# JuliaRobotics/RigidBodyDynamics.jl

Hardware: AMD Instinct MI355X
Metric: ABA dynamics! evals/sec (Atlas 30-DoF, batch) (higher is better)
Workload: dtype f64

## Files before the change

### include/rbd_hip.h

```cpp
#ifndef RBD_HIP_H
#define RBD_HIP_H

#include <stdint.h>

#ifdef __cplusplus
extern "C" {
#endif

enum {
  RBD_OK = 0,
  RBD_ERR_INVALID_ARGUMENT = 1,
  RBD_ERR_DIMENSION_MISMATCH = 2,
  RBD_ERR_UNSUPPORTED = 3,
  RBD_ERR_NO_DEVICE = 4,
  RBD_ERR_HIP = 5,
  RBD_ERR_OUT_OF_MEMORY = 6,
  RBD_ERR_HAS_LOOPS = 7,
  RBD_ERR_NOT_POSITIVE_DEFINITE = 8
};

enum {
  RBD_JOINT_FIXED = 0,
  RBD_JOINT_REVOLUTE = 1,
  RBD_JOINT_PRISMATIC = 2,
// ... 1 lines not shown
  RBD_JOINT_PLANAR = 4,
  RBD_JOINT_QUAT_SPHERICAL = 5,
  RBD_JOINT_SINCOS_REVOLUTE = 6
};

enum { RBD_F64 = 0, RBD_F32 = 1 };
enum { RBD_LAYOUT_SOA = 0, RBD_LAYOUT_AOS = 1 };
enum { RBD_MEM_DEVICE = 0, RBD_MEM_HOST = 1 };
enum {
  RBD_ALGO_ABA = 0,
  RBD_ALGO_CRBA_CHOLESKY = 1,
  RBD_ALGO_ABA_LANES = 2,
  RBD_ALGO_ABA_CHAINS = 3,
  RBD_ALGO_ABA_BANKS = 4,
  RBD_ALGO_ABA_TRACKS = 5,
  RBD_ALGO_ABA_WALK = 6,
  RBD_ALGO_ABA_PIPE = 7,
  RBD_ALGO_ABA_COMPILED = 8
};

typedef struct rbd_loop_joint {
  int32_t predecessor;
  int32_t successor;
  int32_t joint_type;
  int32_t _pad;
  double axis[3];
  double pred_rot[9];
  double pred_trans[3];
  double succ_rot[9];
  double succ_trans[3];
  double rotation_from_z_aligned[9];
  double gains[4];
} rbd_loop_joint_t;

typedef struct rbd_contact_point {
  int32_t body;
  int32_t _pad;
  double location[3];
  double hc_k, hc_lambda, hc_n;
  double mu, k, b;
} rbd_contact_point_t;
typedef struct rbd_halfspace {
  double point[3];
  double outward_normal[3];
} rbd_halfspace_t;

typedef struct rbd_flat_model {
  int32_t n_bodies;
  int32_t nq, nv;
  int32_t n_loops;
  const int32_t* parent;
  const int32_t* joint_type;
  const int32_t* q_offset;
  const int32_t* v_offset;
  const double* joint_axis;
  const double* joint_axis2;
  const double* pred_rot;
  const double* pred_trans;
  const double* inertia_moment;
  const double* inertia_cross;
  const double* inertia_mass;
  double gravity[3];
  const rbd_loop_joint_t* loops;
  int32_t n_contact_points;
  int32_t n_halfspaces;
  const rbd_contact_point_t* contact_points;
  const rbd_halfspace_t* halfspaces;
} rbd_flat_model_t;

typedef struct rbd_model rbd_model_t;
typedef struct rbd_ws rbd_ws_t;

typedef struct rbd_opts {
  int32_t layout;
  int32_t memory;
  int32_t algorithm;
  int32_t stabilization;
} rbd_opts_t;

int rbd_model_create(const rbd_flat_model_t* desc, rbd_model_t** out);
int rbd_model_destroy(rbd_model_t* model);
int rbd_model_bank_plan(const rbd_model_t* model, int32_t* lanes, int32_t* first_level_of_bank1, int32_t* bodies_bank0, int32_t* bodies_bank1,
                        int32_t* aba_in_scope);
int rbd_model_track_plan(const rbd_model_t* model, int32_t* dims, int32_t* table, int32_t table_cap, int32_t* ri, int32_t ri_cap, double* rr, int32_t rr_cap);
int rbd_model_reroot_plan(const rbd_model_t* model, int32_t* dims, int32_t* ri, int32_t ri_cap, double* rr, int32_t rr_cap, int32_t* wk, int32_t wk_cap,
                          int32_t* chain_i, double* chain_r, double* fxp);
int rbd_model_chain_plan(const rbd_model_t* model, int32_t* tracks, int32_t* steps, int32_t* lds_fields, int32_t* table, int32_t capacity);
int rbd_model_dims(const rbd_model_t* model, int32_t* n_bodies, int32_t* nq, int32_t* nv, int32_t* nc);

int rbd_workspace_create(const rbd_model_t* model, int32_t max_batch, int32_t device,
                         int32_t dtype, void* stream, rbd_ws_t** out);
int rbd_workspace_destroy(rbd_ws_t* ws);
int rbd_workspace_set_stream(rbd_ws_t* ws, void* stream);
int rbd_workspace_set_loop_gains(rbd_ws_t* ws, const double* gains);
int rbd_sync(rbd_ws_t* ws);

int rbd_dynamics(rbd_ws_t* ws, int32_t B, const void* q, const void* v, const void* tau,
                 const void* fext, void* vdot, void* qdot, void* lambda, const rbd_opts_t* opts);

int rbd_inverse_dynamics(rbd_ws_t* ws, int32_t B, const void* q, const void* v, const void* vdot,
                         const void* fext, void* tau_out, const rbd_opts_t* opts);

int rbd_dynamics_bias(rbd_ws_t* ws, int32_t B, const void* q, const void* v, const void* fext,
                      void* c_out, const rbd_opts_t* opts);

int rbd_inverse_dynamics_bodies(rbd_ws_t* ws, int32_t B, const void* q, const void* v, const void* vdot, const void* fext, void* tau_out,
                                void* jointwrenches_out, void* accelerations_out, const rbd_opts_t* opts);
int rbd_dynamics_bias_bodies(rbd_ws_t* ws, int32_t B, const void* q, const void* v, const void* fext, void* c_out, void* jointwrenches_out,
                             void* accelerations_out, const rbd_opts_t* opts);

int rbd_mass_matrix(rbd_ws_t* ws, int32_t B, const void* q, void* M_out, const rbd_opts_t* opts);

int rbd_mass_matrix_solve(rbd_ws_t* ws, int32_t B, const void* q, const void* rhs, void* x,
                          void* M_out, const rbd_opts_t* opts);
int rbd_mass_matrix_solve_packed(rbd_ws_t* ws, int32_t B, const void* q, const void* rhs, void* x, void* M_packed_out, const rbd_opts_t* opts);

int rbd_cholesky_solve(rbd_ws_t* ws, int32_t B, const void* M, const void* rhs, void* x, void* L_out, const rbd_opts_t* opts);

int rbd_dynamics_result(rbd_ws_t* ws, int32_t B, void* M, void* c, void* K, void* k,
                        const rbd_opts_t* opts);
int rbd_workspace_bind_result(rbd_ws_t* ws, void* M, void* c);

int rbd_simulate(rbd_ws_t* ws, int32_t B, void* q, void* v, const void* tau, const void* fext, double dt, int32_t nsteps,
                 const rbd_opts_t* opts);
int rbd_mk_stage(rbd_ws_t* ws, int32_t B, int32_t stage, double dt, void* q, void* v, const void* vdot_prev, const rbd_opts_t* opts);

enum { RBD_CONTROL_CONSTANT = 0, RBD_CONTROL_TABLE = 1, RBD_CONTROL_PD = 2 };
typedef struct rbd_control {
  int32_t kind;
  int32_t per_stage;
  const void* tau;
  const void* q_des;
  const void* kp;
  const void* kd;
} rbd_control_t;
int rbd_simulate_controlled(rbd_ws_t* ws, int32_t B, void* q, void* v, const rbd_control_t* control, const void* fext, double dt, int32_t nsteps,
                            const rbd_opts_t* opts);

int rbd_model_contact_dims(const rbd_model_t* model, int32_t* n_contact_points, int32_t* n_halfspaces, int32_t* n_additional_states);
int rbd_contact_dynamics(rbd_ws_t* ws, int32_t B, const void* q, const void* v, void* s, void* contactwrenches, void* sdot, const rbd_opts_t* opts);
int rbd_dynamics_contact(rbd_ws_t* ws, int32_t B, const void* q, const void* v, void* s, const void* tau, const void* fext, void* vdot, void* qdot,
                         void* sdot, void* contactwrenches, void* totalwrenches, const rbd_opts_t* opts);
int rbd_simulate_contact(rbd_ws_t* ws, int32_t B, void* q, void* v, void* s, const void* tau, const void* fext, double dt, int32_t nsteps,
                         const rbd_opts_t* opts);

int rbd_kinematics(rbd_ws_t* ws, int32_t B, const void* q, const void* v, void* momentum_matrix, void* com, void* energy,
                   const rbd_opts_t* opts);

int rbd_momentum(rbd_ws_t* ws, int32_t B, const void* q, const void* v, void* out, const rbd_opts_t* opts);

int rbd_geometric_jacobian(rbd_ws_t* ws, int32_t B, const void* q, int32_t base_body, int32_t target_body, void* jac, const rbd_opts_t* opts);

typedef struct rbd_comm rbd_comm_t;
int rbd_comm_unique_id(void* id128);
int rbd_comm_create(const void* id128, int32_t world, int32_t rank, int32_t device, rbd_comm_t** out);
int rbd_comm_destroy(rbd_comm_t* comm);
int rbd_comm_info(const rbd_comm_t* comm, int32_t* world, int32_t* rank);
int rbd_gather(rbd_comm_t* comm, int32_t dtype, const void* shard, void* gathered, int64_t count, int32_t root , void* stream);
int rbd_gatherv(rbd_comm_t* comm, int32_t dtype, const void* shard, void* gathered, const int64_t* counts, int32_t root , void* stream);
const char* rbd_comm_last_error(void);

int rbd_inverse_dynamics_jvp(rbd_ws_t* ws, int32_t B, int32_t ntan, const void* q, const void* v, const void* vdot,
                             const void* fext, const void* dq, const void* dv, const void* dvdot, const void* dfext,
                             void* tau_out, void* dtau_out, const rbd_opts_t* opts);
int rbd_dynamics_jvp(rbd_ws_t* ws, int32_t B, int32_t ntan, const void* q, const void* v, const void* tau,
                     const void* fext, const void* dq, const void* dv, const void* dtau, const void* dfext,
// ... 50 lines not shown
```

### rigidbodydynamics.jl_amd/__init__.py

```python
from .mechanism import (DEFAULT_GRAVITATIONAL_ACCELERATION, CartesianFrame3D, Fixed, FlatModel, Joint, JointType, Mechanism,
                        Planar, Prismatic, QuaternionFloating, QuaternionSpherical, Revolute, RigidBody, SinCosRevolute,
                        SpatialInertia, Transform3D, attach_, flatten, rand_configuration, rand_velocity,
                        remove_fixed_tree_joints_, rot_z_y_x, rotation_between, ContactPoint, HalfSpace3D, HuntCrossleyModel, SoftContactModel,
                        ViscoelasticCoulombModel, add_contact_point_, add_environment_primitive_, hunt_crossley_hertz)
from .urdf import default_urdf_joint_types, parse_pose, parse_urdf, write_urdf
from .builders import (maximal_coordinates, FOUR_BAR_INITIAL_Q, FOUR_BAR_INITIAL_V, double_pendulum, four_bar_linkage, quickstart_double_pendulum,
                       rand_tree_mechanism, randmech, tree_mechanism)
from .flatio import load_flat_model, save_flat_model
from . import _capi
from .state import (PDGains, SE3PDGains, default_constraint_stabilization_gains, TorqueTable, PDControl, jit_source, jit_precompile, jit_status, bank_plan, track_plan, reroot_plan, momentum, momentum_rate_bias, geometric_jacobian_, chain_plan, center_of_mass, gravitational_potential_energy, kinetic_energy, momentum_matrix_, DimensionMismatch, DynamicsResult, MechanismState, dynamics_, dynamics_bias_, dynamics_ode_, inverse_dynamics_, mass_matrix_, unpack_lower, inverse_dynamics_jvp_, dynamics_jvp_, inverse_dynamics_derivatives_, dynamics_derivatives_, simulate_jvp_, simulate_step_derivatives_, inverse_dynamics_vjp_, dynamics_vjp_, simulate_vjp_, jacobian_view, set_points_, point_kinematics_, point_kinematics_vjp_, point_jacobian_view, contact_dynamics_vjp_, dynamics_contact_vjp_, simulate_contact_vjp_,
                    mass_matrix_solve_, rand_, set_configuration_, set_velocity_, simulate_, sync, last_kernel, zero_configuration_)
from .distributed import Comm, gather_results, shard_range, shard_sizes
from . import autograd
```

### rigidbodydynamics.jl_amd/_capi.py

```python
from __future__ import annotations

import atexit
import ctypes
import os

_HERE = os.path.dirname(os.path.abspath(__file__))
LIB_PATH = os.environ.get("RBD_LIB") or os.path.join(_HERE, "csrc", "librbd_hip.so")

RBD_OK = 0
HEADER_VERSION = 700
F64, F32 = 0, 1
LAYOUT_SOA, LAYOUT_AOS = 0, 1
MEM_DEVICE, MEM_HOST = 0, 1
ALGO_ABA, ALGO_CRBA_CHOLESKY, ALGO_ABA_LANES, ALGO_ABA_CHAINS, ALGO_ABA_BANKS, ALGO_ABA_TRACKS, ALGO_ABA_WALK, ALGO_ABA_PIPE, ALGO_ABA_COMPILED = 0, 1, 2, 3, 4, 5, 6, 7, 8

SYMBOLS = (
    "rbd_model_create", "rbd_model_destroy", "rbd_model_dims", "rbd_workspace_create", "rbd_workspace_destroy",
    "rbd_workspace_set_stream", "rbd_sync", "rbd_dynamics", "rbd_inverse_dynamics", "rbd_dynamics_bias", "rbd_mass_matrix",
    "rbd_mass_matrix_solve", "rbd_dynamics_result", "rbd_status_string", "rbd_last_hip_error",
    "rbd_workspace_enable_timing", "rbd_workspace_last_kernel_ms", "rbd_version", "rbd_simulate", "rbd_mk_stage", "rbd_cholesky_solve", "rbd_kinematics", "rbd_model_chain_plan", "rbd_workspace_last_kernel", "rbd_geometric_jacobian", "rbd_momentum", "rbd_model_bank_plan", "rbd_model_track_plan", "rbd_inverse_dynamics_bodies", "rbd_dynamics_bias_bodies",
    "rbd_model_reroot_plan", "rbd_model_contact_dims", "rbd_contact_dynamics", "rbd_dynamics_contact", "rbd_simulate_contact",
    "rbd_workspace_bind_result", "rbd_workspace_set_loop_gains", "rbd_jit_precompile", "rbd_jit_source", "rbd_jit_status", "rbd_jit_wait_idle", "rbd_simulate_controlled", "rbd_comm_unique_id", "rbd_comm_create", "rbd_comm_destroy", "rbd_comm_info", "rbd_gather", "rbd_gatherv", "rbd_mass_matrix_solve_packed", "rbd_comm_last_error", "rbd_jit_check_walk_object",
    "rbd_inverse_dynamics_jvp", "rbd_dynamics_jvp", "rbd_inverse_dynamics_derivatives", "rbd_dynamics_derivatives",
    "rbd_simulate_jvp", "rbd_simulate_step_derivatives",
    "rbd_inverse_dynamics_vjp", "rbd_dynamics_vjp",
    "rbd_simulate_vjp",
    "rbd_workspace_set_points", "rbd_point_kinematics", "rbd_point_kinematics_vjp",
    "rbd_contact_dynamics_vjp", "rbd_dynamics_contact_vjp",
    "rbd_simulate_contact_vjp",
)


class Opts(ctypes.Structure):
    _fields_ = [("layout", ctypes.c_int32), ("memory", ctypes.c_int32), ("algorithm", ctypes.c_int32), ("stabilization", ctypes.c_int32)]


class Control(ctypes.Structure):
    _fields_ = [("kind", ctypes.c_int32), ("per_stage", ctypes.c_int32), ("tau", ctypes.c_void_p), ("q_des", ctypes.c_void_p), ("kp", ctypes.c_void_p),
                ("kd", ctypes.c_void_p)]


CONTROL_CONSTANT, CONTROL_TABLE, CONTROL_PD = 0, 1, 2


class RBDError(RuntimeError):
    def __init__(self, status, where, detail=""):
        self.status = status
        super().__init__(f"{where}: status {status} ({detail})")


_lib = None


def lib():
    global _lib
    if _lib is None:
        if not os.path.exists(LIB_PATH):
            raise FileNotFoundError(f"{LIB_PATH} not built — run `python -c 'import __graft_entry__ as g; g.build()'` "
                                    "(rigidbodydynamics.jl_amd has no CPU fallback)")
        L = ctypes.CDLL(LIB_PATH)
        if L.rbd_version() != HEADER_VERSION:
            raise RuntimeError(f"{LIB_PATH} reports rbd_version {L.rbd_version()}, this binding is for {HEADER_VERSION}: rebuild (csrc/build.sh)")
        vp, i32 = ctypes.c_void_p, ctypes.c_int32
        L.rbd_status_string.restype = ctypes.c_char_p
        L.rbd_status_string.argtypes = [ctypes.c_int]
        L.rbd_last_hip_error.restype = ctypes.c_char_p
        L.rbd_model_create.argtypes = [vp, ctypes.POINTER(vp)]
        L.rbd_model_destroy.argtypes = [vp]
        L.rbd_model_dims.argtypes = [vp] + [ctypes.POINTER(i32)] * 4
        L.rbd_workspace_create.argtypes = [vp, i32, i32, i32, vp, ctypes.POINTER(vp)]
        L.rbd_workspace_destroy.argtypes = [vp]
        L.rbd_workspace_set_stream.argtypes = [vp, vp]
        L.rbd_workspace_bind_result.argtypes = [vp, vp, vp]
        L.rbd_workspace_set_loop_gains.argtypes = [vp, ctypes.POINTER(ctypes.c_double)]
        L.rbd_sync.argtypes = [vp]
        L.rbd_dynamics.argtypes = [vp, i32, vp, vp, vp, vp, vp, vp, vp, ctypes.POINTER(Opts)]
        L.rbd_inverse_dynamics.argtypes = [vp, i32, vp, vp, vp, vp, vp, ctypes.POINTER(Opts)]
        L.rbd_dynamics_bias.argtypes = [vp, i32, vp, vp, vp, vp, ctypes.POINTER(Opts)]
        L.rbd_inverse_dynamics_bodies.argtypes = [vp, i32, vp, vp, vp, vp, vp, vp, vp, ctypes.POINTER(Opts)]
        L.rbd_dynamics_bias_bodies.argtypes = [vp, i32, vp, vp, vp, vp, vp, vp, ctypes.POINTER(Opts)]
        L.rbd_mass_matrix.argtypes = [vp, i32, vp, vp, ctypes.POINTER(Opts)]
        L.rbd_mass_matrix_solve.argtypes = [vp, i32, vp, vp, vp, vp, ctypes.POINTER(Opts)]
        L.rbd_mass_matrix_solve_packed.argtypes = [vp, i32, vp, vp, vp, vp, ctypes.POINTER(Opts)]
        L.rbd_dynamics_result.argtypes = [vp, i32, vp, vp, vp, vp, ctypes.POINTER(Opts)]
        L.rbd_cholesky_solve.argtypes = [vp, i32, vp, vp, vp, vp, ctypes.POINTER(Opts)]
        L.rbd_inverse_dynamics_jvp.argtypes = [vp, i32, i32] + [vp] * 10 + [ctypes.POINTER(Opts)]
        L.rbd_dynamics_jvp.argtypes = [vp, i32, i32] + [vp] * 10 + [ctypes.POINTER(Opts)]
        L.rbd_inverse_dynamics_derivatives.argtypes = [vp, i32] + [vp] * 8 + [ctypes.POINTER(Opts)]
        L.rbd_dynamics_derivatives.argtypes = [vp, i32] + [vp] * 8 + [ctypes.POINTER(Opts)]
        L.rbd_simulate_jvp.argtypes = [vp, i32, i32, vp, vp, vp, vp, ctypes.c_double, i32, vp, vp, vp, vp, ctypes.POINTER(Opts)]
        L.rbd_simulate_step_derivatives.argtypes = [vp, i32, vp, vp, vp, vp, ctypes.c_double, vp, vp, ctypes.POINTER(Opts)]
        L.rbd_inverse_dynamics_vjp.argtypes = [vp, i32] + [vp] * 10 + [ctypes.POINTER(Opts)]
        L.rbd_dynamics_vjp.argtypes = [vp, i32] + [vp] * 10 + [ctypes.POINTER(Opts)]
        L.rbd_simulate_vjp.argtypes = [vp, i32, vp, vp, vp, vp, ctypes.c_double, i32, vp, vp, vp, vp, ctypes.POINTER(Opts)]
        L.rbd_workspace_set_points.argtypes = [vp, i32, ctypes.POINTER(i32), ctypes.POINTER(ctypes.c_double)]
        L.rbd_point_kinematics.argtypes = [vp, i32] + [vp] * 7 + [ctypes.POINTER(Opts)]
        L.rbd_point_kinematics_vjp.argtypes = [vp, i32] + [vp] * 6 + [ctypes.POINTER(Opts)]
        L.rbd_contact_dynamics_vjp.argtypes = [vp, i32] + [vp] * 9 + [ctypes.POINTER(Opts)]
        L.rbd_dynamics_contact_vjp.argtypes = [vp, i32] + [vp] * 15 + [ctypes.POINTER(Opts)]
        L.rbd_simulate_contact_vjp.argtypes = [vp, i32] + [vp] * 5 + [ctypes.c_double, i32] + [vp] * 5 + [ctypes.POINTER(Opts)]
        L.rbd_model_chain_plan.argtypes = [vp, ctypes.POINTER(i32), ctypes.POINTER(i32), ctypes.POINTER(i32), ctypes.POINTER(i32), i32]
        L.rbd_model_track_plan.argtypes = [vp, ctypes.POINTER(i32), ctypes.POINTER(i32), i32, ctypes.POINTER(i32), i32, ctypes.POINTER(ctypes.c_double), i32]
        L.rbd_comm_unique_id.argtypes = [vp]
        L.rbd_comm_create.argtypes = [vp, i32, i32, i32, ctypes.POINTER(vp)]
        L.rbd_comm_destroy.argtypes = [vp]
        L.rbd_comm_info.argtypes = [vp, ctypes.POINTER(i32), ctypes.POINTER(i32)]
        L.rbd_gather.argtypes = [vp, i32, vp, vp, ctypes.c_int64, i32, vp]
        L.rbd_gatherv.argtypes = [vp, i32, vp, vp, ctypes.POINTER(ctypes.c_int64), i32, vp]
        L.rbd_comm_last_error.restype = ctypes.c_char_p
        L.rbd_workspace_last_kernel.argtypes = [vp]
        L.rbd_workspace_last_kernel.restype = ctypes.c_char_p
        L.rbd_geometric_jacobian.argtypes = [vp, i32, vp, i32, i32, vp, ctypes.POINTER(Opts)]
        L.rbd_momentum.argtypes = [vp, i32, vp, vp, vp, ctypes.POINTER(Opts)]
        L.rbd_model_bank_plan.argtypes = [vp] + [ctypes.POINTER(i32)] * 5
        L.rbd_kinematics.argtypes = [vp, i32, vp, vp, vp, vp, vp, ctypes.POINTER(Opts)]
        L.rbd_simulate.argtypes = [vp, i32, vp, vp, vp, vp, ctypes.c_double, i32, ctypes.POINTER(Opts)]
        L.rbd_mk_stage.argtypes = [vp, i32, i32, ctypes.c_double, vp, vp, vp, ctypes.POINTER(Opts)]
        L.rbd_simulate_controlled.argtypes = [vp, i32, vp, vp, ctypes.POINTER(Control), vp, ctypes.c_double, i32, ctypes.POINTER(Opts)]
        L.rbd_model_reroot_plan.argtypes = [vp, ctypes.POINTER(i32), ctypes.POINTER(i32), i32, ctypes.POINTER(ctypes.c_double), i32, ctypes.POINTER(i32), i32,
                                            ctypes.POINTER(i32), ctypes.POINTER(ctypes.c_double), ctypes.POINTER(ctypes.c_double)]
        L.rbd_model_contact_dims.argtypes = [vp] + [ctypes.POINTER(i32)] * 3
        L.rbd_contact_dynamics.argtypes = [vp, i32, vp, vp, vp, vp, vp, ctypes.POINTER(Opts)]
        L.rbd_dynamics_contact.argtypes = [vp, i32, vp, vp, vp, vp, vp, vp, vp, vp, vp, vp, ctypes.POINTER(Opts)]
        L.rbd_simulate_contact.argtypes = [vp, i32, vp, vp, vp, vp, vp, ctypes.c_double, i32, ctypes.POINTER(Opts)]
        L.rbd_workspace_enable_timing.argtypes = [vp, i32]
        L.rbd_jit_precompile.argtypes = [vp, i32, ctypes.c_char_p, ctypes.c_int64]
        L.rbd_jit_source.argtypes = [vp, i32, i32, ctypes.c_char_p, ctypes.c_int64]
        L.rbd_jit_source.restype = ctypes.c_int64
        L.rbd_jit_status.argtypes = [vp, i32, i32]
        L.rbd_jit_check_walk_object.argtypes = [ctypes.c_char_p, ctypes.c_char_p, ctypes.c_int64, ctypes.c_char_p, ctypes.c_int64]
        L.rbd_jit_wait_idle.argtypes = []
        L.rbd_jit_wait_idle.restype = None
        atexit.register(L.rbd_jit_wait_idle)
        L.rbd_workspace_last_kernel_ms.argtypes = [vp, ctypes.POINTER(ctypes.c_float)]
        _lib = L
    return _lib


def check(status: int, where: str):
    if status != RBD_OK:
        L = lib()
        detail = L.rbd_status_string(status).decode()
        hip = L.rbd_last_hip_error().decode()
        if hip and (status in (4, 5, 6) or (status == 3 and "differs from the interpreting kernel" in hip)):
            detail += "; " + hip
        raise RBDError(status, where, detail)
```

### rigidbodydynamics.jl_amd/csrc/rbd_bank.hpp

```cpp
#pragma once

#ifndef RBD_BANK_WAVES
#define RBD_BANK_WAVES 2
#endif
#ifndef RBD_BANK_FK_LDS
#define RBD_BANK_FK_LDS 0
#endif
#ifndef RBD_BANK_HANDOFF_LDS
#define RBD_BANK_HANDOFF_LDS 0
#endif

#ifdef RBD_BANK_FIXED_NL
#define RBD_BANK_UNROLL _Pragma("unroll")
namespace rbd { constexpr int kBankNs[] = {RBD_BANK_FIXED_NS}; }
#define RBD_BK_NL RBD_BANK_FIXED_NL
#define RBD_BK_L0 RBD_BANK_FIXED_L0
#define RBD_BK_NS(l) kBankNs[l]
#ifdef RBD_BANK_FIXED_PERM
#define RBD_BK_PERM(l) (((RBD_BANK_FIXED_PERM) >> (l)) & 1ull)
#else
#define RBD_BK_PERM(l) (kBankNs[l] > 1)
#endif
#else
#define RBD_BANK_UNROLL _Pragma("unroll 1")
#define RBD_BK_NL M.nlevels
#define RBD_BK_L0 M.L0
#define RBD_BK_NS(l) ns_next(nss, M.ns_desc)
#define RBD_BK_PERM(l) ((M.perm_down >> (l)) & 1)
#endif

namespace rbd {

template <typename T> struct alignas(2 * sizeof(T)) Pair2 { T a, b; };

RBD_DEV void wave_lds_sync() {
  __builtin_amdgcn_fence(__ATOMIC_RELEASE, "wavefront");
  __builtin_amdgcn_wave_barrier();
  __builtin_amdgcn_fence(__ATOMIC_ACQUIRE, "wavefront");
}


#define RBD_MASSIGN6(MOV)                                                                                                              \
  unsigned long long sv;                                                                                                               \
  asm volatile("s_and_saveexec_b64 %[sv], %[mk]\n\t" MOV " %[d0], %[s0]\n\t" MOV " %[d1], %[s1]\n\t" MOV " %[d2], %[s2]\n\t" MOV          \
               " %[d3], %[s3]\n\t" MOV " %[d4], %[s4]\n\t" MOV " %[d5], %[s5]\n\ts_mov_b64 exec, %[sv]\n\ts_nop 0"                         \
               : [sv] "=&s"(sv), [d0] "+v"(d[0]), [d1] "+v"(d[1]), [d2] "+v"(d[2]), [d3] "+v"(d[3]), [d4] "+v"(d[4]), [d5] "+v"(d[5])    \
               : [mk] "s"(mask), [s0] "v"(s[0]), [s1] "v"(s[1]), [s2] "v"(s[2]), [s3] "v"(s[3]), [s4] "v"(s[4]), [s5] "v"(s[5])          \
               : "scc")
RBD_DEV void massign6(unsigned long long mask, double* d, const double* s) { RBD_MASSIGN6("v_mov_b64"); }
RBD_DEV void massign6(unsigned long long mask, float* d, const float* s) { RBD_MASSIGN6("v_mov_b32"); }
template <typename T, int N> RBD_DEV void massign(bool m, T* d, const T* s) {
  static_assert(N % 6 == 0, "blocks of 6");
  const unsigned long long mask = __builtin_amdgcn_ballot_w64(m);
#pragma unroll
  for (int k = 0; k < N; k += 6) massign6(mask, d + k, s + k);
}

enum { PK_KIN = 0, PK_FWD = 6, PARK_PAIRS = 16, PK_XCH = 16, XCH_PAIRS = 14, BANK_LDS_PAIRS = PARK_PAIRS + XCH_PAIRS };

template <typename T, int N> RBD_DEV void lds_put(Pair2<T>* col, int pair0, const T* x) {
#pragma unroll
  for (int i = 0; i < (N + 1) / 2; ++i) {
    Pair2<T> v;
    v.a = x[2 * i];
    v.b = (2 * i + 1 < N) ? x[2 * i + 1] : T(0);
    col[(pair0 + i) * 256] = v;
  }
}
template <typename T, int N> RBD_DEV void lds_get(const Pair2<T>* col, int pair0, T* x) {
#pragma unroll
  for (int i = 0; i < (N + 1) / 2; ++i) {
    const Pair2<T> v = col[(pair0 + i) * 256];
    x[2 * i] = v.a;
    if (2 * i + 1 < N) x[2 * i + 1] = v.b;
  }
}

__host__ __device__ constexpr int sym_row(int e) { return e < 6 ? 0 : e < 11 ? 1 : e < 15 ? 2 : e < 18 ? 3 : e < 20 ? 4 : 5; }
__host__ __device__ constexpr int sym_col(int e) { return e - SI(sym_row(e), sym_row(e)) + sym_row(e); }

template <typename T> struct BankRegs {
  Body<T> b;
  const T* rb;
  int pcol;
  T K[24];
  RBD_DEV T* R() { return K; }
  RBD_DEV T* p() { return K + 9; }
  RBD_DEV T* Tw() { return K + 12; }
  RBD_DEV T* vJ() { return K + 18; }
  T S[6], cb[6], IA[21], pA[6], U[6], Dinv, u;
  T tj[6];
  T acc[6], vd[6];
};

template <typename T> RBD_DEV void load_bank_body(const BankModel& M, int k, long B, Body<T>& b) {
  const int tid = blockIdx.x * blockDim.x + threadIdx.x;
  b.lane = threadIdx.x & 63;
  const long wave = tid >> 6;
  const int lps = M.lps;
  b.sub = b.lane & (lps - 1);
  b.base = b.lane - b.sub;
  b.state = wave * (64 / lps) + (b.lane / lps);
  b.valid = (b.sub < M.nbk[k]) && (b.state < B);
  const int4* ib4 = reinterpret_cast<const int4*>(M.ib[k] + (b.sub < M.nbk[k] ? b.sub : 0) * IB_STRIDE);
  const int4 w0 = ib4[0], w1 = ib4[1], w2 = ib4[2], w3 = ib4[3];
  static_assert(IB_PARENT == 0 && IB_JTYPE == 1 && IB_QOFF == 2 && IB_VOFF == 3 && IB_LEVEL == 4 && IB_NCHILD == 5 && IB_ORIG == 6 && IB_CHILD0 == 7 &&
                IB_MAXCHILD == 8 && IB_FLAGS == 15 && IB_STRIDE == 16, "record layout");
  b.parent = w0.x; b.jtype = w0.y; b.qoff = w0.z; b.voff = w0.w;
  b.level = b.valid ? w1.x : -1;
  b.nchild = w1.y; b.orig = w1.z;
  b.child[0] = w1.w; b.child[1] = w2.x; b.child[2] = w2.y; b.child[3] = w2.z; b.child[4] = w2.w; b.child[5] = w3.x; b.child[6] = w3.y; b.child[7] = w3.z;
  b.flags = w3.w;
  b.plane = b.parent >= 0 ? b.base + b.parent : b.lane;
}

template <typename T, bool SIMPLE>
RBD_DEV void bank_fk_commit(bool mine, BankRegs<T>& c, const T* k18 , const T* XR, const T* Xp, const T* tl) {
  const T* pR = k18;
  const T* pp = k18 + 9;
  const T* pT = k18 + 12;
  T n[24];
  matmul3(pR, XR, n);
  matvec3(pR, Xp, n + 9);
#pragma unroll
  for (int k = 0; k < 3; ++k) n[9 + k] += pp[k];
  if (SIMPLE) {
    T S[6];
    matvec3(n, tl, S);
    cross3(n + 9, S, S + 3);
#pragma unroll
    for (int k = 0; k < 6; ++k) n[12 + k] = pT[k] + S[k] * tl[3];
    massign<T, 18>(mine, c.K, n);
  } else {
    xmotion(n, n + 9, tl, n + 18);
#pragma unroll
    for (int k = 0; k < 6; ++k) n[12 + k] = pT[k] + n[18 + k];
    massign<T, 24>(mine, c.K, n);
  }
}
template <typename T, bool SIMPLE> RBD_DEV void bank_fk_step(const BankModel& M, int l, bool perm, BankRegs<T>& c, Pair2<T>* lds, const T* XR, const T* Xp, const T* tl) {
  T k18[18];
  if (RBD_BANK_FK_LDS || perm) {
    if (c.b.level == l - 1 && c.b.nchild >= 1) {
      RBD_KEEP_BRANCH();
      lds_put<T, 18>(lds + threadIdx.x, PK_XCH, c.K);
    }
    wave_lds_sync();
    lds_get<T, 18>(lds + c.pcol, PK_XCH, k18);
    wave_lds_sync();
  } else {
#pragma unroll
    for (int k = 0; k < 18; ++k) k18[k] = from_prev_lane(c.K[k]);
  }
  bank_fk_commit<T, SIMPLE>(c.b.level == l, c, k18, XR, Xp, tl);
}
template <typename T, bool SIMPLE> RBD_DEV void bank_fk_cross(int L0, BankRegs<T>& c, const Pair2<T>* lds, const T* XR, const T* Xp, const T* tl) {
  T k18[18];
// ... 41 lines not shown
  {
    T g[7], h[7];
    g[0] = gv.IA[20] - W[5] * gv.U[5];
    Iac[5] += g[0] * gv.cb[5];
#pragma unroll
    for (int k = 0; k < 6; ++k) g[1 + k] = gv.pA[k] + Iac[k] + W[k] * gv.u;
    if (MODE == 0) {
#pragma unroll
      for (int e = 0; e < 7; ++e) h[e] = from_next_lane(g[e]);
    }
    if (xw) lds_put<T, 7>(mycol, PK_XCH + 10, g);
    if (MODE == 0) {
      if (take0) {
        RBD_KEEP_BRANCH();
        tk.IA[20] += h[0];
#pragma unroll
        for (int k = 0; k < 6; ++k) tk.pA[k] += h[1 + k];
      }
    }
  }
  if (xw) {
    wave_lds_sync();
#pragma unroll 1
    for (int s = (MODE == 1 ? 0 : 1); s < ns; ++s) {
      if (takes && s < tk.b.nchild) {
        RBD_KEEP_BRANCH();
        const Pair2<T>* src = lds + (threadIdx.x - tk.b.sub + child_sel(tk.b, s));
        T x[28];
        lds_get<T, 28>(src, PK_XCH, x);
#pragma unroll
        for (int e = 0; e < 21; ++e) tk.IA[e] += x[e];
#pragma unroll
        for (int k = 0; k < 6; ++k) tk.pA[k] += x[21 + k];
      }
    }
    wave_lds_sync();
  }
}

template <typename T> RBD_DEV void bank_joint_accel(bool mine, BankRegs<T>& r, const T* a_parent) {
  T ap[6], n[6];
#pragma unroll
  for (int k = 0; k < 6; ++k) ap[k] = a_parent[k] + r.cb[k];
  const T x = r.Dinv * (r.u - dot6(r.U, ap));
#pragma unroll
  for (int k = 0; k < 6; ++k) n[k] = ap[k] + r.S[k] * x;
  massign<T, 6>(mine, r.acc, n);
  r.vd[0] = mine ? x : r.vd[0];
}
template <typename T> RBD_DEV void bank_accel_step(const BankModel& M, int l, bool perm, BankRegs<T>& c, Pair2<T>* lds) {
  T ap[6];
  if (RBD_BANK_FK_LDS || perm) {
    if (c.b.level == l - 1 && c.b.nchild >= 1) {
      RBD_KEEP_BRANCH();
      lds_put<T, 6>(lds + threadIdx.x, PK_XCH, c.acc);
    }
    wave_lds_sync();
    lds_get<T, 6>(lds + c.pcol, PK_XCH, ap);
    wave_lds_sync();
  } else {
#pragma unroll
    for (int k = 0; k < 6; ++k) ap[k] = from_prev_lane(c.acc[k]);
  }
  bank_joint_accel(c.b.level == l, c, ap);
}

#ifdef RBD_PROFILE_PHASES
__device__ long long rbd_bank_phase_clock[16];
#define RBD_MARK(i) do { if (blockIdx.x == 0 && threadIdx.x == 0) rbd_bank_phase_clock[i] = clock64(); } while (0)
#else
#define RBD_MARK(i)
#endif

template <typename T, bool R> struct InPtr { typedef const T* type; };
template <typename T> struct InPtr<T, true> { typedef const T* __restrict__ type; };

template <typename T, bool FUSED, bool SIMPLE>
RBD_DEV void aba_bank_body(const BankModel& M, long B, typename InPtr<T, !FUSED>::type q, typename InPtr<T, !FUSED>::type v, const T* __restrict__ tau,
                           const T* __restrict__ fext, T* __restrict__ vdot, T* __restrict__ qdot, Layout Lq, Layout Lv, Layout Lf, const MkFuse& F,
                           Pair2<T>* const lds) {
  Pair2<T>* const col = lds + threadIdx.x;
  RBD_MARK(0);
  BankRegs<T> r0, r1;
  auto fetch = [&](int k, BankRegs<T>& c, T* qj, T* vj) {
    load_bank_body(M, k, B, c.b);
    c.rb = reinterpret_cast<const T*>(M.rb[k]) + (c.b.sub < M.nbk[k] ? c.b.sub : 0) * RB_STRIDE;
    c.pcol = (int)threadIdx.x - c.b.sub + (c.b.parent >= 0 ? c.b.parent : c.b.sub);
    if (SIMPLE) {
      const bool fl = c.b.jtype == RBD_JOINT_QUAT_FLOATING;
      const long sc = c.b.state < B ? c.b.state : B - 1;
      const T* qp = q + ((long)c.b.qoff * Lq.sk + sc * Lq.sb);
      const long va = (long)c.b.voff * Lv.sk + sc * Lv.sb;
      const bool hv = v != nullptr, ht = tau != nullptr;
      qj[0] = qp[0];
      vj[0] = hv ? v[va] : T(0);
      c.tj[0] = ht ? tau[va] : T(0);
#pragma unroll
      for (int k2 = 1; k2 < 7; ++k2) qj[k2] = T(0);
#pragma unroll
      for (int k2 = 1; k2 < 6; ++k2) { vj[k2] = T(0); c.tj[k2] = T(0); }
      if (fl) {
        RBD_KEEP_BRANCH();
#pragma unroll
        for (int k2 = 1; k2 < 7; ++k2) qj[k2] = qp[k2 * Lq.sk];
        if (hv) {
#pragma unroll
          for (int k2 = 1; k2 < 6; ++k2) vj[k2] = v[va + k2 * Lv.sk];
        }
        if (ht) {
#pragma unroll
          for (int k2 = 1; k2 < 6; ++k2) c.tj[k2] = tau[va + k2 * Lv.sk];
        }
      }
    } else {
      load_joint_q(c.b, q, Lq, qj);
      load_joint_v(c.b, v, Lv, vj);
      load_joint_v(c.b, tau, Lv, c.tj);
    }
  };
  auto setup = [&](BankRegs<T>& c, T* qj, T* vj, T* XR, T* Xp, T* tl, T* ta ) {
    if (SIMPLE) {
      const bool fl = c.b.jtype == RBD_JOINT_QUAT_FLOATING;
      const T ax[3] = {c.rb[RB_AXIS], c.rb[RB_AXIS + 1], c.rb[RB_AXIS + 2]};
      T Rj[9], pj[3] = {T(0), T(0), T(0)};
      T sn, cs;
      ta[0] = ax[0]; ta[1] = ax[1]; ta[2] = ax[2]; ta[3] = vj[0];
      sincos_fast(qj[0], &sn, &cs);
      rot_axis_sc(ax, sn, cs, Rj);
#pragma unroll
      for (int k = 0; k < 3; ++k) { tl[k] = ax[k] * vj[0]; tl[3 + k] = T(0); }
      if (fl) {
        RBD_KEEP_BRANCH();
        rot_quat(qj[0], qj[1], qj[2], qj[3], Rj);
        pj[0] = qj[4]; pj[1] = qj[5]; pj[2] = qj[6];
#pragma unroll
        for (int k = 0; k < 6; ++k) tl[k] = vj[k];
        if (qdot != nullptr && c.b.valid) {
          const T w = qj[0], x = qj[1], y = qj[2], z = qj[3];
          T o[7];
          o[0] = (-x * vj[0] - y * vj[1] - z * vj[2]) * T(0.5);
          o[1] = (w * vj[0] - z * vj[1] + y * vj[2]) * T(0.5);
          o[2] = (z * vj[0] + w * vj[1] - x * vj[2]) * T(0.5);
          o[3] = (-y * vj[0] + x * vj[1] + w * vj[2]) * T(0.5);
          matvec3(Rj, vj + 3, o + 4);
#pragma unroll
          for (int k = 0; k < 7; ++k) qdot[(long)(c.b.qoff + k) * Lq.sk + c.b.state * Lq.sb] = o[k];
        }
      } else if (qdot != nullptr && c.b.valid) {
        qdot[(long)c.b.qoff * Lq.sk + c.b.state * Lq.sb] = vj[0];
      }
      T XpR[9], Xpp[3];
#pragma unroll
      for (int k = 0; k < 9; ++k) XpR[k] = c.rb[RB_XPR + k];
#pragma unroll
      for (int k = 0; k < 3; ++k) Xpp[k] = c.rb[RB_XPP + k];
      matmul3(XpR, Rj, XR);
      matvec3(XpR, pj, Xp);
#pragma unroll
      for (int k = 0; k < 3; ++k) Xp[k] += Xpp[k];
    } else {
      store_qdot(c.b, qdot, Lq, qj, vj);
      local_transform(c.b, c.rb, qj, XR, Xp);
      local_joint_motion(c.b, c.rb, vj, tl);
    }
#pragma unroll
    for (int i = 0; i < 9; ++i) c.R()[i] = XR[i];
#pragma unroll
    for (int i = 0; i < 3; ++i) c.p()[i] = Xp[i];
    xmotion(c.R(), c.p(), tl, c.Tw());
    if (SIMPLE) {
      c.K[18] = ta[3];
      c.K[19] = T(0);
    } else {
#pragma unroll
      for (int i = 0; i < 6; ++i) c.vJ()[i] = c.Tw()[i];
    }
  };
  auto terms = [&](BankRegs<T>& c, bool accumulate) {
    const bool floating = c.b.jtype == RBD_JOINT_QUAT_FLOATING;
    if (SIMPLE) {
      const T ax[3] = {c.rb[RB_AXIS], c.rb[RB_AXIS + 1], c.rb[RB_AXIS + 2]};
      matvec3(c.R(), ax, c.S);
      cross3(c.p(), c.S, c.S + 3);
    } else {
      T e1[6] = {T(1), T(0), T(0), T(0), T(0), T(0)}, sl[6];
      local_joint_motion(c.b, c.rb, e1, sl);
      xmotion(c.R(), c.p(), sl, c.S);
    }
    if (floating || (!SIMPLE && joint_nv(c.b.jtype) == 0)) {
#pragma unroll
      for (int i = 0; i < 6; ++i) c.S[i] = T(0);
    }
    if (SIMPLE) {
      se3_comm(c.Tw(), c.S, c.cb);
#pragma unroll
      for (int i = 0; i < 6; ++i) c.cb[i] *= c.K[18];
    } else {
      se3_comm(c.Tw(), c.vJ(), c.cb);
    }
    RInertia<T> I;
    T Jb[6], mc[3], fe[6];
#pragma unroll
    for (int i = 0; i < 6; ++i) Jb[i] = c.rb[RB_J + i];
#pragma unroll
    for (int i = 0; i < 3; ++i) mc[i] = c.rb[RB_MC + i];
    inertia_to_root(Jb, mc, c.rb[RB_M], c.R(), c.p(), I);
    T Io[21], po[6];
    sym6_from_inertia(I, Io);
    momentum_cross(I, c.Tw(), po);
    load_body_wrench(c.b, fext, Lf, fe);
#pragma unroll
    for (int i = 0; i < 21; ++i) c.IA[i] = accumulate ? c.IA[i] + Io[i] : Io[i];
#pragma unroll
    for (int i = 0; i < 6; ++i) c.pA[i] = accumulate ? c.pA[i] + (po[i] - fe[i]) : po[i] - fe[i];
#pragma unroll
    for (int i = 0; i < 6; ++i) c.U[i] = T(0);
    c.Dinv = T(0);
    c.u = T(0);
    if (floating) xforce(c.R(), c.p(), c.tj, c.U);
  };

  T qj0[7], vj0[6], qj1[7], vj1[6];
  fetch(0, r0, qj0, vj0);
  fetch(1, r1, qj1, vj1);
  if (FUSED) {
    if (F.close_prev) {
      mk_stage_lane(r0.b, 4, (T)F.dt, qj0, vj0, (const T*)nullptr, F.W, (T*)F.q_state, (T*)F.v_state, Lq, Lv);
      mk_stage_lane(r1.b, 4, (T)F.dt, qj1, vj1, (const T*)nullptr, F.W, (T*)F.q_state, (T*)F.v_state, Lq, Lv);
    }
    mk_stage_lane(r0.b, F.stage, (T)F.dt, qj0, vj0, (const T*)nullptr, F.W, (T*)F.q_state, (T*)F.v_state, Lq, Lv);
    mk_stage_lane(r1.b, F.stage, (T)F.dt, qj1, vj1, (const T*)nullptr, F.W, (T*)F.q_state, (T*)F.v_state, Lq, Lv);
    pd_control_lane(r0.b, F, Lq, qj0, vj0, r0.tj);
    pd_control_lane(r1.b, F, Lq, qj1, vj1, r1.tj);
  }
  {
    T XR[9], Xp[3], tl[6], ta[4];
    setup(r0, qj0, vj0, XR, Xp, tl, ta);
    RBD_MARK(1);
RBD_BANK_UNROLL
    for (int l = 1; l < RBD_BK_L0; ++l) bank_fk_step<T, SIMPLE>(M, l, RBD_BK_PERM(l), r0, lds, XR, Xp, SIMPLE ? ta : tl);
  }
  {
    T XR[9], Xp[3], tl[6], ta[4];
    RBD_MARK(2);
    setup(r1, qj1, vj1, XR, Xp, tl, ta);
    RBD_MARK(3);
    lds_put<T, (SIMPLE ? 20 : 24)>(col, PK_KIN, r0.K);
    wave_lds_sync();
    bank_fk_cross<T, SIMPLE>(RBD_BK_L0, r1, lds, XR, Xp, SIMPLE ? ta : tl);
RBD_BANK_UNROLL
    for (int l = RBD_BK_L0 + 1; l < RBD_BK_NL; ++l) bank_fk_step<T, SIMPLE>(M, l, RBD_BK_PERM(l), r1, lds, XR, Xp, SIMPLE ? ta : tl);
  }
  RBD_MARK(4);
  terms(r1, false);
  RBD_MARK(5);

  NsStream nss = ns_begin(M.ns_desc);
  (void)nss;
RBD_BANK_UNROLL
  for (int l = RBD_BK_NL - 1; l > RBD_BK_L0; --l) {
    bank_finish_joint<T, SIMPLE>(l, r1);
    bank_handoff<T, RBD_BANK_HANDOFF_LDS>(l, RBD_BK_NS(l), r1, r1, lds);
  }
  bank_finish_joint<T, SIMPLE>(RBD_BK_L0, r1);
  RBD_MARK(6);
#pragma unroll
  for (int i = 0; i < 21; ++i) r0.IA[i] = T(0);
#pragma unroll
  for (int i = 0; i < 6; ++i) r0.pA[i] = T(0);
  bank_handoff<T, 1>(RBD_BK_L0, RBD_BK_NS(RBD_BK_L0), r1, r0, lds);
  {
    lds_get<T, (SIMPLE ? 20 : 24)>(col, PK_KIN, r0.K);
    T f20[20];
#pragma unroll
    for (int i = 0; i < 6; ++i) { f20[i] = r1.U[i]; f20[8 + i] = r1.S[i]; f20[14 + i] = r1.cb[i]; }
    f20[6] = r1.Dinv;
    f20[7] = r1.u;
    lds_put<T, 20>(col, PK_FWD, f20);
  }
  RBD_MARK(7);
  terms(r0, true);
  RBD_MARK(8);
RBD_BANK_UNROLL
  for (int l = RBD_BK_L0 - 1; l >= 1; --l) {
    bank_finish_joint<T, SIMPLE>(l, r0);
    bank_handoff<T, RBD_BANK_HANDOFF_LDS>(l, RBD_BK_NS(l), r0, r0, lds);
  }
  bank_finish_joint<T, SIMPLE>(0, r0);
  RBD_MARK(9);

#pragma unroll
  for (int i = 0; i < 6; ++i) { r0.acc[i] = T(0); r0.vd[i] = T(0); }
  {
    const T a0[6] = {T(0), T(0), T(0), T(-M.gravity[0]), T(-M.gravity[1]), T(-M.gravity[2])};
    BankRegs<T>& c = r0;
    const bool fl0 = c.b.level == 0 && c.b.jtype == RBD_JOINT_QUAT_FLOATING;
    T fa[6] = {T(0), T(0), T(0), T(0), T(0), T(0)}, fv[6] = {T(0), T(0), T(0), T(0), T(0), T(0)};
    if (fl0) {
      RBD_KEEP_BRANCH();
      T rhs[6], d[6], k12[12];
#pragma unroll
      for (int i = 0; i < 6; ++i) rhs[i] = c.U[i] - c.pA[i];
      sym6_solve(c.IA, rhs, fa);
#pragma unroll
      for (int i = 0; i < 6; ++i) d[i] = fa[i] - a0[i];
      lds_get<T, 12>(col, PK_KIN, k12);
      xmotion_inv(k12, k12 + 9, d, fv);
    }
    massign<T, 6>(fl0, c.acc, fa);
    massign<T, 6>(fl0, c.vd, fv);
    bank_joint_accel(c.b.level == 0 && !fl0, c, a0);
  }
RBD_BANK_UNROLL
  for (int l = 1; l < RBD_BK_L0; ++l) bank_accel_step<T>(M, l, RBD_BK_PERM(l), r0, lds);
  RBD_MARK(10);
  if (vdot) store_joint_v(r0.b, vdot, Lv, r0.vd);
  if (FUSED) store_joint_v(r0.b, (T*)F.W.vd[F.stage], Lv, r0.vd);
  {
    T f20[20];
    lds_get<T, 20>(col, PK_FWD, f20);
#pragma unroll
    for (int i = 0; i < 6; ++i) {
      r1.U[i] = f20[i];
      r1.S[i] = f20[8 + i];
      r1.cb[i] = f20[14 + i];
      r1.acc[i] = T(0);
      r1.vd[i] = T(0);
    }
    r1.Dinv = f20[6];
    r1.u = f20[7];
  }
  {
    lds_put<T, 6>(col, PK_XCH, r0.acc);
    wave_lds_sync();
    T ap[6];
    lds_get<T, 6>(lds + r1.pcol, PK_XCH, ap);
    wave_lds_sync();
    bank_joint_accel(r1.b.level == RBD_BK_L0, r1, ap);
  }
RBD_BANK_UNROLL
  for (int l = RBD_BK_L0 + 1; l < RBD_BK_NL; ++l) bank_accel_step<T>(M, l, RBD_BK_PERM(l), r1, lds);
  RBD_MARK(11);
  if (vdot) store_joint_v(r1.b, vdot, Lv, r1.vd);
  if (FUSED) store_joint_v(r1.b, (T*)F.W.vd[F.stage], Lv, r1.vd);
}
#ifndef RBD_BANK_FIXED_NL
template <typename T, bool FUSED, bool SIMPLE>
__global__ __launch_bounds__(256, RBD_BANK_WAVES) void aba_bank_kernel(BankModel M, long B, typename InPtr<T, !FUSED>::type q, typename InPtr<T, !FUSED>::type v,
                                                         const T* __restrict__ tau, const T* __restrict__ fext, T* __restrict__ vdot,
                                                         T* __restrict__ qdot, Layout Lq, Layout Lv, Layout Lf, MkFuse F) {
  extern __shared__ double bank_lds_raw[];
  aba_bank_body<T, FUSED, SIMPLE>(M, B, q, v, tau, fext, vdot, qdot, Lq, Lv, Lf, F, reinterpret_cast<Pair2<T>*>(bank_lds_raw));
}
#endif

enum { RNEA_LDS_PAIRS = 12 };
template <typename T> struct RneaRegs {
  Body<T> b;
  const T* rb;
  int pcol;
  T K[24], w[6];
  RBD_DEV T* R() { return K; }
  RBD_DEV T* p() { return K + 9; }
  RBD_DEV T* Tw() { return K + 12; }
  RBD_DEV T* acc() { return K + 18; }
};

template <typename T, bool SIMPLE>
RBD_DEV void rnea_fk_commit(bool mine, RneaRegs<T>& c, const T* k24, const T* XR, const T* Xp, const T* tl, const T* al) {
  const T* pR = k24;
  const T* pp = k24 + 9;
  const T* pT = k24 + 12;
  const T* pa = k24 + 18;
  T n[24], vJ[6], nT[6], cr[6], aj[6];
  matmul3(pR, XR, n);
  matvec3(pR, Xp, n + 9);
#pragma unroll
  for (int k = 0; k < 3; ++k) n[9 + k] += pp[k];
  if (SIMPLE) {
    T S[6];
    matvec3(n, tl, S);
    cross3(n + 9, S, S + 3);
#pragma unroll
    for (int k = 0; k < 6; ++k) { vJ[k] = S[k] * tl[3]; aj[k] = S[k] * tl[4]; }
  } else {
    xmotion(n, n + 9, tl, vJ);
    xmotion(n, n + 9, al, aj);
  }
#pragma unroll
  for (int k = 0; k < 6; ++k) { n[12 + k] = pT[k] + vJ[k]; nT[k] = -n[12 + k]; }
  se3_comm(nT, pT, cr);
#pragma unroll
  for (int k = 0; k < 6; ++k) n[18 + k] = pa[k] + cr[k] + aj[k];
  massign<T, 24>(mine, c.K, n);
}
template <typename T, bool SIMPLE>
RBD_DEV void rnea_fk_step(const BankModel& M, int l, bool perm, RneaRegs<T>& c, Pair2<T>* lds, const T* XR, const T* Xp, const T* tl, const T* al) {
  T k24[24];
  if (perm) {
    if (c.b.level == l - 1 && c.b.nchild >= 1) {
      RBD_KEEP_BRANCH();
      lds_put<T, 24>(lds + threadIdx.x, 0, c.K);
    }
    wave_lds_sync();
    lds_get<T, 24>(lds + c.pcol, 0, k24);
    wave_lds_sync();
  } else {
#pragma unroll
    for (int k = 0; k < 24; ++k) k24[k] = from_prev_lane(c.K[k]);
  }
  rnea_fk_commit<T, SIMPLE>(c.b.level == l, c, k24, XR, Xp, tl, al);
}

template <typename T, bool CROSS> RBD_DEV void rnea_gather(int l, int ns, const RneaRegs<T>& gv, RneaRegs<T>& tk) {
  const bool takes = (tk.b.level == l - 1);
  if (!CROSS) {
    T t[6];
#pragma unroll
    for (int k = 0; k < 6; ++k) t[k] = from_next_lane(gv.w[k]);
    if (takes && tk.b.nchild >= 1) {
      RBD_KEEP_BRANCH();
#pragma unroll
      for (int k = 0; k < 6; ++k) tk.w[k] += t[k];
    }
  }
#pragma unroll 1
  for (int s = CROSS ? 0 : 1; s < ns; ++s) {
    const bool take = takes && (s < tk.b.nchild);
    const int src = take ? tk.b.base + child_sel(tk.b, s) : tk.b.lane;
    T t[6];
#pragma unroll
    for (int k = 0; k < 6; ++k) t[k] = shfl(gv.w[k], src);
    if (take) {
      RBD_KEEP_BRANCH();
#pragma unroll
      for (int k = 0; k < 6; ++k) tk.w[k] += t[k];
    }
  }
}

template <typename T, bool SIMPLE>
RBD_DEV void rnea_bank_body(const BankModel& M, long B, int ncol, const T* __restrict__ q, const T* __restrict__ v, const T* __restrict__ vdot,
                            const T* __restrict__ fext, T* __restrict__ tau, T* __restrict__ qdot, Layout Lq, Layout Lv, Layout Lf, T* __restrict__ acc_out,
                            T* __restrict__ jw_out, Pair2<T>* const lds) {
  RneaRegs<T> r0, r1;
  const bool out_vec = store6_vec(acc_out ? acc_out : jw_out, Lf, (int)sizeof(T)) && store6_vec(jw_out ? jw_out : acc_out, Lf, (int)sizeof(T));
  auto fetch = [&](int k, RneaRegs<T>& c, T* qj, T* vj, T* aj) {
    load_bank_body(M, k, B, c.b);
    c.rb = reinterpret_cast<const T*>(M.rb[k]) + (c.b.sub < M.nbk[k] ? c.b.sub : 0) * RB_STRIDE;
    c.pcol = (int)threadIdx.x - c.b.sub + (c.b.parent >= 0 ? c.b.parent : c.b.sub);
    if (SIMPLE) {
      const bool fl = c.b.jtype == RBD_JOINT_QUAT_FLOATING;
      const long sc = c.b.state < B ? c.b.state : B - 1;
      const T* qp = q + ((long)c.b.qoff * Lq.sk + sc * Lq.sb);
      const long va = (long)c.b.voff * Lv.sk + sc * Lv.sb;
      const bool hv = v != nullptr, ha = vdot != nullptr;
      qj[0] = qp[0];
      vj[0] = hv ? v[va] : T(0);
      aj[0] = ha ? vdot[va] : T(0);
#pragma unroll
      for (int k2 = 1; k2 < 7; ++k2) qj[k2] = T(0);
#pragma unroll
      for (int k2 = 1; k2 < 6; ++k2) { vj[k2] = T(0); aj[k2] = T(0); }
      if (fl) {
        RBD_KEEP_BRANCH();
#pragma unroll
        for (int k2 = 1; k2 < 7; ++k2) qj[k2] = qp[k2 * Lq.sk];
        if (hv) {
#pragma unroll
          for (int k2 = 1; k2 < 6; ++k2) vj[k2] = v[va + k2 * Lv.sk];
        }
        if (ha) {
#pragma unroll
          for (int k2 = 1; k2 < 6; ++k2) aj[k2] = vdot[va + k2 * Lv.sk];
        }
      }
    } else {
      load_joint_q(c.b, q, Lq, qj);
      load_joint_v(c.b, v, Lv, vj);
      load_joint_v(c.b, vdot, Lv, aj);
    }
  };
  auto setup = [&](RneaRegs<T>& c, const T* qj, const T* vj, const T* aj, T* XR, T* Xp, T* tl, T* al, T* ta) {
    if (SIMPLE) {
      const bool fl = c.b.jtype == RBD_JOINT_QUAT_FLOATING;
      const T ax[3] = {c.rb[RB_AXIS], c.rb[RB_AXIS + 1], c.rb[RB_AXIS + 2]};
      ta[0] = ax[0]; ta[1] = ax[1]; ta[2] = ax[2]; ta[3] = vj[0]; ta[4] = aj[0];
      T Rj[9], pj[3] = {T(0), T(0), T(0)}, sn, cs;
      sincos_fast(qj[0], &sn, &cs);
      rot_axis_sc(ax, sn, cs, Rj);
#pragma unroll
      for (int k = 0; k < 3; ++k) { tl[k] = ax[k] * vj[0]; tl[3 + k] = T(0); al[k] = ax[k] * aj[0]; al[3 + k] = T(0); }
      if (fl) {
        RBD_KEEP_BRANCH();
        rot_quat(qj[0], qj[1], qj[2], qj[3], Rj);
        pj[0] = qj[4]; pj[1] = qj[5]; pj[2] = qj[6];
#pragma unroll
        for (int k = 0; k < 6; ++k) { tl[k] = vj[k]; al[k] = aj[k]; }
        if (qdot != nullptr && c.b.valid) {
          const T w = qj[0], x = qj[1], y = qj[2], z = qj[3];
          T o[7];
          o[0] = (-x * vj[0] - y * vj[1] - z * vj[2]) * T(0.5);
          o[1] = (w * vj[0] - z * vj[1] + y * vj[2]) * T(0.5);
          o[2] = (z * vj[0] + w * vj[1] - x * vj[2]) * T(0.5);
          o[3] = (-y * vj[0] + x * vj[1] + w * vj[2]) * T(0.5);
          matvec3(Rj, vj + 3, o + 4);
#pragma unroll
          for (int k = 0; k < 7; ++k) qdot[(long)(c.b.qoff + k) * Lq.sk + c.b.state * Lq.sb] = o[k];
        }
      } else if (qdot != nullptr && c.b.valid) {
        qdot[(long)c.b.qoff * Lq.sk + c.b.state * Lq.sb] = vj[0];
      }
      T XpR[9], Xpp[3];
#pragma unroll
      for (int k = 0; k < 9; ++k) XpR[k] = c.rb[RB_XPR + k];
#pragma unroll
      for (int k = 0; k < 3; ++k) Xpp[k] = c.rb[RB_XPP + k];
      matmul3(XpR, Rj, XR);
      matvec3(XpR, pj, Xp);
#pragma unroll
      for (int k = 0; k < 3; ++k) Xp[k] += Xpp[k];
    } else {
      store_qdot(c.b, qdot, Lq, qj, vj);
      local_transform(c.b, c.rb, qj, XR, Xp);
      local_joint_motion(c.b, c.rb, vj, tl);
      local_joint_motion(c.b, c.rb, aj, al);
    }
#pragma unroll
    for (int i = 0; i < 9; ++i) c.R()[i] = XR[i];
#pragma unroll
    for (int i = 0; i < 3; ++i) c.p()[i] = Xp[i];
    xmotion(c.R(), c.p(), tl, c.Tw());
    xmotion(c.R(), c.p(), al, c.acc());
    c.acc()[3] -= T(M.gravity[0]); c.acc()[4] -= T(M.gravity[1]); c.acc()[5] -= T(M.gravity[2]);
  };
  auto newton_euler = [&](RneaRegs<T>& c) {
    RInertia<T> I;
    T Jb[6], mc[3], Ia[6], x[6], fe[6];
#pragma unroll
    for (int k = 0; k < 6; ++k) Jb[k] = c.rb[RB_J + k];
#pragma unroll
    for (int k = 0; k < 3; ++k) mc[k] = c.rb[RB_MC + k];
    inertia_to_root(Jb, mc, c.rb[RB_M], c.R(), c.p(), I);
    mul_inertia(I, c.acc(), Ia);
    momentum_cross(I, c.Tw(), x);
    load_body_wrench(c.b, fext, Lf, fe);
#pragma unroll
    for (int k = 0; k < 6; ++k) c.w[k] = Ia[k] + x[k] - fe[k];
    if (acc_out != nullptr && c.b.valid) store6(acc_out, 6L * c.b.orig, Lf, c.b.state, c.acc(), out_vec);
  };
  auto project = [&](RneaRegs<T>& c) {
    T out[6] = {T(0), T(0), T(0), T(0), T(0), T(0)};
    if (c.b.jtype == RBD_JOINT_QUAT_FLOATING) {
      xforce_inv(c.R(), c.p(), c.w, out);
    } else if (SIMPLE) {
      const T ax[3] = {c.rb[RB_AXIS], c.rb[RB_AXIS + 1], c.rb[RB_AXIS + 2]};
      T S[6];
      matvec3(c.R(), ax, S);
      cross3(c.p(), S, S + 3);
      out[0] = dot6(S, c.w);
    } else {
      const T ax[3] = {c.rb[RB_AXIS], c.rb[RB_AXIS + 1], c.rb[RB_AXIS + 2]}, ay[3] = {c.rb[RB_AXIS2], c.rb[RB_AXIS2 + 1], c.rb[RB_AXIS2 + 2]};
      for (int k = 0; k < ncol; ++k) {
        T sl[6], S[6];
        subspace_col(c.b.jtype, ax, ay, k, sl);
        xmotion(c.R(), c.p(), sl, S);
        const T d = dot6(S, c.w);
        if (k == 0) out[0] = d; else if (k == 1) out[1] = d; else out[2] = d;
      }
    }
    store_joint_v(c.b, tau, Lv, out);
    if (jw_out != nullptr && c.b.valid) store6(jw_out, 6L * c.b.orig, Lf, c.b.state, c.w, out_vec);
  };

  T qj0[7], vj0[6], aj0[6], qj1[7], vj1[6], aj1[6];
  fetch(0, r0, qj0, vj0, aj0);
  fetch(1, r1, qj1, vj1, aj1);
  {
    T XR[9], Xp[3], tl[6], al[6], ta[5];
    setup(r0, qj0, vj0, aj0, XR, Xp, tl, al, ta);
RBD_BANK_UNROLL
    for (int l = 1; l < RBD_BK_L0; ++l) rnea_fk_step<T, SIMPLE>(M, l, RBD_BK_PERM(l), r0, lds, XR, Xp, SIMPLE ? ta : tl, al);
  }
  {
    T XR[9], Xp[3], tl[6], al[6], ta[5];
    setup(r1, qj1, vj1, aj1, XR, Xp, tl, al, ta);
    {
      T k24[24];
      lds_put<T, 24>(lds + threadIdx.x, 0, r0.K);
      wave_lds_sync();
      lds_get<T, 24>(lds + r1.pcol, 0, k24);
      wave_lds_sync();
      rnea_fk_commit<T, SIMPLE>(r1.b.level == RBD_BK_L0, r1, k24, XR, Xp, SIMPLE ? ta : tl, al);
    }
RBD_BANK_UNROLL
    for (int l = RBD_BK_L0 + 1; l < RBD_BK_NL; ++l) rnea_fk_step<T, SIMPLE>(M, l, RBD_BK_PERM(l), r1, lds, XR, Xp, SIMPLE ? ta : tl, al);
  }
  newton_euler(r1);
  newton_euler(r0);
  NsStream nss = ns_begin(M.ns_desc);
  (void)nss;
RBD_BANK_UNROLL
  for (int l = RBD_BK_NL - 1; l > RBD_BK_L0; --l) rnea_gather<T, false>(l, RBD_BK_NS(l), r1, r1);
  rnea_gather<T, true>(RBD_BK_L0, RBD_BK_NS(RBD_BK_L0), r1, r0);
RBD_BANK_UNROLL
  for (int l = RBD_BK_L0 - 1; l >= 1; --l) rnea_gather<T, false>(l, RBD_BK_NS(l), r0, r0);
  project(r0);
  project(r1);
}
#ifndef RBD_BANK_FIXED_NL
template <typename T, bool SIMPLE>
__global__ __launch_bounds__(256, 2) void rnea_bank_kernel(BankModel M, long B, int ncol, const T* __restrict__ q, const T* __restrict__ v,
                                                          const T* __restrict__ vdot, const T* __restrict__ fext, T* __restrict__ tau,
                                                          T* __restrict__ qdot, Layout Lq, Layout Lv, Layout Lf, T* __restrict__ acc_out,
                                                          T* __restrict__ jw_out) {
  extern __shared__ double bank_lds_raw[];
  rnea_bank_body<T, SIMPLE>(M, B, ncol, q, v, vdot, fext, tau, qdot, Lq, Lv, Lf, acc_out, jw_out, reinterpret_cast<Pair2<T>*>(bank_lds_raw));
}
#endif

}
```

### rigidbodydynamics.jl_amd/csrc/rbd_bank_kernels.hip

```cpp
#include "rbd_lane.hpp"
#include "rbd_internal.hpp"
#include "rbd_bank.hpp"

namespace rbd {

static_assert(BANK_LDS_PAIRS == 30, "rbd_capi.hip sizes the resident batch of the banked kernel with BANK_LDS_PAIRS_HOST = 30");
template <typename T> static size_t bank_lds_bytes() { return (size_t)BANK_LDS_PAIRS * 256 * sizeof(Pair2<T>); }

template <typename T>
hipError_t launch_aba_bank(const BankModel& M, long B, const void* q, const void* v, const void* tau, const void* fext, void* vdot, void* qdot,
                           Layout Lq, Layout Lv, Layout Lf, hipStream_t s, const MkFuse* fuse) {
  MkFuse F{};
  F.stage = -1;
  if (fuse) F = *fuse;
  const long spw = 64 / M.lps, waves = (B + spw - 1) / spw;
  const dim3 grid((unsigned)((waves + 3) / 4)), block(256);
  const size_t lds = bank_lds_bytes<T>();
#define RBD_LAUNCH_BANK(FU, SI) \
  hipLaunchKernelGGL((aba_bank_kernel<T, FU, SI>), grid, block, lds, s, M, B, (const T*)q, (const T*)v, (const T*)tau, (const T*)fext, (T*)vdot, (T*)qdot, Lq, Lv, Lf, F)
  if (F.stage >= 0) { if (M.simple) RBD_LAUNCH_BANK(true, true); else RBD_LAUNCH_BANK(true, false); }
  else if (M.simple) RBD_LAUNCH_BANK(false, true);
  else RBD_LAUNCH_BANK(false, false);
#undef RBD_LAUNCH_BANK
  return hipGetLastError();
}
template <typename T> hipError_t configure_bank_kernels() {
  const int lds = (int)bank_lds_bytes<T>();
  hipError_t e = hipFuncSetAttribute(reinterpret_cast<const void*>(&aba_bank_kernel<T, false, false>), hipFuncAttributeMaxDynamicSharedMemorySize, lds);
  if (e == hipSuccess) e = hipFuncSetAttribute(reinterpret_cast<const void*>(&aba_bank_kernel<T, false, true>), hipFuncAttributeMaxDynamicSharedMemorySize, lds);
  if (e == hipSuccess) e = hipFuncSetAttribute(reinterpret_cast<const void*>(&aba_bank_kernel<T, true, false>), hipFuncAttributeMaxDynamicSharedMemorySize, lds);
  if (e == hipSuccess) e = hipFuncSetAttribute(reinterpret_cast<const void*>(&aba_bank_kernel<T, true, true>), hipFuncAttributeMaxDynamicSharedMemorySize, lds);
  return e;
}
template hipError_t configure_bank_kernels<double>();
template hipError_t configure_bank_kernels<float>();

#ifdef RBD_PROFILE_PHASES
extern "C" int rbd_debug_bank_phase_clock(long long* out16) {
  return (int)hipMemcpyFromSymbol(out16, HIP_SYMBOL(rbd_bank_phase_clock), sizeof(long long) * 16);
}
#endif
template hipError_t launch_aba_bank<double>(const BankModel&, long, const void*, const void*, const void*, const void*, void*, void*, Layout, Layout, Layout, hipStream_t, const MkFuse*);
template hipError_t launch_aba_bank<float>(const BankModel&, long, const void*, const void*, const void*, const void*, void*, void*, Layout, Layout, Layout, hipStream_t, const MkFuse*);

template <typename T>
hipError_t launch_rnea_bank(const BankModel& M, long B, int ncol, const void* q, const void* v, const void* vdot, const void* fext, void* tau, void* qdot,
                            Layout Lq, Layout Lv, Layout Lf, hipStream_t s, void* acc_out, void* jw_out) {
  const long spw = 64 / M.lps, waves = (B + spw - 1) / spw;
  const size_t lds = (size_t)RNEA_LDS_PAIRS * 256 * sizeof(Pair2<T>);
  if (M.simple)
    hipLaunchKernelGGL((rnea_bank_kernel<T, true>), dim3((unsigned)((waves + 3) / 4)), dim3(256), lds, s, M, B, ncol, (const T*)q, (const T*)v, (const T*)vdot,
                       (const T*)fext, (T*)tau, (T*)qdot, Lq, Lv, Lf, (T*)acc_out, (T*)jw_out);
  else
    hipLaunchKernelGGL((rnea_bank_kernel<T, false>), dim3((unsigned)((waves + 3) / 4)), dim3(256), lds, s, M, B, ncol, (const T*)q, (const T*)v, (const T*)vdot,
                       (const T*)fext, (T*)tau, (T*)qdot, Lq, Lv, Lf, (T*)acc_out, (T*)jw_out);
  return hipGetLastError();
}
template hipError_t launch_rnea_bank<double>(const BankModel&, long, int, const void*, const void*, const void*, const void*, void*, void*, Layout, Layout, Layout, hipStream_t, void*, void*);
template hipError_t launch_rnea_bank<float>(const BankModel&, long, int, const void*, const void*, const void*, const void*, void*, void*, Layout, Layout, Layout, hipStream_t, void*, void*);

}
```

### rigidbodydynamics.jl_amd/csrc/rbd_capi.hip

```cpp
#include "rbd_capi_internal.hpp"
enum { BANK_LDS_PAIRS_HOST = 30 };

thread_local std::string g_last_hip_error;

static int joint_nq_host(int t) {
  switch (t) {
    case RBD_JOINT_FIXED: return 0;
    case RBD_JOINT_REVOLUTE: case RBD_JOINT_PRISMATIC: return 1;
    case RBD_JOINT_QUAT_FLOATING: return 7;
    case RBD_JOINT_PLANAR: return 3;
    case RBD_JOINT_QUAT_SPHERICAL: return 4;
    case RBD_JOINT_SINCOS_REVOLUTE: return 2;
    default: return -1;
  }
}
static int joint_nv_host(int t) {
  switch (t) {
    case RBD_JOINT_FIXED: return 0;
    case RBD_JOINT_REVOLUTE: case RBD_JOINT_PRISMATIC: case RBD_JOINT_SINCOS_REVOLUTE: return 1;
    case RBD_JOINT_QUAT_FLOATING: return 6;
    case RBD_JOINT_PLANAR: case RBD_JOINT_QUAT_SPHERICAL: return 3;
    default: return -1;
  }
}

long tune(const char* key, long dflt, bool* has) {
  if (has) *has = false;
  const char* e = getenv("RBD_TUNE");
  if (!e) return dflt;
  const size_t n = strlen(key);
  for (const char* p = e; *p;) {
    const char* end = strchr(p, ',');
    const size_t len = end ? (size_t)(end - p) : strlen(p);
    if (len > n && memcmp(p, key, n) == 0 && p[n] == '=') { if (has) *has = true; return atol(p + n + 1); }
    if (len == n && memcmp(p, key, n) == 0) { if (has) *has = true; return 1; }
    if (!end) break;
    p = end + 1;
  }
  return dflt;
}

static std::string loop_program_source(const rbd_model* m, int dtype, std::vector<int32_t>* xi_store);
static int bank_simple(const rbd_model* m);
static std::string bank_program_source(const rbd_model* m, int dtype, int simple);
static std::string walk_program_source(const rbd_model* m, int dtype, bool rerooted, int kind = 0, int pair = 0);
static bool walk_program_rerooted(const rbd_model* m, int dtype, int pair = 0);

extern "C" {

int rbd_version(void) { return RBD_HIP_H_VERSION; }
static std::string program_source(const rbd_model* m, int32_t dtype, int32_t family) {
  if (!m || (dtype != RBD_F32 && dtype != RBD_F64) || family < 0 || family > SPEC_KIN) return std::string();
  if (family == SPEC_KIN) return m->spec_plan().ok ? spec_source(m->spec_plan(), m->nb, m->nq, m->nv, m->row_mask.data(), m->gravity, dtype, SPEC_KIN) : std::string();
  if (family == SPEC_FAMILIES + 6) return walk_program_source(m, dtype, walk_program_rerooted(m, dtype), 2);
  if (family == SPEC_FAMILIES + 7) return dtype == RBD_F32 ? walk_program_source(m, dtype, walk_program_rerooted(m, dtype, 1), 2, 1) : std::string();
  std::vector<int32_t> xi;
  if (family < SPEC_FAMILIES && !m->spec_plan().ok) return std::string();
  if (family == SPEC_FAMILIES + 5) return bank_program_source(m, dtype, bank_simple(m));
  return family == SPEC_FAMILIES + 4 ? (dtype == RBD_F32 ? walk_program_source(m, dtype, false, 1, 1) : std::string())
         : family == SPEC_FAMILIES + 3 ? (dtype == RBD_F32 ? walk_program_source(m, dtype, walk_program_rerooted(m, dtype, 1), 0, 1) : std::string())
         : family == SPEC_FAMILIES + 2 ? walk_program_source(m, dtype, false, 1)
         : family == SPEC_FAMILIES + 1 ? walk_program_source(m, dtype, walk_program_rerooted(m, dtype))
         : family == SPEC_FAMILIES ? loop_program_source(m, dtype, &xi)
                                   : spec_source(m->spec_plan(), m->nb, m->nq, m->nv, m->row_mask.data(), m->gravity, dtype, family);
}
static bool family_is_walk(int family) { return (family > SPEC_FAMILIES && family <= SPEC_FAMILIES + 4) || family == SPEC_FAMILIES + 6 || family == SPEC_FAMILIES + 7; }
static int code_object_get(const std::string& src, bool walk, bool wait, std::vector<char>* code, std::string* log) {
  return walk ? jit_walk_code_object_get(src, wait, code, log) : jit_code_object_get(src, wait, code, log);
}
int64_t rbd_jit_source(const rbd_model_t* m, int32_t dtype, int32_t family, char* buf, int64_t cap) {
  const std::string s = program_source(m, dtype, family);
  if (s.empty()) return -1;
  if (buf && cap > 0) { const int64_t n = std::min<int64_t>(cap - 1, (int64_t)s.size()); memcpy(buf, s.data(), (size_t)n); buf[n] = 0; }
  return (int64_t)s.size();
}
void rbd_jit_wait_idle(void) { jit_wait_idle(); }
int rbd_jit_check_walk_object(const char* source, const void* code, int64_t size, char* log, int64_t cap) {
  if (log && cap > 0) log[0] = 0;
  if (!source || !code || size <= 0) return RBD_ERR_INVALID_ARGUMENT;
  std::vector<char> c((const char*)code, (const char*)code + size);
  std::string l;
  const bool ok = jit_walk_admit(source, &c, &l);
  if (log && cap > 0) { const int64_t n = std::min<int64_t>(cap - 1, (int64_t)l.size()); memcpy(log, l.data(), (size_t)n); log[n] = 0; }
  return ok ? RBD_OK : RBD_ERR_UNSUPPORTED;
// ... 226 lines not shown
    const int nc = (int)kids[i].size();
    if (nc > IB_MAXCHILD) { delete m; return RBD_ERR_UNSUPPORTED; }
    ib[IB_NCHILD] = nc;
    for (int k = 0; k < nc; ++k) ib[IB_CHILD0 + k] = m->slot_of[kids[i][k]];
    if (nc > m->maxchild) m->maxchild = nc;
  }
  for (int s = 0; s < nb; ++s) {
    const int i = m->order[s];
    for (int k = 0; k < (int)kids[i].size(); ++k) m->ib[(size_t)s * IB_STRIDE + IB_CHILD0 + k] = m->slot_of[kids[i][k]];
  }
  if (m->nlevels > MAX_LEVELS) { delete m; return RBD_ERR_UNSUPPORTED; }
  m->nslots.assign(MAX_LEVELS, 0);
  m->perm_down = 0;
  for (int s = 0; s < nb; ++s) {
    const int nc = m->ib[(size_t)s * IB_STRIDE + IB_NCHILD];
    if (nc > 0 && nc > m->nslots[level[s] + 1]) m->nslots[level[s] + 1] = nc;
    const int ps = m->ib[(size_t)s * IB_STRIDE + IB_PARENT];
    if (ps >= 0 && ps != s - 1) m->perm_down |= (uint64_t)1 << level[s];
    if (ps >= 0 && m->ib[(size_t)ps * IB_STRIDE + IB_CHILD0] != ps + 1) { delete m; return RBD_ERR_INVALID_ARGUMENT; }
  }
  m->rb.assign((size_t)nb * RB_STRIDE, 0.0);
  for (int s = 0; s < nb; ++s) {
    const int i = m->order[s];
    double* rb = &m->rb[(size_t)s * RB_STRIDE];
    for (int k = 0; k < 3; ++k) rb[RB_AXIS + k] = d->joint_axis[3 * i + k];
    if (d->joint_axis2) for (int k = 0; k < 3; ++k) rb[RB_AXIS2 + k] = d->joint_axis2[3 * i + k];
    for (int k = 0; k < 9; ++k) rb[RB_XPR + k] = d->pred_rot[9 * i + k];
    for (int k = 0; k < 3; ++k) rb[RB_XPP + k] = d->pred_trans[3 * i + k];
    const double* J = d->inertia_moment + 9 * i;
    rb[RB_J + 0] = J[0]; rb[RB_J + 1] = J[1]; rb[RB_J + 2] = J[2]; rb[RB_J + 3] = J[4]; rb[RB_J + 4] = J[5]; rb[RB_J + 5] = J[8];
    for (int k = 0; k < 3; ++k) rb[RB_MC + k] = d->inertia_cross[3 * i + k];
    rb[RB_M] = d->inertia_mass[i];
  }
  m->dof_body.assign(m->nv > 0 ? m->nv : 1, 0);
  for (int i = 0; i < nb; ++i)
    for (int k = 0; k < joint_nv_host(d->joint_type[i]); ++k) m->dof_body[d->v_offset[i] + k] = m->slot_of[i];
  m->anc.assign((size_t)nb * m->nlevels, -1);
  for (int s = 0; s < nb; ++s) {
    int a = s;
    for (int k = 0; k < m->nlevels && a >= 0; ++k) { m->anc[(size_t)s * m->nlevels + k] = a; a = m->ib[(size_t)a * IB_STRIDE + IB_PARENT]; }
  }
  m->row_words = std::max(1, (m->nv + 63) / 64);
  m->row_mask.assign((size_t)(m->nv > 0 ? m->nv : 1) * m->row_words, 0);
  for (int r = 0; r < m->nv; ++r) {
    const int sr = m->dof_body[r];
    for (int c = 0; c <= r; ++c) {
      const int sc = m->dof_body[c];
      bool sup = false;
      for (int k = 0; k < m->nlevels; ++k) sup |= (m->anc[(size_t)sr * m->nlevels + k] == sc);
      if (sup) m->row_mask[(size_t)r * m->row_words + c / 64] |= (uint64_t)1 << (c % 64);
    }
  }
  m->nc = 0;
  m->jt_ref.assign(d->joint_type, d->joint_type + nb);
  m->parent_ref.assign(d->parent, d->parent + nb);
  m->voff_ref.assign(d->v_offset, d->v_offset + nb);
  m->qoff_ref.assign(d->q_offset, d->q_offset + nb);
  for (int i = 0; i < nb; ++i) {
    const int jt = d->joint_type[i];
    if (jt == RBD_JOINT_QUAT_FLOATING) { m->mkf.push_back(d->q_offset[i]); m->mkf.push_back(d->v_offset[i]); }
    else if (jt == RBD_JOINT_REVOLUTE || jt == RBD_JOINT_PRISMATIC || jt == RBD_JOINT_SINCOS_REVOLUTE) { m->mk1.push_back(d->q_offset[i]); m->mk1.push_back(d->v_offset[i]); m->mk1.push_back(jt); }
  }
  m->loop_fused_ok = d->n_loops > 0 && nb <= 4 && m->nv <= 4;
  for (int i = 0; i < nb && m->loop_fused_ok; ++i) {
    const int t = d->joint_type[i];
    m->loop_fused_ok = d->parent[i] < i && (t == RBD_JOINT_REVOLUTE || t == RBD_JOINT_PRISMATIC || t == RBD_JOINT_SINCOS_REVOLUTE || t == RBD_JOINT_FIXED);
  }
  m->axis_ref.assign(d->joint_axis, d->joint_axis + 3 * nb);
  if (d->joint_axis2) m->axis2_ref.assign(d->joint_axis2, d->joint_axis2 + 3 * nb); else m->axis2_ref.assign(3 * nb, 0.0);
  if (int lst = build_loop_tables(m, d)) { delete m; return lst; }
  m->bank_aba_ok = (m->nloops == 0 && !m->has3dof && !m->inner_floating);
  if (m->nlevels >= 2) {
    std::vector<int> per_level(m->nlevels, 0);
    for (int s = 0; s < nb; ++s) per_level[level[s]]++;
    int best_L0 = 0, best_lanes = 1 << 30, best_diff = 1 << 30;
    for (int L0 = 1; L0 < m->nlevels; ++L0) {
      int cA = 0, cB = 0;
      for (int l = 0; l < m->nlevels; ++l) (l < L0 ? cA : cB) += per_level[l];
      int lanes = 1;
      while (lanes < std::max(cA, cB)) lanes <<= 1;
      const int diff = std::abs(cA - cB);
      if (lanes < best_lanes || (lanes == best_lanes && diff < best_diff)) { best_lanes = lanes; best_L0 = L0; best_diff = diff; }
    }
    if (best_lanes < m->lps) {
      m->bank_lps = best_lanes; m->bank_L0 = best_L0;
      std::vector<int> bslot(nb, -1);
      int cnt[2] = {0, 0};
      for (int s = 0; s < nb; ++s) bslot[s] = cnt[level[s] >= best_L0]++;
      m->bank_nb[0] = cnt[0]; m->bank_nb[1] = cnt[1];
      for (int k = 0; k < 2; ++k) { m->bank_ib[k].assign((size_t)std::max(cnt[k], 1) * IB_STRIDE, -1); m->bank_rb[k].assign((size_t)std::max(cnt[k], 1) * RB_STRIDE, 0.0); }
      m->bank_perm_down = 0;
      for (int s = 0; s < nb; ++s) {
        const int k = level[s] >= best_L0, j = bslot[s];
        const int32_t* src = &m->ib[(size_t)s * IB_STRIDE];
        int32_t* dst = &m->bank_ib[k][(size_t)j * IB_STRIDE];
        memcpy(dst, src, sizeof(int32_t) * IB_STRIDE);
        const int ps = src[IB_PARENT];
        dst[IB_PARENT] = ps < 0 ? -1 : bslot[ps];
        for (int c2 = 0; c2 < src[IB_NCHILD]; ++c2) dst[IB_CHILD0 + c2] = bslot[src[IB_CHILD0 + c2]];
        if (ps >= 0 && level[s] != best_L0 && bslot[ps] != j - 1) { m->bank_perm_down |= (uint64_t)1 << level[s]; dst[IB_FLAGS] |= BFD_NOTFIRST; }
        memcpy(&m->bank_rb[k][(size_t)j * RB_STRIDE], &m->rb[(size_t)s * RB_STRIDE], sizeof(double) * RB_STRIDE);
      }
    }
  }
  {
    int nheads = 0;
    for (int s = 0; s < nb; ++s) {
      const int ps = m->ib[(size_t)s * IB_STRIDE + IB_PARENT];
      if (ps < 0 || m->ib[(size_t)ps * IB_STRIDE + IB_CHILD0] != s) ++nheads;
    }
    int G = 1;
    while (G < nheads && G < 4) G <<= 1;
    if (m->nloops == 0) m->chain = build_chain_plan(nb, m->ib, G);
    if (m->nloops == 0 && G <= 4) m->track = build_track_plan(nb, m->ib, m->rb, G);
    if (m->track.ok) m->walk = build_walk_plan(m->track.ns, m->track.G, m->track.ri);
    if (m->nloops == 0 && m->nv <= 64) m->state = build_state_plan(nb, m->ib, m->rb);
    if (m->nloops == 0 && m->nv <= 64 && !m->state.ok) m->state_wide = build_state_plan(nb, m->ib, m->rb, true);
  }
  if (m->bank_aba_ok) {
    m->rr = build_reroot(d);
    if (m->rr.ok) {
      const Reroot& R = m->rr;
      rbd_model::RrSlots& S = m->rrs;
      std::vector<std::vector<int>> kd(nb);
      for (int i = 0; i < nb; ++i) if (R.parent[i] >= 0) kd[R.parent[i]].push_back(i);
      std::vector<int> ord, slot(nb, -1), lev(nb, 0);
      {
        std::vector<int> stack{R.root};
        while (!stack.empty()) {
          const int i = stack.back(); stack.pop_back();
          slot[i] = (int)ord.size();
          ord.push_back(i);
          for (auto it = kd[i].rbegin(); it != kd[i].rend(); ++it) stack.push_back(*it);
        }
      }
      bool fits = (int)ord.size() == nb;
      for (int i = 0; i < nb && fits; ++i) fits = (int)kd[i].size() <= IB_MAXCHILD;
      if (fits) {
        S.ib.assign((size_t)nb * IB_STRIDE, -1);
        S.rb.assign((size_t)nb * RB_STRIDE, 0.0);
        S.nslots.assign(MAX_LEVELS, 0);
        for (int s2 = 0; s2 < nb; ++s2) {
          const int i = ord[s2], p = R.parent[i], ps = p < 0 ? -1 : slot[p];
          lev[s2] = ps < 0 ? 0 : lev[ps] + 1;
          if (lev[s2] + 1 > S.nlevels) S.nlevels = lev[s2] + 1;
          int32_t* ib = &S.ib[(size_t)s2 * IB_STRIDE];
          ib[IB_PARENT] = ps; ib[IB_JTYPE] = R.jtype[i]; ib[IB_QOFF] = R.qoff[i]; ib[IB_VOFF] = R.voff[i]; ib[IB_LEVEL] = lev[s2]; ib[IB_ORIG] = i;
          ib[IB_FLAGS] = R.flags[i];
          ib[IB_NCHILD] = (int)kd[i].size();
          for (int k = 0; k < (int)kd[i].size(); ++k) ib[IB_CHILD0 + k] = slot[kd[i][k]];
          double* rb = &S.rb[(size_t)s2 * RB_STRIDE];
          for (int k = 0; k < 3; ++k) { rb[RB_AXIS + k] = R.axis[3 * i + k]; rb[RB_AXIS2 + k] = R.axis2[3 * i + k]; rb[RB_XPP + k] = R.Xpp[3 * i + k]; rb[RB_MC + k] = R.mc[3 * i + k]; }
          for (int k = 0; k < 9; ++k) rb[RB_XPR + k] = R.XpR[9 * i + k];
          for (int k = 0; k < 6; ++k) rb[RB_J + k] = R.J6[6 * i + k];
          rb[RB_M] = R.mass[i];
        }
        for (int s2 = 0; s2 < nb; ++s2) {
          const int nc = S.ib[(size_t)s2 * IB_STRIDE + IB_NCHILD];
          if (nc > 0 && nc > S.nslots[lev[s2] + 1]) S.nslots[lev[s2] + 1] = nc;
        }
        int nheads = 0;
        for (int s2 = 0; s2 < nb; ++s2) {
          const int ps = S.ib[(size_t)s2 * IB_STRIDE + IB_PARENT];
          if (ps < 0 || S.ib[(size_t)ps * IB_STRIDE + IB_CHILD0] != s2) ++nheads;
        }
        int G = 1;
        while (G < nheads && G < 4) G <<= 1;
        S.track = build_track_plan(nb, S.ib, S.rb, G);
        if (S.track.ok) {
          S.walk = build_walk_plan(S.track.ns, S.track.G, S.track.ri);
          if (S.walk.ok)
            for (size_t k = 0; k < S.walk.wk.size(); ++k) {
              const int e = S.track.tab[k];
              if (e >= 0) S.walk.wk[k] |= S.ib[(size_t)e * IB_STRIDE + IB_FLAGS] << 8;
            }
        }
        S.ok = true;
      }
    }
  }
  *out = m;
  return RBD_OK;
}

int rbd_model_destroy(rbd_model_t* m) {
  delete m;
  return RBD_OK;
}

int rbd_model_bank_plan(const rbd_model_t* m, int32_t* lanes, int32_t* first_level_of_bank1, int32_t* bodies_bank0, int32_t* bodies_bank1,
                        int32_t* aba_in_scope) {
  if (!m) return RBD_ERR_INVALID_ARGUMENT;
  if (m->bank_lps <= 0) return RBD_ERR_UNSUPPORTED;
  if (lanes) *lanes = m->bank_lps;
  if (first_level_of_bank1) *first_level_of_bank1 = m->bank_L0;
  if (bodies_bank0) *bodies_bank0 = m->bank_nb[0];
  if (bodies_bank1) *bodies_bank1 = m->bank_nb[1];
  if (aba_in_scope) *aba_in_scope = m->bank_aba_ok;
  return RBD_OK;
}

int rbd_model_chain_plan(const rbd_model_t* m, int32_t* tracks, int32_t* steps, int32_t* lds_fields, int32_t* table, int32_t capacity) {
  if (!m) return RBD_ERR_INVALID_ARGUMENT;
  if (!m->chain.ok) return RBD_ERR_UNSUPPORTED;
  if (tracks) *tracks = m->chain.G;
  if (steps) *steps = m->chain.ns;
  if (lds_fields) *lds_fields = 0;
  if (table) {
    if (capacity < (int32_t)m->chain.tab.size()) return RBD_ERR_DIMENSION_MISMATCH;
    for (size_t i = 0; i < m->chain.tab.size(); ++i) table[i] = m->chain.tab[i] < 0 ? -1 : m->order[m->chain.tab[i]];
  }
  return RBD_OK;
}

int rbd_model_track_plan(const rbd_model_t* m, int32_t* dims, int32_t* table, int32_t table_cap, int32_t* ri, int32_t ri_cap, double* rr, int32_t rr_cap) {
  if (!m) return RBD_ERR_INVALID_ARGUMENT;
  if (!m->track.ok) return RBD_ERR_UNSUPPORTED;
  const TrackPlan& P = m->track;
  if (dims) { dims[0] = P.G; dims[1] = P.ns; dims[2] = P.nA; dims[3] = P.nB; dims[4] = P.has_floating; dims[5] = P.general; }
  if (table) {
    if (table_cap < (int32_t)P.tab.size()) return RBD_ERR_DIMENSION_MISMATCH;
    for (size_t i = 0; i < P.tab.size(); ++i) table[i] = P.tab[i] < 0 ? -1 : m->order[P.tab[i]];
  }
  if (ri) {
    if (ri_cap < (int32_t)(P.ri.size() + P.sf.size())) return RBD_ERR_DIMENSION_MISMATCH;
    memcpy(ri, P.ri.data(), P.ri.size() * sizeof(int32_t));
    memcpy(ri + P.ri.size(), P.sf.data(), P.sf.size() * sizeof(int32_t));
  }
  if (rr) { if (rr_cap < (int32_t)P.rr.size()) return RBD_ERR_DIMENSION_MISMATCH; memcpy(rr, P.rr.data(), P.rr.size() * sizeof(double)); }
  return RBD_OK;
}

int rbd_model_reroot_plan(const rbd_model_t* m, int32_t* dims, int32_t* ri, int32_t ri_cap, double* rr, int32_t rr_cap, int32_t* wk, int32_t wk_cap,
                          int32_t* chain_i, double* chain_r, double* fxp) {
  if (!m) return RBD_ERR_INVALID_ARGUMENT;
  if (!m->rrs.ok || !m->rrs.track.ok || !m->rrs.walk.ok) return RBD_ERR_UNSUPPORTED;
  const TrackPlan& P = m->rrs.track;
  const Reroot& R = m->rr;
  const int nch = (int)(R.chain_i.size() / RC_I_STRIDE);
  if (dims) {
    const int32_t d[12] = {P.G, P.ns, P.nA, P.nB, P.has_floating, P.general, m->rrs.walk.nS, nch, R.fq, R.fv, R.root, R.fb};
    memcpy(dims, d, sizeof d);
  }
  if (ri) {
    if (ri_cap < (int32_t)(P.ri.size() + P.sf.size())) return RBD_ERR_DIMENSION_MISMATCH;
    memcpy(ri, P.ri.data(), P.ri.size() * sizeof(int32_t));
    memcpy(ri + P.ri.size(), P.sf.data(), P.sf.size() * sizeof(int32_t));
  }
  if (rr) { if (rr_cap < (int32_t)P.rr.size()) return RBD_ERR_DIMENSION_MISMATCH; memcpy(rr, P.rr.data(), P.rr.size() * sizeof(double)); }
  if (wk) { if (wk_cap < (int32_t)m->rrs.walk.wk.size()) return RBD_ERR_DIMENSION_MISMATCH; memcpy(wk, m->rrs.walk.wk.data(), m->rrs.walk.wk.size() * sizeof(int32_t)); }
  if (chain_i) memcpy(chain_i, R.chain_i.data(), R.chain_i.size() * sizeof(int32_t));
  if (chain_r) memcpy(chain_r, R.chain_r.data(), R.chain_r.size() * sizeof(double));
  if (fxp) memcpy(fxp, R.fXp, sizeof R.fXp);
  return RBD_OK;
}

int rbd_model_dims(const rbd_model_t* m, int32_t* nb, int32_t* nq, int32_t* nv, int32_t* nc) {
  if (!m) return RBD_ERR_INVALID_ARGUMENT;
  if (nb) *nb = m->nb;
  if (nq) *nq = m->nq;
  if (nv) *nv = m->nv;
  if (nc) *nc = m->nc;
  return RBD_OK;
}

static int upload_loop_tables(rbd_ws* w, const rbd_model* m, int dtype) {
  int st = RBD_OK;
  if (st == RBD_OK && m->nloops > 0) {
    st = upload(w->d_loop_i, m->loop_i.data(), m->loop_i.size() * sizeof(int32_t));
    if (st == RBD_OK) st = upload(w->d_loop_path, m->loop_path.data(), m->loop_path.size() * sizeof(int32_t));
    if (st == RBD_OK) st = upload(w->d_jt_ref, m->jt_ref.data(), m->jt_ref.size() * sizeof(int32_t));
    if (st == RBD_OK) st = upload(w->d_voff_ref, m->voff_ref.data(), m->voff_ref.size() * sizeof(int32_t));
    if (st == RBD_OK && m->loop_fused_ok) {
      std::vector<int32_t> xi(3 * (size_t)m->nb);
      for (int i = 0; i < m->nb; ++i) { xi[3 * i] = m->parent_ref[i]; xi[3 * i + 1] = m->qoff_ref[i]; xi[3 * i + 2] = m->slot_of[i]; }
      st = upload(w->d_fused_i, xi.data(), xi.size() * sizeof(int32_t));
    }
    if (st == RBD_OK) st = upload_real(w->d_loop_r, m->loop_r, dtype);
    if (st == RBD_OK) st = upload_real(w->d_axis_ref, m->axis_ref, dtype);
    if (st == RBD_OK) st = upload_real(w->d_axis2_ref, m->axis2_ref, dtype);
  }
  return st;
}

static int upload_contact_tables(rbd_ws* w, const rbd_model* m, int dtype) {
  if (m->ncp <= 0) return RBD_OK;
  int st = upload(w->d_cp_body, m->cp_body.data(), m->cp_body.size() * sizeof(int32_t));
  if (st == RBD_OK) st = upload_real(w->d_cp_r, m->cp_r, dtype);
  if (st == RBD_OK) st = upload_real(w->d_hs_r, m->hs_r, dtype);
  if (st != RBD_OK) return st;
  w->ctm.nb = m->nb; w->ctm.np = m->ncp; w->ctm.nh = m->nhs;
  w->ctm.cbody = (const int32_t*)w->d_cp_body.p; w->ctm.cp = w->d_cp_r.p; w->ctm.hs = w->d_hs_r.p;
  return RBD_OK;
}

int rbd_workspace_create(const rbd_model_t* m, int32_t max_batch, int32_t device, int32_t dtype, void* stream, rbd_ws_t** out) {
  if (!m || !out || max_batch < 1 || (dtype != RBD_F64 && dtype != RBD_F32)) return RBD_ERR_INVALID_ARGUMENT;
  *out = nullptr;
  int ndev = 0;
  if (hipGetDeviceCount(&ndev) != hipSuccess || ndev < 1) {
    g_last_hip_error = "hipGetDeviceCount: no device";
    return RBD_ERR_NO_DEVICE;
  }
  if (device < 0 || device >= ndev) return RBD_ERR_INVALID_ARGUMENT;
  HIP_TRY(hipSetDevice(device));
  std::unique_ptr<rbd_ws> owner(new (std::nothrow) rbd_ws());
  rbd_ws* w = owner.get();
  if (!w) return RBD_ERR_OUT_OF_MEMORY;
  w->model = m; w->device = device; w->dtype = dtype; w->max_batch = max_batch; w->stream = (hipStream_t)stream;
  if (m->big) {
    int st = upload(w->d_big_tbl, m->big_tbl.data(), m->big_tbl.size() * sizeof(int32_t));
    if (st == RBD_OK) st = upload_real(w->d_big_rb, m->big_rb, dtype);
    if (st == RBD_OK) { int zero = 0; st = upload(w->d_notpd, &zero, sizeof(int)); }
    if (st == RBD_OK) st = upload_loop_tables(w, m, dtype);
    if (st == RBD_OK) st = upload_contact_tables(w, m, dtype);
    if (st != RBD_OK) return st;
    w->big.nb = m->nb; w->big.nq = m->nq; w->big.nv = m->nv; w->big.tbl = (const int32_t*)w->d_big_tbl.p; w->big.rb = w->d_big_rb.p;
    memcpy(w->big.gravity, m->gravity, sizeof w->big.gravity);
    w->last_kernel = "big_* kernels (one thread per state, HBM scratch)";
    *out = owner.release();
    return RBD_OK;
  }
  int st = upload(w->d_ib, m->ib.data(), m->ib.size() * sizeof(int32_t));
  if (st == RBD_OK) st = upload_real(w->d_rb, m->rb, dtype);
  if (st == RBD_OK) st = upload(w->d_dof_body, m->dof_body.data(), m->dof_body.size() * sizeof(int32_t));
  if (st == RBD_OK) st = upload(w->d_anc, m->anc.data(), m->anc.size() * sizeof(int32_t));
  if (st == RBD_OK) st = upload(w->d_row_mask, m->row_mask.data(), m->row_mask.size() * sizeof(uint64_t));
  if (st == RBD_OK) { int zero = 0; st = upload(w->d_notpd, &zero, sizeof(int)); }
  if (st == RBD_OK) st = upload_loop_tables(w, m, dtype);
  if (st != RBD_OK) return st;
  DevModel& dm = w->dm;
  dm.nb = m->nb; dm.nq = m->nq; dm.nv = m->nv; dm.lps = m->lps; dm.nlevels = m->nlevels; dm.maxchild = m->maxchild; dm.maxnvj = m->maxnvj;
  dm.ib = (const int32_t*)w->d_ib.p; dm.rb = w->d_rb.p;
  dm.perm_down = m->perm_down;
  dm.inner_floating = m->inner_floating;
  dm.has3dof = m->has3dof;
  dm.nheavy = 0;
  for (int s2 = 0; s2 < m->nb; ++s2) {
    const int jt = m->ib[(size_t)s2 * IB_STRIDE + IB_JTYPE];
    if (jt != RBD_JOINT_QUAT_FLOATING && jt != RBD_JOINT_QUAT_SPHERICAL) continue;
    if (dm.nheavy < 4) { dm.heavy[dm.nheavy][0] = jt; dm.heavy[dm.nheavy][1] = m->ib[(size_t)s2 * IB_STRIDE + IB_QOFF]; dm.heavy[dm.nheavy][2] = m->ib[(size_t)s2 * IB_STRIDE + IB_VOFF]; }
    ++dm.nheavy;
  }
  nslots_pack_desc(dm.ns_desc, m->nslots.data(), m->nlevels);
  dm.dof_body = (const int32_t*)w->d_dof_body.p; dm.anc = (const int32_t*)w->d_anc.p; dm.row_mask = (const uint64_t*)w->d_row_mask.p; dm.row_words = m->row_words;
  memcpy(dm.gravity, m->gravity, sizeof dm.gravity);
  if (m->bank_lps > 0) {
    BankModel& bm = w->bm;
    for (int k = 0; k < 2 && st == RBD_OK; ++k) {
      st = upload(w->d_bank_ib[k], m->bank_ib[k].data(), m->bank_ib[k].size() * sizeof(int32_t));
      if (st != RBD_OK) break;
      st = upload_real(w->d_bank_rb[k], m->bank_rb[k], dtype);
      bm.ib[k] = (const int32_t*)w->d_bank_ib[k].p; bm.rb[k] = w->d_bank_rb[k].p; bm.nbk[k] = m->bank_nb[k];
    }
    if (st != RBD_OK) return st;
    bm.lps = m->bank_lps; bm.nlevels = m->nlevels; bm.L0 = m->bank_L0; bm.perm_down = m->bank_perm_down;
    bm.simple = bank_simple(m);
    if (tune("bank_generic", 0)) bm.simple = 0;
    nslots_pack_desc(bm.ns_desc, m->nslots.data(), m->nlevels);
    memcpy(bm.gravity, m->gravity, sizeof bm.gravity);
    w->bank_min_batch = 0;
    w->rnea_bank_min_batch = 0;
    {
      int ncu = 256;
      (void)hipDeviceGetAttribute(&ncu, hipDeviceAttributeMultiprocessorCount, device);
      if (m->has3dof) w->rnea_bank_min_batch = (long)ncu * 28 + 1;
    }
    { bool has; const long t = tune("bank_min_batch", 0, &has); if (has) w->bank_min_batch = w->rnea_bank_min_batch = t; }
    {
      int ncu = 256;
      (void)hipDeviceGetAttribute(&ncu, hipDeviceAttributeMultiprocessorCount, device);
      const size_t lds = (size_t)BANK_LDS_PAIRS_HOST * 256 * 2 * (dtype == RBD_F64 ? 8 : 4);
      const long per_cu = std::max<long>(1, std::min<long>(2, (long)(160 * 1024 / lds)));
      w->bank_resident_states = (long)ncu * per_cu * (256 / m->bank_lps);
    }
  }
  if (m->rrs.ok) {
    const Reroot& R = m->rr;
    const rbd_model::RrSlots& S = m->rrs;
    st = upload(w->d_rr_chain_i, R.chain_i.data(), R.chain_i.size() * sizeof(int32_t));
    if (st == RBD_OK) st = upload_real(w->d_rr_chain_r, R.chain_r, dtype);
    RerootView V{};
    V.nchain = (int32_t)(R.chain_i.size() / RC_I_STRIDE); V.fq = R.fq; V.fv = R.fv;
    V.chain_i = (const int32_t*)w->d_rr_chain_i.p; V.chain_r = w->d_rr_chain_r.p;
    memcpy(V.fXp, R.fXp, sizeof V.fXp);
    if (st == RBD_OK && S.track.ok && S.walk.ok) {
      const TrackPlan& P = S.track;
      st = upload(w->d_rrtrack_ri, P.ri.data(), P.ri.size() * sizeof(int32_t));
      if (st == RBD_OK) st = upload_real(w->d_rrtrack_rr, P.rr, dtype);
      if (st == RBD_OK) st = upload(w->d_rrwalk_wk, S.walk.wk.data(), S.walk.wk.size() * sizeof(int32_t));
      WalkModel& wm = w->wm_rr;
      wm.ns = P.ns; wm.G = P.G; wm.nA = P.nA; wm.nB = P.nB; wm.nS = S.walk.nS; wm.nq = m->nq; wm.nv = m->nv; wm.reroot = V;
      wm.ri = (const int32_t*)w->d_rrtrack_ri.p; wm.rr = w->d_rrtrack_rr.p; wm.wk = (const int32_t*)w->d_rrwalk_wk.p;
      for (int k = 0; k < 5; ++k) { wm.sfm[k] = 0; for (int s2 = 0; s2 < P.ns; ++s2) wm.sfm[k] |= (uint64_t)((P.sf[s2] >> k) & 1) << s2; }
      memcpy(wm.gravity, m->gravity, sizeof wm.gravity);
      const size_t es2 = dtype == RBD_F64 ? 8 : 4;
      w->walk_rr_lds_bytes = walk_lds_bytes(P.ns, P.G, m->nq, m->nv, P.nA, P.nB, S.walk.nS, es2, es2);
      if (w->walk_rr_lds_bytes > 160 * 1024) w->walk_rr_lds_bytes = 0;
      w->walk_rr_lds_bytes_pair = dtype == RBD_F32 ? walk_lds_bytes(P.ns, P.G, m->nq, m->nv, P.nA, P.nB, S.walk.nS, 8, 4) : 0;
      if (w->walk_rr_lds_bytes_pair > 160 * 1024) w->walk_rr_lds_bytes_pair = 0;
      w->walk_rr = st == RBD_OK && (w->walk_rr_lds_bytes > 0 || w->walk_rr_lds_bytes_pair > 0);
    }
    if (st != RBD_OK) return st;
  }
  if (m->track.ok) {
    const TrackPlan& P = m->track;
    st = upload(w->d_track_ri, P.ri.data(), P.ri.size() * sizeof(int32_t));
    if (st == RBD_OK) st = upload_real(w->d_track_rr, P.rr, dtype);
    if (st != RBD_OK) return st;
    TrackModel& tm = w->tm;
    tm.ns = P.ns; tm.G = P.G; tm.nA = P.nA; tm.nB = P.nB; tm.ri = (const int32_t*)w->d_track_ri.p; tm.rr = w->d_track_rr.p;
    for (int k = 0; k < 5; ++k) { tm.sfm[k] = 0; for (int s2 = 0; s2 < P.ns; ++s2) tm.sfm[k] |= (uint64_t)((P.sf[s2] >> k) & 1) << s2; }
    memcpy(tm.gravity, m->gravity, sizeof tm.gravity);
  }
  if ((st = upload_contact_tables(w, m, dtype)) != RBD_OK) return st;
  if (m->track.ok && m->walk.ok) {
    const TrackPlan& P = m->track;
    st = upload(w->d_walk_wk, m->walk.wk.data(), m->walk.wk.size() * sizeof(int32_t));
    if (st != RBD_OK) return st;
    w->spec_walk_min_batch = 8192;
    { bool has; const long t = tune("spec_walk_min_batch", 0, &has); if (has) w->spec_walk_min_batch = t; }
    w->spec_walk_f32 = tune("spec_walk_f32", 1) != 0;
    WalkModel& wm = w->wm;
    wm.ns = P.ns; wm.G = P.G; wm.nA = P.nA; wm.nB = P.nB; wm.nS = m->walk.nS; wm.nq = m->nq; wm.nv = m->nv;
    wm.ri = (const int32_t*)w->d_track_ri.p; wm.rr = w->d_track_rr.p; wm.wk = (const int32_t*)w->d_walk_wk.p;
    for (int k = 0; k < 5; ++k) wm.sfm[k] = w->tm.sfm[k];
    memcpy(wm.gravity, m->gravity, sizeof wm.gravity);
    const size_t es = dtype == RBD_F64 ? 8 : 4;
    w->walk_lds_bytes = walk_lds_bytes(P.ns, P.G, m->nq, m->nv, P.nA, P.nB, m->walk.nS, es, es);
    if (w->walk_lds_bytes > 160 * 1024) w->walk_lds_bytes = 0;
    w->walk_lds_bytes_pair = dtype == RBD_F32 ? walk_lds_bytes(P.ns, P.G, m->nq, m->nv, P.nA, P.nB, m->walk.nS, 8, 4) : 0;
    if (w->walk_lds_bytes_pair > 160 * 1024) w->walk_lds_bytes_pair = 0;
    {
      const size_t l1 = std::max(w->walk_lds_bytes, w->walk_rr ? w->walk_rr_lds_bytes : (size_t)0), l2 = std::max(w->walk_lds_bytes_pair, w->walk_rr ? w->walk_rr_lds_bytes_pair : (size_t)0);
      const hipError_t e = by_dtype(dtype, [&](auto t) { return configure_walk_kernel<decltype(t)>(P.has_floating, P.general, l1, l2); });
      if (e != hipSuccess) { g_last_hip_error = std::string("configure_walk_kernel: ") + hipGetErrorString(e); return RBD_ERR_HIP; }
    }
    {
      int ncu = 256;
      (void)hipDeviceGetAttribute(&ncu, hipDeviceAttributeMultiprocessorCount, device);
      w->walk_pair_min_batch = (long)ncu * 64 + 1;
      { bool has; const long t = tune("walk_pair_min_batch", 0, &has); if (has) w->walk_pair_min_batch = t; }
    }
    {
      int ncu = 256;
      (void)hipDeviceGetAttribute(&ncu, hipDeviceAttributeMultiprocessorCount, device);
      w->walk_min_batch = (m->bank_lps > 0 && m->bank_aba_ok ? w->bank_resident_states : (long)ncu * 4 * 2 * (64 / m->lps)) + 1;
      const bool banked = m->bank_lps > 0 && m->bank_aba_ok;
      w->walk_one_round_batch = banked ? (long)ncu * (256 / m->bank_lps) + 1 : w->walk_min_batch;
      w->rnea_walk_min_batch = banked ? std::max<long>(w->walk_min_batch, (long)ncu * 2 * (256 / m->bank_lps) + 1) : w->walk_min_batch;
      if (bool has = false; (void)tune("spec_walk_min_batch", 0, &has), !has) w->spec_walk_min_batch = std::min<long>(w->spec_walk_min_batch, w->walk_one_round_batch);
    }
    { bool has; const long t = tune("walk_min_batch", 0, &has); if (has) w->walk_min_batch = t; }
  }
  if (m->state.ok && m->state.nlevels <= state_max_levels(dtype == RBD_F64 ? 8 : 4)) {
    const StatePlan& P = m->state;
// ... 89 lines not shown
    HIP_TRY(hipMemcpy((char*)w->d_loop_r.p + es * (64 * (size_t)l + 24), w->dtype == RBD_F64 ? (const void*)g64 : (const void*)g32, 4 * es, hipMemcpyHostToDevice));
  }
  w->loop_gains = want;
  w->custom_gains = custom;
  return RBD_OK;
}

int rbd_workspace_bind_result(rbd_ws_t* w, void* M, void* c) {
  if (!w) return RBD_ERR_INVALID_ARGUMENT;
  for (void* p : {M, c}) {
    if (!p) continue;
    hipPointerAttribute_t a{};
    if (hipPointerGetAttributes(&a, p) != hipSuccess) { (void)hipGetLastError(); return RBD_ERR_INVALID_ARGUMENT; }
    if (a.type != hipMemoryTypeDevice && a.type != hipMemoryTypeManaged && a.type != hipMemoryTypeUnified) return RBD_ERR_INVALID_ARGUMENT;
  }
  w->bound_M = M;
  w->bound_c = c;
  return RBD_OK;
}

int rbd_sync(rbd_ws_t* w) {
  if (!w) return RBD_ERR_INVALID_ARGUMENT;
  HIP_TRY(hipSetDevice(w->device));
  HIP_TRY(hipStreamSynchronize(w->stream));
  int flag = 0;
  HIP_TRY(hipMemcpy(&flag, (int*)w->d_notpd.p, sizeof(int), hipMemcpyDeviceToHost));
  if (flag) {
    HIP_TRY(hipMemset((int*)w->d_notpd.p, 0, sizeof(int)));
    return RBD_ERR_NOT_POSITIVE_DEFINITE;
  }
  return RBD_OK;
}

int rbd_workspace_enable_timing(rbd_ws_t* w, int32_t enable) {
  if (!w) return RBD_ERR_INVALID_ARGUMENT;
  HIP_TRY(hipSetDevice(w->device));
  if (enable && !w->ev0) {
    HIP_TRY(hipEventCreate(&w->ev0));
    HIP_TRY(hipEventCreate(&w->ev1));
  }
  w->timing = enable ? 1 : 0;
  return RBD_OK;
}

const char* rbd_workspace_last_kernel(const rbd_ws_t* w) { return w ? w->last_kernel : ""; }

int rbd_workspace_last_kernel_ms(rbd_ws_t* w, float* ms) {
  if (!w || !ms || !w->ev_pending) return RBD_ERR_INVALID_ARGUMENT;
  HIP_TRY(hipEventSynchronize(w->ev1));
  HIP_TRY(hipEventElapsedTime(ms, w->ev0, w->ev1));
  return RBD_OK;
}

}

int ensure(DevBuf& b, size_t need) {
  if (b.bytes >= need) return RBD_OK;
  b.reset();
  HIP_TRY(hipMalloc(&b.p, need));
  b.bytes = need;
  return RBD_OK;
}

int upload(DevBuf& dst, const void* src, size_t bytes) {
  dst.reset();
  if (int st = ensure(dst, bytes ? bytes : 16)) return st;
  if (bytes) HIP_TRY(hipMemcpy(dst.p, src, bytes, hipMemcpyHostToDevice));
  return RBD_OK;
}

int upload_real(DevBuf& dst, const std::vector<double>& src, int dtype) {
  if (dtype == RBD_F64) return upload(dst, src.data(), src.size() * sizeof(double));
  const std::vector<float> f(src.begin(), src.end());
  return upload(dst, f.data(), f.size() * sizeof(float));
}

static int bank_simple(const rbd_model* m) {
  for (int i = 0; i < m->nb; ++i)
    if (m->jt_ref[i] != RBD_JOINT_REVOLUTE && !(m->jt_ref[i] == RBD_JOINT_QUAT_FLOATING && m->parent_ref[i] < 0)) return 0;
  return 1;
}
static std::string bank_program_source(const rbd_model* m, int dtype, int simple) {
  if (m->bank_lps <= 0) return std::string();
  return spec_bank_source(m->nlevels, m->bank_L0, m->nslots.data(), (unsigned long long)m->bank_perm_down, simple, dtype);
}
static std::string loop_program_source(const rbd_model* m, int dtype, std::vector<int32_t>* xi_store) {
  if (!m->loop_fused_ok) return std::string();
  xi_store->assign(3 * (size_t)m->nb, 0);
  for (int i = 0; i < m->nb; ++i) { (*xi_store)[3 * i] = m->parent_ref[i]; (*xi_store)[3 * i + 1] = m->qoff_ref[i]; (*xi_store)[3 * i + 2] = m->slot_of[i]; }
  LoopTables L{m->nb, m->nq, m->nv, m->nc, m->nloops, &m->loop_i, &m->loop_path, &m->jt_ref, &m->voff_ref, xi_store, &m->loop_r, &m->axis_ref, &m->axis2_ref, &m->rb, m->gravity};
  return spec_loop_source(L, dtype);
}
static bool walk_tables(const rbd_model* m, bool rerooted, WalkTables* W) {
  const TrackPlan* P; const WalkPlan* K;
  if (rerooted) { if (!m->rrs.ok || !m->rrs.track.ok || !m->rrs.walk.ok) return false; P = &m->rrs.track; K = &m->rrs.walk; }
  else { if (!m->track.ok || !m->walk.ok) return false; P = &m->track; K = &m->walk; }
  *W = WalkTables{};
  W->ns = P->ns; W->G = P->G; W->nA = P->nA; W->nB = P->nB; W->nS = K->nS; W->nq = m->nq; W->nv = m->nv; W->flt = P->has_floating; W->gen = P->general; W->rr = rerooted;
  W->ri = &P->ri; W->wk = &K->wk; W->rrc = &P->rr;
  W->mk1 = &m->mk1; W->mkf = &m->mkf;
  for (int k = 0; k < 5; ++k) { W->sfm[k] = 0; for (int s2 = 0; s2 < P->ns; ++s2) W->sfm[k] |= (uint64_t)((P->sf[s2] >> k) & 1) << s2; }
  if (rerooted) {
    W->nchain = (int)(m->rr.chain_i.size() / RC_I_STRIDE); W->fq = m->rr.fq; W->fv = m->rr.fv; W->chain_i = &m->rr.chain_i; W->chain_r = &m->rr.chain_r; W->fXp = m->rr.fXp;
    if (W->nchain < 1) return false;
  }
  return true;
}
static bool walk_program_rerooted(const rbd_model* m, int dtype, int pair) {
  WalkTables W;
  return tune("walk_no_reroot", 0) == 0 && walk_tables(m, true, &W) && walk_lds_bytes(W.ns, W.G, W.nq, W.nv, W.nA, W.nB, W.nS, (dtype == RBD_F64 || pair) ? 8 : 4, dtype == RBD_F64 ? 8 : 4) <= 160 * 1024;
}
static std::string walk_program_source(const rbd_model* m, int dtype, bool rerooted, int kind, int pair) {
  WalkTables W;
  if (!walk_tables(m, rerooted, &W)) return std::string();
  return walk_spec_source(W, dtype, kind, pair);
}
static bool capturing(rbd_ws* w);
template <class Source>
static hipModule_t spec_module(rbd_ws* w, SpecSlot& p, Source source, bool walk, bool wait, const char* fallback) {
  if (p.tried) return nullptr;
  if (!jit_available()) { p.tried = true; return nullptr; }
  if (capturing(w)) return nullptr;
  if (p.src.empty()) p.src = source();
  if (p.src.empty()) { p.tried = true; return nullptr; }
  std::string log;
  std::vector<char> code;
  const int js = code_object_get(p.src, walk, wait, &code, &log);
  if (js == JIT_PENDING) return nullptr;
  p.tried = true;
  std::string src;
  src.swap(p.src);
  if (js == JIT_FAILED || code.empty()) { g_last_hip_error = std::string("run-time compilation failed (") + fallback + "): " + log; return nullptr; }
  if (hipModuleLoadData(&p.mod, code.data()) != hipSuccess) { (void)hipGetLastError(); p.mod = nullptr; jit_cache_discard(src); return nullptr; }
  return p.mod;
}
static const int kNoScratchCheck = INT_MAX;
static hipFunction_t spec_kernel(hipModule_t mod, const char* name, int max_scratch, int* scratch = nullptr) {
  hipFunction_t f = nullptr;
  int bytes = 0;
  if (hipModuleGetFunction(&f, mod, name) != hipSuccess) { (void)hipGetLastError(); f = nullptr; }
  else if (max_scratch != kNoScratchCheck && (hipFuncGetAttribute(&bytes, HIP_FUNC_ATTRIBUTE_LOCAL_SIZE_BYTES, f) != hipSuccess || bytes > max_scratch)) { (void)hipGetLastError(); f = nullptr; }
  if (scratch) *scratch = bytes;
  return f;
}
static hipFunction_t spec_walk(rbd_ws* w, bool rerooted, int kind = 0, int pair = 0) {
  const int k = 4 * kind + (rerooted ? 2 : 0) + (pair ? 1 : 0);
  if (hipModule_t mod = spec_module(w, w->spec_prog[SPEC_WALK + k], [&] { return walk_program_source(w->model, w->dtype, rerooted, kind, pair); }, true, !jit_async(),
                                    "the interpreting kernel is used")) {
    const std::string name = std::string(kind == 1 ? "rnea_walk_spec_" : kind == 2 ? "aba_walk_sim_spec_" : "aba_walk_spec_") + walk_spec_suffix(w->dtype, pair);
    w->spec_walk[k].f = spec_kernel(mod, name.c_str(), w->spec_max_scratch);
  }
  return w->spec_walk[k].f;
}
int big_scratch(rbd_ws* w, int32_t B) { return ensure(w->d_big_scratch, esize(w) * big_scratch_elems(w->big, B)); }
static hipFunction_t spec_loop(rbd_ws* w) {
  auto source = [&] { std::vector<int32_t> xi; return loop_program_source(w->model, w->dtype, &xi); };
  if (hipModule_t mod = spec_module(w, w->spec_prog[SPEC_LOOP], source, false, !jit_async(), "the generic loop kernels are used"))
    w->spec_loop = spec_kernel(mod, w->dtype == RBD_F64 ? "loop_spec_f64" : "loop_spec_f32", 0);
  return w->spec_loop;
}

static bool spec_bank(rbd_ws* w) {
  SpecSlot& p = w->spec_prog[SPEC_BANK];
  if (w->model->bank_lps <= 0) p.tried = true;
  if (hipModule_t mod = spec_module(w, p, [&] { return bank_program_source(w->model, w->dtype, w->bm.simple); }, false, !jit_async(),
                                    "the banked kernels built with the library are used")) {
    const std::string sfx = w->dtype == RBD_F64 ? "f64" : "f32";
// ... 1134 lines not shown
```

### rigidbodydynamics.jl_amd/csrc/rbd_device.hpp

```cpp
#pragma once
#include <hip/hip_runtime.h>
#include <stdint.h>

#include "rbd_hip.h"

namespace rbd {

enum { IB_PARENT = 0, IB_JTYPE = 1, IB_QOFF = 2, IB_VOFF = 3, IB_LEVEL = 4, IB_NCHILD = 5, IB_ORIG = 6, IB_CHILD0 = 7, IB_MAXCHILD = 8, IB_FLAGS = IB_CHILD0 + IB_MAXCHILD , IB_STRIDE = 16  };
enum { BFD_VROOT = 1, BFD_FCARRY = 2, BFD_NOTFIRST = 4  };
struct RerootView {
  int32_t nchain, fq, fv, _pad;
  const int32_t* chain_i;
  const void* chain_r;
  double fXp[12];
};
enum { RB_AXIS = 0, RB_AXIS2 = 3, RB_XPR = 6, RB_XPP = 15, RB_J = 18, RB_MC = 24, RB_M = 27, RB_STRIDE = 28 };
enum { MAX_LEVELS = 64 };

struct NsStream {
  uint64_t w;
  int j;
};
__host__ __device__ inline NsStream ns_begin(const uint64_t (&desc)[4]) { return NsStream{desc[0], 0}; }
__host__ __device__ inline int ns_next(NsStream& s, const uint64_t (&desc)[4]) {
  if (s.j != 0 && (s.j & 15) == 0) s.w = desc[(s.j >> 4) & 3];
  const int ns = (int)(s.w & 15);
  s.w >>= 4;
  ++s.j;
  return ns;
}
inline void nslots_pack_desc(uint64_t (&desc)[4], const int32_t* per_level, int nlevels) {
  desc[0] = desc[1] = desc[2] = desc[3] = 0;
  for (int l = nlevels - 1, j = 0; l >= 1 && j < 64; --l, ++j) desc[j >> 4] |= (uint64_t)(per_level[l] & 15) << ((j & 15) * 4);
}
struct DevModel {
  int32_t nb, nq, nv;
  int32_t lps;
  int32_t nlevels;
  int32_t maxchild;
  int32_t maxnvj;
  int32_t has3dof;
  int32_t inner_floating;
  int32_t debug_stop;
  int32_t nheavy;
  int32_t heavy[4][3];
  const int32_t* ib;
  const void* rb;
  const int32_t* dof_body;
  const uint64_t* row_mask;
  int32_t row_words;
  const int32_t* anc;
  uint64_t perm_down;
  uint64_t ns_desc[4];
  double gravity[3];
};

struct BankModel {
  int32_t lps, nlevels, L0;
  int32_t nbk[2];
  int32_t simple;
  const int32_t* ib[2];
  const void* rb[2];
  uint64_t perm_down;
  uint64_t ns_desc[4];
  double gravity[3];
};

enum { TI_W0 = 0, TI_W1, TI_W2, TI_W3, TI_STRIDE = 4 };
enum { TR_C = 0, TR_PP = 9, TR_J = 12, TR_MC = 18, TR_M = 21, TR_STRIDE = 24 };
enum { TF_VALID = 1, TF_LEVEL0 = 2, TF_CHAINED = 4, TF_CARRY = 8, TF_FLOATING = 16, TF_PRISMATIC = 32, TF_FIXED = 64, TF_SINCOS = 128 };
enum { TMB_A = 30, TMB_B = 27, TMB_C = 6 };
struct TrackModel {
  int32_t ns, G, nA, nB;
  const int32_t* ri;
  const void* rr;
  uint64_t sfm[5];
  double gravity[3];
};

struct WalkModel {
  int32_t ns, G, nA, nB, nS, nq, nv;
  RerootView reroot;
  const int32_t* ri;
  const void* rr;
  const int32_t* wk;
  uint64_t sfm[5];
  double gravity[3];
};

enum { SO_W0 = 0, SO_SLOT, SO_QOFF, SO_VOFF, SO_ORIG6, SO_STRIDE = 8 };
enum { SK_ENTER = 0, SK_EXIT = 1 };
enum { SC_STRIDE = 16, SC_FLOATING = 0x10000, SC_SPHERICAL = 0x20000, SC_PLANAR = 0x40000, SC_MULTI = 0x70000 };
struct StateModel {
  int32_t nb, nq, nv, nops, nlevels;
  const int32_t* ops;
  const int32_t* cols;
  const void* sr;
  const uint64_t* row_mask;
  double gravity[3];
};

struct BigModel {
  int32_t nb, nq, nv, _pad;
  const int32_t* tbl;
  const void* rb;
  double gravity[3];
};

enum { CP_LOC = 0, CP_HCK = 3, CP_HCL = 4, CP_HCN = 5, CP_MU = 6, CP_K = 7, CP_B = 8, CP_STRIDE = 9 };
struct ContactModel {
  int32_t nb, np, nh;
  const int32_t* cbody;
  const void* cp;
  const void* hs;
};

struct Layout {
  long sk, sb;
};
__host__ __device__ inline long layout_base(Layout L, long b) { return L.sb >= 0 ? b * L.sb : (b >> 4) * (16 * -L.sb) + (b & 15); }

template <typename T> struct LoopView {
  int nloops, nc, nv, nb;
  const int32_t* li;
  const T* lr;
  const int32_t* path;
  const int32_t* jt;
  const int32_t* voff;
  const T* axis;
  const T* axis2;
  const int32_t* xi;
  const T* rb;
  const T* gains = nullptr;
};

struct MkBuffers;
struct MkBuffers {
  void* q0; void* v0;
  void* phid[4]; void* vd[4];
};

struct MkFuse {
  int32_t stage;
  int32_t close_prev;
  double dt;
  MkBuffers W;
  void* q_state; void* v_state;
  const void* pd_kp; const void* pd_kd; const void* pd_qdes;
};
// ... 445 lines not shown
```

### rigidbodydynamics.jl_amd/csrc/rbd_jit.hip

```cpp
#include <dlfcn.h>
#include <hip/hip_runtime.h>
#include <hip/hiprtc.h>
#include <sys/stat.h>
#include <unistd.h>

#include <cstdio>
#include <cstdlib>
#include <algorithm>
#include <cstring>
#include <atomic>
#include <map>
#include <memory>
#include <mutex>
#include <thread>
#include <string>
#include <vector>

#include "rbd_internal.hpp"
#include "rbd_jit.hpp"
#include "rbd_walk_plan.hpp"
#include "rbd_jit_embed.inc"

namespace rbd {

// ... 436 lines not shown
    snprintf(b, sizeof b, "  __shared__ __align__(16) %s rnea_lds[%d];\n  rbd::spec::rnea_spec<%s, %s>(B, q, v, vdot, fext, tau, Lq, Lv, Lf, acc_out, jw_out, Lo, rnea_lds);\n}\n", T,
             (dtype == RBD_F32 ? nq + 2 * nv : nq) * 65, T, dtype == RBD_F32 ? "false" : "true");
    s += b;
  }
  if (aba) {
    for (int gst = 0; gst <= (dtype == RBD_F64 ? 1 : 0); ++gst) {
      const int udl = dtype == RBD_F64 ? aba_udl(nb, nq, nv, P.n3, gst) : 0;
      char lds[160];
      snprintf(lds, sizeof lds, "  __shared__ __align__(16) %s aba_lds[%d];\n", T,
               (dtype == RBD_F64 ? aba_f64_rows(nb, nq, nv, P.n3, gst) + udl * nb : nq + 2 * nv + std::max(nq, nb) + 10 * P.n3) * 65);
      for (int fx = 1; fx >= 0; --fx) {
        snprintf(b, sizeof b, "extern \"C\" __global__ __launch_bounds__(64) void aba_spec_%s%s%s(long B, const %s* q, const %s* v, const %s* tau, const %s* fext, %s* vdot,\n"
                 "                                                            %s* qdot, rbd::Layout Lq, rbd::Layout Lv, rbd::Layout Lf, %s gx, %s gy, %s gz, rbd::MkStage F%s) {\n",
                 gst ? "gst_" : "", fx ? "" : "nofext_", sfx, T, T, T, T, T, T, T, T, T, dtype == RBD_F64 ? ", double* stash" : "");
        s += b;
        s += lds;
        snprintf(b, sizeof b, "  rbd::spec::aba_spec<%s, %s, %d, %d>(B, q, v, tau, %s, vdot, qdot, Lq, Lv, Lf, gx, gy, gz, aba_lds, F%s);\n}\n", T, fx ? "true" : "false", udl, gst,
                 fx ? "fext" : "nullptr", dtype == RBD_F64 ? ", stash" : "");
        s += b;
      }
    }
  }
  if (chol) {
    s += "extern \"C\" __global__ __launch_bounds__(256) void crba_spec_perm_f32(long B, const float* q, float* M, rbd::Layout Lq, rbd::Layout Lm, int zero_fill) {\n"
         "  extern __shared__ __align__(16) unsigned char spec_lds[];\n"
         "  rbd::spec::crba_spec<float, true>(B, q, M, Lq, Lm, zero_fill, reinterpret_cast<float*>(spec_lds));\n}\n";
    s += "extern \"C\" __global__ __launch_bounds__(64, RBD_SPEC_CHOL_WAVES) void chol_spec_f32(long B, const float* Mg, const float* tau, const float* c, float* x, rbd::Layout Lv,\n"
         "                                                                   int* notpd, float* Mcopy, rbd::Layout Lc) {\n"
         "  __shared__ __align__(16) float mst[rbd::spec::chol_emit_lds()];\n"
         "  rbd::spec::chol_spec<false, true>(B, blockIdx.x, Mg, tau, c, x, Lv, notpd, Mcopy, Lc, mst);\n}\n";
    s += "extern \"C\" __global__ __launch_bounds__(64, RBD_SPEC_CHOL_WAVES) void chol_spec_nom_f32(long B, const float* Mg, const float* tau, const float* c, float* x, rbd::Layout Lv,\n"
         "                                                                       int* notpd, float* Mcopy, rbd::Layout Lc) {\n"
         "  rbd::spec::chol_spec<false, false>(B, blockIdx.x, Mg, tau, c, x, Lv, notpd, nullptr, Lc, nullptr);\n}\n";
    s += "extern \"C\" __global__ __launch_bounds__(64, RBD_SPEC_CHOL_WAVES) void chol_spec_packed_f32(long B, const float* Mg, const float* tau, const float* c, float* x, rbd::Layout Lv,\n"
         "                                                                          int* notpd, float* Mcopy, rbd::Layout Lc) {\n"
         "  __shared__ __align__(16) float mst[rbd::spec::chol_emit_lds()];\n"
         "  rbd::spec::chol_spec<true, true>(B, blockIdx.x, Mg, tau, c, x, Lv, notpd, Mcopy, Lc, mst);\n}\n";
  }
  if (emit) {
    snprintf(b, sizeof b, "extern \"C\" __global__ __launch_bounds__(64, 2) void emit_spec_%s(long B, const %s* Mg, %s* Mcopy, rbd::Layout Lc) {\n"
                          "  __shared__ __align__(16) %s mst[16 * rbd::spec::emit_mst<%s>()];\n  rbd::spec::emit_spec<%s>(B, blockIdx.x, Mg, Mcopy, Lc, mst);\n}\n", sfx, T, T, T, T, T);
    s += b;
  }
  return s;
}

std::string spec_loop_source(const LoopTables& L, int dtype) {
  if (!(L.nloops > 0 && L.nb <= 4 && L.nv <= 4 && L.nc <= 6 && L.nv < L.nc)) return std::string();
  const char* T = dtype == RBD_F32 ? "float" : "double";
  const char* sfx = dtype == RBD_F32 ? "f32" : "f64";
  std::string s;
  char b[1024];
  s += "// generated by rbd_jit.hip: the loop tables of one small mechanism as constants (rbd_loop_small.hpp)\n#include \"rbd_loop_small.hpp\"\nnamespace rbd_loop_plan {\n";
  auto ints = [&](const char* name, const std::vector<int32_t>& v) {
    snprintf(b, sizeof b, "__device__ const int32_t %s[%d] = ", name, (int)std::max<size_t>(v.size(), 1));
    s += b;
    if (v.empty()) s += "{0}"; else put_ints(s, v.data(), (int)v.size());
    s += ";\n";
  };
  auto reals = [&](const char* name, const std::vector<double>& v) {
    snprintf(b, sizeof b, "__device__ const %s %s[%d] = ", T, name, (int)std::max<size_t>(v.size(), 1));
    s += b;
    if (v.empty()) s += "{0}"; else put_reals(s, v.data(), (int)v.size());
    s += ";\n";
  };
  ints("LI", *L.li); ints("PATH", *L.path); ints("JT", *L.jt); ints("VOFF", *L.voff); ints("XI", *L.xi);
  reals("LR", *L.lr); reals("AXIS", *L.axis); reals("AXIS2", *L.axis2); reals("RB", *L.rb);
  snprintf(b, sizeof b, "struct View {\n  static constexpr int nloops = %d, nc = %d, nv = %d, nb = %d;\n", L.nloops, L.nc, L.nv, L.nb);
  s += b;
  snprintf(b, sizeof b, "  const int32_t* li = LI; const %s* lr = LR; const int32_t* path = PATH; const int32_t* jt = JT; const int32_t* voff = VOFF;\n"
                        "  const %s* axis = AXIS; const %s* axis2 = AXIS2; const int32_t* xi = XI; const %s* rb = RB; const %s* gains = nullptr;\n};\n}  // namespace rbd_loop_plan\n", T, T, T, T, T);
  s += b;
  snprintf(b, sizeof b, "extern \"C\" __global__ __launch_bounds__(64) void loop_spec_%s(long B, int stabilize, const %s* q, const %s* v, const %s* tau, const %s* fext,\n"
                        "    %s* Mg, %s* cg, %s* vdot, %s* qdot, %s* lambda, %s* Kg, %s* kg, rbd::Layout Lq, rbd::Layout Lm, rbd::Layout Lv, rbd::Layout Lf, rbd::Layout Lc,\n"
                        "    rbd::Layout Lk, int* notpd, const %s* gains) {\n", sfx, T, T, T, T, T, T, T, T, T, T, T, T);
  s += b;
  s += "  const long st = (long)blockIdx.x * blockDim.x + threadIdx.x;\n  if (st >= B) return;\n  rbd_loop_plan::View V;\n  V.gains = gains;  // nullptr: the model's gains, compile-time constants\n";
  snprintf(b, sizeof b, "  rbd::loop_fused_small_state<%s, rbd_loop_plan::View, %d, %d, %d, true>(V, st, stabilize, q, v, tau, fext, Mg, Mg, cg, vdot, qdot, lambda, Kg, kg,\n"
                        "      Lq, Lm, Lv, Lf, Lc, Lk, %.17g, %.17g, %.17g, notpd);\n}\n", T, L.nb, L.nv, L.nc, L.gravity[0], L.gravity[1], L.gravity[2]);
  s += b;
  return s;
}

std::string spec_bank_source(int nlevels, int L0, const int32_t* nslots, unsigned long long perm_down, int simple, int dtype) {
  if (nlevels < 2 || nlevels > 64 || L0 < 1 || L0 >= nlevels) return std::string();
  const char* T = dtype == RBD_F32 ? "float" : "double";
  const char* sfx = dtype == RBD_F32 ? "f32" : "f64";
  const char* SI = simple ? "true" : "false";
  std::string s;
  char b[1600];
  s += "// generated by rbd_jit.hip: the level structure of one mechanism for the banked kernels (aba_bank_body / rnea_bank_body, rbd_bank.hpp): loops over the levels unrolled,\n"
       "// DPP hop or exchange column and the number of later children known per level\n";
  snprintf(b, sizeof b, "#define RBD_BANK_FIXED_NL %d\n#define RBD_BANK_FIXED_L0 %d\n#define RBD_BANK_FIXED_PERM 0x%llxull\n#define RBD_BANK_FIXED_NS ", nlevels, L0, perm_down);
  s += b;
  for (int l = 0; l < nlevels; ++l) { snprintf(b, sizeof b, "%s%d", l ? "," : "", (int)nslots[l]); s += b; }
  s += "\n#include \"rbd_lane.hpp\"\n#include \"rbd_bank.hpp\"\n";
  const char* lds = "  __shared__ __align__(16) unsigned char lds[(size_t)rbd::BANK_LDS_PAIRS * 256 * sizeof(rbd::Pair2<%s>)];\n";
  for (int fused = 0; fused < 2; ++fused) {
    snprintf(b, sizeof b, "extern \"C\" __global__ __launch_bounds__(256, RBD_BANK_WAVES) void aba_bank_%sspec_%s(rbd::BankModel M, long B, const %s* q, const %s* v, const %s* tau,\n"
                          "    const %s* fext, %s* vdot, %s* qdot, rbd::Layout Lq, rbd::Layout Lv, rbd::Layout Lf, rbd::MkFuse F) {\n",
             fused ? "fused_" : "", sfx, T, T, T, T, T, T);
    s += b;
    snprintf(b, sizeof b, lds, T);
    s += b;
    snprintf(b, sizeof b, "  rbd::aba_bank_body<%s, %s, %s>(M, B, q, v, tau, fext, vdot, qdot, Lq, Lv, Lf, F, reinterpret_cast<rbd::Pair2<%s>*>(lds));\n}\n", T, fused ? "true" : "false", SI, T);
    s += b;
  }
  snprintf(b, sizeof b, "extern \"C\" __global__ __launch_bounds__(256, 2) void rnea_bank_spec_%s(rbd::BankModel M, long B, int ncol, const %s* q, const %s* v, const %s* vdot, const %s* fext,\n"
                        "    %s* tau, %s* qdot, rbd::Layout Lq, rbd::Layout Lv, rbd::Layout Lf, %s* acc_out, %s* jw_out) {\n"
                        "  __shared__ __align__(16) unsigned char lds[(size_t)rbd::RNEA_LDS_PAIRS * 256 * sizeof(rbd::Pair2<%s>)];\n"
                        "  rbd::rnea_bank_body<%s, %s>(M, B, ncol, q, v, vdot, fext, tau, qdot, Lq, Lv, Lf, acc_out, jw_out, reinterpret_cast<rbd::Pair2<%s>*>(lds));\n}\n",
           sfx, T, T, T, T, T, T, T, T, T, T, SI, T);
  s += b;
  return s;
}

size_t walk_spec_lds_bytes(const WalkTables& W, int dtype, int pair) {
  return walk_rows(W.nq, W.nv, W.nA, W.nB, W.nS) * WR_STRIDE * ((dtype == RBD_F64 || pair) ? 8 : 4);
}
bool walk_spec_has(int dtype, int ns, int G, size_t lds_rows_bytes) {
  return (dtype == RBD_F64 || dtype == RBD_F32) && ns >= 1 && ns <= WALK_MAX_STEPS && G >= 1 && G <= 4 && lds_rows_bytes <= 160 * 1024;
}
const char* walk_spec_suffix(int dtype, int pair) { return dtype == RBD_F64 ? "f64" : pair ? "f32x2" : "f32"; }
std::string walk_spec_source(const WalkTables& W, int dtype, int kind, int pair) {
  if (dtype == RBD_F64) pair = 0;
  const size_t lds = walk_spec_lds_bytes(W, dtype, pair);
  if (!walk_spec_has(dtype, W.ns, W.G, lds)) return std::string();
  const char* S = dtype == RBD_F64 ? "double" : "float";
  const char* T = dtype == RBD_F64 ? "double" : pair ? "rbd::f2" : "float";
  const char* sfx = walk_spec_suffix(dtype, pair);
  std::string s;
  char b[1400];
  {
    const char* e = getenv("RBD_TUNE"); const char* k = e ? strstr(e, "spec_variant=") : nullptr;
    if (k && (atol(k + 13) & 32)) s += "#define RBD_WALK_ABLATE_OUT_LOCAL 1\n";
    if (k && (atol(k + 13) & 256)) s += "#define RBD_WALK_NO_STAGE 1\n";
  }
  if (kind == 2) {
    snprintf(b, sizeof b, "// rbd-walk-sim-loop stash-from=a%d\n// rbd-jit-option: -mllvm\n// rbd-jit-option: -disable-machine-licm\n",
             256 - ((dtype == RBD_F64 || pair) ? 2 : 1) * W.ns * WALK_STASH_N);
    s += b;
  }
  s += "// generated by rbd_jit.hip: the walk plan of one mechanism as constants (aba_walk_spec / rnea_walk_spec, rbd_walk.hpp)\n#include \"rbd_walk.hpp\"\nnamespace rbd_walk_tables {\n";
  const int nrec = W.ns * W.G;
  snprintf(b, sizeof b, "__device__ const int32_t RI[%d] __attribute__((aligned(16))) = ", nrec * TI_STRIDE);
  s += b; put_ints(s, W.ri->data(), nrec * TI_STRIDE); s += ";\n";
  snprintf(b, sizeof b, "__device__ const %s RR[%d] = ", S, nrec * TR_STRIDE);
  s += b; put_reals(s, W.rrc->data(), nrec * TR_STRIDE); s += ";\n";
  snprintf(b, sizeof b, "__device__ const int32_t WK[%d] = ", nrec);
  s += b; put_ints(s, W.wk->data(), nrec); s += ";\n";
  const int nch = W.rr ? W.nchain : 0;
  snprintf(b, sizeof b, "__device__ const int32_t CHI[%d] = ", std::max(nch, 1) * 4);
  s += b; if (nch) put_ints(s, W.chain_i->data(), nch * 4); else s += "{0, 0, 0, 0}"; s += ";\n";
  snprintf(b, sizeof b, "__device__ const %s CHR[%d] = ", S, std::max(nch, 1) * 15);
  s += b; if (nch) put_reals(s, W.chain_r->data(), nch * 15); else s += "{0}"; s += ";\n";
  const int n1 = W.mk1 ? (int)W.mk1->size() / 3 : 0, nf = W.mkf ? (int)W.mkf->size() / 2 : 0;
  snprintf(b, sizeof b, "__device__ const int32_t MK1[%d] = ", std::max(3 * n1, 1));
  s += b; if (n1) put_ints(s, W.mk1->data(), 3 * n1); else s += "{0}"; s += ";\n";
  snprintf(b, sizeof b, "__device__ const int32_t MKF[%d] = ", std::max(2 * nf, 1));
  s += b; if (nf) put_ints(s, W.mkf->data(), 2 * nf); else s += "{0}"; s += ";\n";
  int fw = 0, fewest = 1 << 30;
  for (int g = 0; g < W.G; ++g) {
    int n = 0;
    for (int st = 0; st < W.ns; ++st) n += ((*W.ri)[((size_t)st * W.G + g) * TI_STRIDE + TI_W1] >> 16) & TF_VALID ? 1 : 0;
    if (n < fewest) { fewest = n; fw = g; }
  }
  snprintf(b, sizeof b, "struct Plan {\n  static constexpr int NS = %d, G = %d, NQ = %d, NV = %d, MK_N1 = %d, MK_NF = %d, MK_FW = %d;\n  static constexpr unsigned long long SFM_AW = 0x%llxull, SFM_BW = 0x%llxull;\n",
           W.ns, W.G, W.nq, W.nv, n1, nf, fw, (unsigned long long)W.sfm[1], (unsigned long long)W.sfm[3]);
  s += b;
  s += "  static __device__ __forceinline__ rbd::WalkModel model() {\n    rbd::WalkModel M{};\n";
  snprintf(b, sizeof b, "    M.ns = %d; M.G = %d; M.nA = %d; M.nB = %d; M.nS = %d; M.nq = %d; M.nv = %d;\n    M.ri = RI; M.rr = RR; M.wk = WK;\n", W.ns, W.G, W.nA, W.nB, W.nS,
           W.nq, W.nv);
  s += b;
  for (int k = 0; k < 5; ++k) { snprintf(b, sizeof b, "    M.sfm[%d] = 0x%llxull;\n", k, (unsigned long long)W.sfm[k]); s += b; }
  if (nch) {
    snprintf(b, sizeof b, "    M.reroot.nchain = %d; M.reroot.fq = %d; M.reroot.fv = %d; M.reroot.chain_i = CHI; M.reroot.chain_r = CHR;\n", nch, W.fq, W.fv);
    s += b;
    for (int k = 0; k < 12; ++k) { snprintf(b, sizeof b, "    M.reroot.fXp[%d] = %.17g;\n", k, W.fXp[k]); s += b; }
  }
  s += "    return M;\n  }\n};\n}  // namespace rbd_walk_tables\n";
  if (kind == 0 || kind == 2)
    snprintf(b, sizeof b, "extern \"C\" __global__ __launch_bounds__(%d) void aba_walk_%sspec_%s(long B, const %s* q, const %s* v, const %s* tau, const %s* fext,\n"
                          "    %s* vdot, %s* qdot, rbd::Layout Lq, rbd::Layout Lv, rbd::Layout Lf, double gx, double gy, double gz, rbd::MkStage F) {\n"
                          "  __shared__ __align__(16) unsigned char lds[%zu];\n"
                          "  rbd::aba_walk_spec<%s, %s, %s, %s, rbd_walk_tables::Plan, %s>(B, q, v, tau, fext, vdot, qdot, Lq, Lv, Lf, gx, gy, gz, lds, F, rbd_walk_tables::MK1, rbd_walk_tables::MKF);\n}\n",
             64 * W.G, kind == 2 ? "sim_" : "", sfx, S, S, S, S, S, S, lds, T, W.flt ? "true" : "false", W.gen ? "true" : "false", nch ? "true" : "false", kind == 2 ? "true" : "false");
  else
    snprintf(b, sizeof b, "extern \"C\" __global__ __launch_bounds__(%d) void rnea_walk_spec_%s(long B, const %s* q, const %s* v, const %s* vdot, const %s* fext,\n"
                          "    %s* tau, %s* qdot, rbd::Layout Lq, rbd::Layout Lv, rbd::Layout Lf, %s* acc_out, %s* jw_out, double gx, double gy, double gz) {\n"
                          "  __shared__ __align__(16) unsigned char lds[%zu];\n"
                          "  rbd::rnea_walk_spec<%s, %s, %s, rbd_walk_tables::Plan>(B, q, v, vdot, fext, tau, qdot, Lq, Lv, Lf, acc_out, jw_out, gx, gy, gz, lds);\n}\n",
             64 * W.G, sfx, S, S, S, S, S, S, S, S, lds, T, W.flt ? "true" : "false", W.gen ? "true" : "false");
  s += b;
  return s;
}
// ... 291 lines not shown
```

### rigidbodydynamics.jl_amd/csrc/rbd_jit.hpp

```cpp
#pragma once
#include <cstdint>
#include <string>
#include <vector>

#include "rbd_state_plan.hpp"

namespace rbd {
bool jit_available();
enum { SPEC_MASS = 0, SPEC_ABA = 1, SPEC_RNEA = 2, SPEC_FAMILIES = 3 };
enum { SPEC_KIN = 11, SPEC_SLOTS = 4 };
inline int spec_slot(int family) { return family == SPEC_KIN ? 3 : family; }
bool spec_has(int family, int dtype, int nb, int nq, int nv, int n3 = 0);
bool spec_has_chol(int dtype, int nv);
std::string spec_source(const StatePlan& P, int nb, int nq, int nv, const uint64_t* row_mask, const double* gravity, int dtype, int family);
struct LoopTables {
  int nb, nq, nv, nc, nloops;
  const std::vector<int32_t>*li, *path, *jt, *voff, *xi;
  const std::vector<double>*lr, *axis, *axis2, *rb;
  const double* gravity;
};
std::string spec_loop_source(const LoopTables& L, int dtype);
std::string spec_bank_source(int nlevels, int L0, const int32_t* nslots, unsigned long long perm_down, int simple, int dtype);
struct WalkTables {
  int ns, G, nA, nB, nS, nq, nv, flt, gen, rr;
  const std::vector<int32_t>*ri, *wk;
  const std::vector<double>* rrc;
  uint64_t sfm[5];
  int nchain, fq, fv;
  const std::vector<int32_t>* chain_i;
  const std::vector<double>* chain_r;
  const double* fXp;
  const std::vector<int32_t>*mk1, *mkf;
};
bool walk_spec_has(int dtype, int ns, int G, size_t lds_rows_bytes);
size_t walk_spec_lds_bytes(const WalkTables& W, int dtype, int pair = 0);
const char* walk_spec_suffix(int dtype, int pair);
std::string walk_spec_source(const WalkTables& W, int dtype, int kind = 0, int pair = 0);
enum { JIT_READY = 0, JIT_PENDING = 1, JIT_FAILED = 2 };
bool jit_async();
void jit_wait_idle();
int jit_code_object_get(const std::string& source, bool wait, std::vector<char>* code, std::string* log);
int jit_walk_code_object_get(const std::string& source, bool wait, std::vector<char>* code, std::string* log);
int jit_kd_cover_agprs(std::vector<char>* code);
bool jit_walk_admit(const std::string& source, std::vector<char>* code, std::string* log);
std::vector<char> jit_walk_code_object(const std::string& source, std::string* log);
std::vector<char> jit_code_object(const std::string& source, std::string* log);
void jit_cache_discard(const std::string& source);
}
```

### rigidbodydynamics.jl_amd/state.py

```python
from __future__ import annotations

import ctypes
from typing import Optional

import numpy as np
import torch

from . import _capi
from .mechanism import FlatModel, Mechanism, flatten


class DimensionMismatch(ValueError):
    """Julia's DimensionMismatch (e.g. src/mechanism_algorithms.jl:250)."""


def _raise(status, where):
    try:
        _capi.check(status, where)
    except _capi.RBDError as e:
        if e.status == 2:
            raise DimensionMismatch(str(e)) from None
        if e.status == 1:
            raise ValueError(str(e)) from None
        if e.status == 7:
# ... 875 lines not shown
    import numpy as np
    L = _capi.lib()
    h = ctypes.c_void_p()
    _raise(L.rbd_model_create(ctypes.cast(ctypes.byref(flat.c_struct()), ctypes.c_void_p), ctypes.byref(h)), "rbd_model_create")
    try:
        dims = np.zeros(12, np.int32)
        pi = lambda a: a.ctypes.data_as(ctypes.POINTER(ctypes.c_int32))
        pd = lambda a: a.ctypes.data_as(ctypes.POINTER(ctypes.c_double))
        st = L.rbd_model_reroot_plan(h, pi(dims), None, 0, None, 0, None, 0, None, None, None)
        if st == 3:
            return None
        _raise(st, "rbd_model_reroot_plan")
        n, nch = int(dims[0]) * int(dims[1]), int(dims[7])
        ri, rr, wk = np.zeros(n * 4 + int(dims[1]), np.int32), np.zeros(n * 24, np.float64), np.zeros(n, np.int32)
        ci, cr, fxp = np.zeros(max(4 * nch, 1), np.int32), np.zeros(max(15 * nch, 1), np.float64), np.zeros(12, np.float64)
        _raise(L.rbd_model_reroot_plan(h, None, pi(ri), ri.size, pd(rr), rr.size, pi(wk), wk.size, pi(ci), pd(cr), pd(fxp)), "rbd_model_reroot_plan")
        return {"tracks": int(dims[0]), "steps": int(dims[1]), "root": int(dims[10]), "floating_body": int(dims[11]), "chain": nch, "dims": dims,
                "ri": ri, "rr": rr, "wk": wk, "chain_i": ci, "chain_r": cr, "fxp": fxp}
    finally:
        L.rbd_model_destroy(h)


def track_plan(flat):
    import numpy as np
    L = _capi.lib()
    h = ctypes.c_void_p()
    _raise(L.rbd_model_create(ctypes.cast(ctypes.byref(flat.c_struct()), ctypes.c_void_p), ctypes.byref(h)), "rbd_model_create")
    try:
        dims = np.zeros(6, np.int32)
        pi = lambda a: a.ctypes.data_as(ctypes.POINTER(ctypes.c_int32))
        st = L.rbd_model_track_plan(h, pi(dims), None, 0, None, 0, None, 0)
        if st == 3:
            return None
        _raise(st, "rbd_model_track_plan")
        n = int(dims[0]) * int(dims[1])
        tab, ri, rr = np.zeros(n, np.int32), np.zeros(n * 4 + int(dims[1]), np.int32), np.zeros(n * 24, np.float64)
        _raise(L.rbd_model_track_plan(h, None, pi(tab), tab.size, pi(ri), ri.size, rr.ctypes.data_as(ctypes.POINTER(ctypes.c_double)), rr.size), "rbd_model_track_plan")
        return {"tracks": int(dims[0]), "steps": int(dims[1]), "mailboxes": (int(dims[2]), int(dims[3])), "floating": bool(dims[4]), "general": bool(dims[5]),
                "dims": dims, "table": tab.reshape(int(dims[1]), int(dims[0])), "ri": ri, "rr": rr}
    finally:
        L.rbd_model_destroy(h)


def geometric_jacobian_(out: torch.Tensor, state: MechanismState, base: int, body: int):
    state._check(out, 6 * state.flat.nv, "jacobian")
    state.ws.use_current_stream()
    opts = state._opts()
    _raise(_capi.lib().rbd_geometric_jacobian(state.ws.handle, state.batch, _ptr(state.q), int(base), int(body), _ptr(out), ctypes.byref(opts)),
           "rbd_geometric_jacobian")
    return out


def _momentum(state: MechanismState) -> torch.Tensor:
    out = state._zeros(12)
    state.ws.use_current_stream()
    opts = state._opts()
    _raise(_capi.lib().rbd_momentum(state.ws.handle, state.batch, _ptr(state.q), _ptr(state.v), _ptr(out), ctypes.byref(opts)), "rbd_momentum")
    return out if state.layout == "aos" else out.t()


def momentum(state: MechanismState) -> torch.Tensor:
    return _momentum(state)[:, :6]


def momentum_rate_bias(state: MechanismState) -> torch.Tensor:
    return _momentum(state)[:, 6:]


def bank_plan(flat):
    L = _capi.lib()
    h = ctypes.c_void_p()
    _raise(L.rbd_model_create(ctypes.cast(ctypes.byref(flat.c_struct()), ctypes.c_void_p), ctypes.byref(h)), "rbd_model_create")
    try:
        v = [ctypes.c_int32() for _ in range(5)]
        st = L.rbd_model_bank_plan(h, *[ctypes.byref(x) for x in v])
        if st == 3:
            return None
        _raise(st, "rbd_model_bank_plan")
        return {"lanes": v[0].value, "L0": v[1].value, "bodies": (v[2].value, v[3].value), "aba": bool(v[4].value)}
    finally:
        L.rbd_model_destroy(h)



def contact_dynamics_vjp_(state: MechanismState, cw_bar: Optional[torch.Tensor] = None, sd_bar: Optional[torch.Tensor] = None,
                          s_out_bar: Optional[torch.Tensor] = None, q_bar: Optional[torch.Tensor] = None, v_bar: Optional[torch.Tensor] = None,
                          s_bar: Optional[torch.Tensor] = None, q: Optional[torch.Tensor] = None, v: Optional[torch.Tensor] = None,
                          s: Optional[torch.Tensor] = None):
    f = state.flat
    q = state.q if q is None else q
    v = state.v if v is None else v
    s = state.s if s is None else s
    state._check(q, f.nq, "q")
    state._check(v, f.nv, "v")
    state._check(s, f.ns, "s")
    state._check(cw_bar, 6 * f.n_bodies, "cw_bar")
    state._check(sd_bar, f.ns, "sd_bar")
    state._check(s_out_bar, f.ns, "s_out_bar")
    state._check(q_bar, f.nq, "q_bar")
    state._check(v_bar, f.nv, "v_bar")
    state._check(s_bar, f.ns, "s_bar")
    state.ws.use_current_stream()
    opts = state._opts()
    st = _capi.lib().rbd_contact_dynamics_vjp(state.ws.handle, state.batch, _ptr(q), _ptr(v), _ptr(s), _ptr(cw_bar), _ptr(sd_bar), _ptr(s_out_bar),
                                              _ptr(q_bar), _ptr(v_bar), _ptr(s_bar), ctypes.byref(opts))
    _raise(st, "rbd_contact_dynamics_vjp")
    return q_bar, v_bar, s_bar


def dynamics_contact_vjp_(state: MechanismState, vd_bar: Optional[torch.Tensor] = None, sd_bar: Optional[torch.Tensor] = None,
                          s_out_bar: Optional[torch.Tensor] = None, torques: Optional[torch.Tensor] = None, externalwrenches: Optional[torch.Tensor] = None,
                          q_bar: Optional[torch.Tensor] = None, v_bar: Optional[torch.Tensor] = None, s_bar: Optional[torch.Tensor] = None,
                          tau_bar: Optional[torch.Tensor] = None, fext_bar: Optional[torch.Tensor] = None, vdout: Optional[torch.Tensor] = None,
                          sdout: Optional[torch.Tensor] = None, q: Optional[torch.Tensor] = None, v: Optional[torch.Tensor] = None,
                          s: Optional[torch.Tensor] = None):
    f = state.flat
    q = state.q if q is None else q
    v = state.v if v is None else v
    s = state.s if s is None else s
    state._check(q, f.nq, "q")
    state._check(v, f.nv, "v")
    state._check(s, f.ns, "s")
    state._check(torques, f.nv, "torques")
    state._check(externalwrenches, 6 * f.n_bodies, "externalwrenches")
    state._check(vd_bar, f.nv, "vd_bar")
    state._check(sd_bar, f.ns, "sd_bar")
    state._check(s_out_bar, f.ns, "s_out_bar")
    state._check(vdout, f.nv, "vdout")
    state._check(sdout, f.ns, "sdout")
    state._check(q_bar, f.nq, "q_bar")
    state._check(v_bar, f.nv, "v_bar")
    state._check(s_bar, f.ns, "s_bar")
    state._check(tau_bar, f.nv, "tau_bar")
    state._check(fext_bar, 6 * f.n_bodies, "fext_bar")
    state.ws.use_current_stream()
    opts = state._opts()
    st = _capi.lib().rbd_dynamics_contact_vjp(state.ws.handle, state.batch, _ptr(q), _ptr(v), _ptr(s), _ptr(torques), _ptr(externalwrenches), _ptr(vd_bar),
                                              _ptr(sd_bar), _ptr(s_out_bar), _ptr(vdout), _ptr(sdout), _ptr(q_bar), _ptr(v_bar), _ptr(s_bar), _ptr(tau_bar),
                                              _ptr(fext_bar), ctypes.byref(opts))
    _raise(st, "rbd_dynamics_contact_vjp")
    return q_bar, v_bar, s_bar, tau_bar, fext_bar


def simulate_contact_vjp_(q_bar: torch.Tensor, v_bar: torch.Tensor, s_bar: torch.Tensor, state: MechanismState, dt: float, nsteps: int = 1,
                          torques: Optional[torch.Tensor] = None, externalwrenches: Optional[torch.Tensor] = None, tau_bar: Optional[torch.Tensor] = None,
                          fext_bar: Optional[torch.Tensor] = None, q: Optional[torch.Tensor] = None, v: Optional[torch.Tensor] = None,
                          s: Optional[torch.Tensor] = None):
    f = state.flat
    q = state.q if q is None else q
    v = state.v if v is None else v
    s = state.s if s is None else s
    if not float(dt) > 0:
        raise ValueError("dt must be positive")
    if int(nsteps) < 0:
        raise ValueError("nsteps must be non-negative")
    if q_bar is None or v_bar is None or s_bar is None:
        raise ValueError("q_bar, v_bar and s_bar are required (in / out)")
    state._check(q, f.nq, "q")
    state._check(v, f.nv, "v")
    state._check(s, f.ns, "s")
    state._check(q_bar, f.nq, "q_bar")
    state._check(v_bar, f.nv, "v_bar")
    state._check(s_bar, f.ns, "s_bar")
    state._check(torques, f.nv, "torques")
    state._check(externalwrenches, 6 * f.n_bodies, "externalwrenches")
    state._check(tau_bar, f.nv, "tau_bar")
# ... 9 lines not shown
```

Before: 216.0 million.

## Stage bank body tables and per-state q/v/tau rows in LDS before compute

The banked ABA and RNEA kernels now copy the per-body constant table into LDS cooperatively, using 16-byte vector loads from all threads, and read it from there instead of from global memory per lane. Per-state q, v and tau rows are also loaded coalesced into the exchange region of LDS and then gathered per joint, replacing strided per-lane global loads. The LDS size grows with the body count, so occupancy accounting is recomputed through shared helpers, and a query API exposes the sizes. The cost is an extra block-wide barrier and larger LDS use, which for f64 can limit residency to one workgroup per CU.

```diff
diff --git a/include/rbd_hip.h b/include/rbd_hip.h
--- a/include/rbd_hip.h
+++ b/include/rbd_hip.h
@@ -107,6 +107,8 @@
 int rbd_model_destroy(rbd_model_t* model);
 int rbd_model_bank_plan(const rbd_model_t* model, int32_t* lanes, int32_t* first_level_of_bank1, int32_t* bodies_bank0, int32_t* bodies_bank1,
                         int32_t* aba_in_scope);
+int rbd_model_bank_lds(const rbd_model_t* model, int32_t dtype, int64_t* dynamics_bytes, int64_t* inverse_dynamics_bytes, int32_t* workgroups_per_cu,
+                       int32_t* states_per_workgroup, int32_t* row_scalars_per_wavefront);
 int rbd_model_track_plan(const rbd_model_t* model, int32_t* dims, int32_t* table, int32_t table_cap, int32_t* ri, int32_t ri_cap, double* rr, int32_t rr_cap);
 int rbd_model_reroot_plan(const rbd_model_t* model, int32_t* dims, int32_t* ri, int32_t ri_cap, double* rr, int32_t rr_cap, int32_t* wk, int32_t wk_cap,
                           int32_t* chain_i, double* chain_r, double* fxp);
diff --git a/rigidbodydynamics.jl_amd/__init__.py b/rigidbodydynamics.jl_amd/__init__.py
--- a/rigidbodydynamics.jl_amd/__init__.py
+++ b/rigidbodydynamics.jl_amd/__init__.py
@@ -8,7 +8,7 @@
                        rand_tree_mechanism, randmech, tree_mechanism)
 from .flatio import load_flat_model, save_flat_model
 from . import _capi
-from .state import (PDGains, SE3PDGains, default_constraint_stabilization_gains, TorqueTable, PDControl, jit_source, jit_precompile, jit_status, bank_plan, track_plan, reroot_plan, momentum, momentum_rate_bias, geometric_jacobian_, chain_plan, center_of_mass, gravitational_potential_energy, kinetic_energy, momentum_matrix_, DimensionMismatch, DynamicsResult, MechanismState, dynamics_, dynamics_bias_, dynamics_ode_, inverse_dynamics_, mass_matrix_, unpack_lower, inverse_dynamics_jvp_, dynamics_jvp_, inverse_dynamics_derivatives_, dynamics_derivatives_, simulate_jvp_, simulate_step_derivatives_, inverse_dynamics_vjp_, dynamics_vjp_, simulate_vjp_, jacobian_view, set_points_, point_kinematics_, point_kinematics_vjp_, point_jacobian_view, contact_dynamics_vjp_, dynamics_contact_vjp_, simulate_contact_vjp_,
+from .state import (PDGains, SE3PDGains, default_constraint_stabilization_gains, TorqueTable, PDControl, jit_source, jit_precompile, jit_status, bank_plan, bank_lds, track_plan, reroot_plan, momentum, momentum_rate_bias, geometric_jacobian_, chain_plan, center_of_mass, gravitational_potential_energy, kinetic_energy, momentum_matrix_, DimensionMismatch, DynamicsResult, MechanismState, dynamics_, dynamics_bias_, dynamics_ode_, inverse_dynamics_, mass_matrix_, unpack_lower, inverse_dynamics_jvp_, dynamics_jvp_, inverse_dynamics_derivatives_, dynamics_derivatives_, simulate_jvp_, simulate_step_derivatives_, inverse_dynamics_vjp_, dynamics_vjp_, simulate_vjp_, jacobian_view, set_points_, point_kinematics_, point_kinematics_vjp_, point_jacobian_view, contact_dynamics_vjp_, dynamics_contact_vjp_, simulate_contact_vjp_,
                     mass_matrix_solve_, rand_, set_configuration_, set_velocity_, simulate_, sync, last_kernel, zero_configuration_)
 from .distributed import Comm, gather_results, shard_range, shard_sizes
 from . import autograd
diff --git a/rigidbodydynamics.jl_amd/_capi.py b/rigidbodydynamics.jl_amd/_capi.py
--- a/rigidbodydynamics.jl_amd/_capi.py
+++ b/rigidbodydynamics.jl_amd/_capi.py
@@ -28,6 +28,7 @@
     "rbd_workspace_set_points", "rbd_point_kinematics", "rbd_point_kinematics_vjp",
     "rbd_contact_dynamics_vjp", "rbd_dynamics_contact_vjp",
     "rbd_simulate_contact_vjp",
+    "rbd_model_bank_lds",
 )
 
 
@@ -113,6 +114,8 @@
         L.rbd_geometric_jacobian.argtypes = [vp, i32, vp, i32, i32, vp, ctypes.POINTER(Opts)]
         L.rbd_momentum.argtypes = [vp, i32, vp, vp, vp, ctypes.POINTER(Opts)]
         L.rbd_model_bank_plan.argtypes = [vp] + [ctypes.POINTER(i32)] * 5
+        if hasattr(L, "rbd_model_bank_lds"):
+            L.rbd_model_bank_lds.argtypes = [vp, i32] + [ctypes.POINTER(ctypes.c_int64)] * 2 + [ctypes.POINTER(i32)] * 3
         L.rbd_kinematics.argtypes = [vp, i32, vp, vp, vp, vp, vp, ctypes.POINTER(Opts)]
         L.rbd_simulate.argtypes = [vp, i32, vp, vp, vp, vp, ctypes.c_double, i32, ctypes.POINTER(Opts)]
         L.rbd_mk_stage.argtypes = [vp, i32, i32, ctypes.c_double, vp, vp, vp, ctypes.POINTER(Opts)]
diff --git a/rigidbodydynamics.jl_amd/csrc/rbd_bank.hpp b/rigidbodydynamics.jl_amd/csrc/rbd_bank.hpp
--- a/rigidbodydynamics.jl_amd/csrc/rbd_bank.hpp
+++ b/rigidbodydynamics.jl_amd/csrc/rbd_bank.hpp
@@ -56,7 +56,7 @@
   for (int k = 0; k < N; k += 6) massign6(mask, d + k, s + k);
 }
 
-enum { PK_KIN = 0, PK_FWD = 6, PARK_PAIRS = 16, PK_XCH = 16, XCH_PAIRS = 14, BANK_LDS_PAIRS = PARK_PAIRS + XCH_PAIRS };
+enum { PK_KIN = 0, PK_FWD = 6, PARK_PAIRS = BANK_PARK_PAIRS, PK_XCH = BANK_PARK_PAIRS, XCH_PAIRS = BANK_XCH_PAIRS };
 
 template <typename T, int N> RBD_DEV void lds_put(Pair2<T>* col, int pair0, const T* x) {
 #pragma unroll
@@ -73,6 +73,115 @@
     const Pair2<T> v = col[(pair0 + i) * 256];
     x[2 * i] = v.a;
     if (2 * i + 1 < N) x[2 * i + 1] = v.b;
+  }
+}
+
+template <typename T> struct Quad16Of;
+template <> struct Quad16Of<double> { typedef double type __attribute__((ext_vector_type(2))); };
+template <> struct Quad16Of<float> { typedef float type __attribute__((ext_vector_type(4))); };
+template <typename T> using Quad16 = typename Quad16Of<T>::type;
+template <typename T> struct BankTableRegs {
+  enum { CH = RB_STRIDE * sizeof(T) / 16 , N = (64 * CH + 255) / 256  };
+  static_assert(RB_STRIDE * sizeof(T) % 16 == 0 && bank_table_stride(sizeof(T)) * sizeof(T) % 16 == 0 && bank_table_stride(sizeof(T)) >= RB_STRIDE, "16-byte chunks");
+  Quad16<T> c[N];
+};
+template <typename T> RBD_DEV void bank_table_load(const BankModel& M, BankTableRegs<T>& r) {
+  constexpr int CH = BankTableRegs<T>::CH;
+  const int n0 = M.nbk[0] * CH, n = n0 + M.nbk[1] * CH;
+  const Quad16<T>* const s0 = reinterpret_cast<const Quad16<T>*>(M.rb[0]);
+  const Quad16<T>* const s1 = reinterpret_cast<const Quad16<T>*>(M.rb[1]);
+#pragma unroll
+  for (int i = 0; i < BankTableRegs<T>::N; ++i) {
+    const int c = (int)threadIdx.x + 256 * i;
+    if (c < n) r.c[i] = c < n0 ? s0[c] : s1[c - n0];
+  }
+}
+template <typename T> RBD_DEV void bank_table_store(const BankModel& M, const BankTableRegs<T>& r, T* tbl) {
+  constexpr int CH = BankTableRegs<T>::CH, ST = bank_table_stride(sizeof(T));
+  const int n0 = M.nbk[0] * CH, n = n0 + M.nbk[1] * CH;
+#pragma unroll
+  for (int i = 0; i < BankTableRegs<T>::N; ++i) {
+    const int c = (int)threadIdx.x + 256 * i;
+    if (c < n) {
+      const int cc = c < n0 ? c : c - n0, row = cc / CH + (c < n0 ? 0 : M.nbk[0]);
+      *reinterpret_cast<Quad16<T>*>(tbl + row * ST + (cc % CH) * (16 / (int)sizeof(T))) = r.c[i];
+    }
+  }
+}
+template <typename T> RBD_DEV const T* bank_table_row(const BankModel& M, const T* tbl, int k, int sub) {
+  return tbl + ((k ? M.nbk[0] : 0) + (sub < M.nbk[k] ? sub : 0)) * bank_table_stride(sizeof(T));
+}
+
+enum { BANK_ROWS_BATCH = 3 };
+template <typename T> struct BankRows {
+  T* base;
+  int first, nq, nv, sub, lps;
+  long sc;
+  RBD_DEV T& at(int e) const { const int L = first + e; return base[((L >> 7) << 9) + (L & 127)]; }
+};
+template <typename T> struct BankRowsRegs { T q[BANK_ROWS_BATCH], v[BANK_ROWS_BATCH], a[BANK_ROWS_BATCH]; };
+template <typename T> RBD_DEV BankRows<T> bank_rows_begin(const BankModel& M, long B, Pair2<T>* lds, int xch_pair0) {
+  BankRows<T> r;
+  const int lane = threadIdx.x & 63;
+  const long wave = ((long)blockIdx.x * blockDim.x + threadIdx.x) >> 6;
+  r.base = reinterpret_cast<T*>(lds + xch_pair0 * 256 + ((int)threadIdx.x - lane));
+  r.nq = M.nq; r.nv = M.nv; r.lps = M.lps;
+  r.sub = lane & (M.lps - 1);
+  const int sh = __builtin_ctz(M.lps), g = lane >> sh;
+  r.first = g * (M.nq + 2 * M.nv);
+  const long state = wave * (64 >> sh) + g;
+  r.sc = state < B ? state : B - 1;
+  return r;
+}
+template <typename T> RBD_DEV void bank_row_load(const BankRows<T>& r, const T* __restrict__ p, Layout L, int n, T* x) {
+  const T* const p0 = p + ((long)r.sub * L.sk + r.sc * L.sb);
+  const long d = (long)r.lps * L.sk;
+#pragma unroll
+  for (int i = 0; i < BANK_ROWS_BATCH; ++i) x[i] = (p != nullptr && r.sub + i * r.lps < n) ? p0[i * d] : T(0);
+}
+template <typename T> RBD_DEV void bank_row_store(const BankRows<T>& r, const T* __restrict__ p, Layout L, int n, int e0, const T* x) {
+#pragma unroll
+  for (int i = 0; i < BANK_ROWS_BATCH; ++i) {
+    const int e = r.sub + i * r.lps;
+    if (e < n) r.at(e0 + e) = x[i];
+  }
+#pragma unroll 1
+  for (int e = r.sub + BANK_ROWS_BATCH * r.lps; e < n; e += r.lps) r.at(e0 + e) = p != nullptr ? p[(long)e * L.sk + r.sc * L.sb] : T(0);
+}
+template <typename T> RBD_DEV void bank_rows_load(const BankRows<T>& r, const T* __restrict__ q, const T* __restrict__ v, const T* __restrict__ a, Layout Lq, Layout Lv, BankRowsRegs<T>& x) {
+  bank_row_load<T>(r, q, Lq, r.nq, x.q);
+  bank_row_load<T>(r, v, Lv, r.nv, x.v);
+  bank_row_load<T>(r, a, Lv, r.nv, x.a);
+}
+template <typename T> RBD_DEV void bank_rows_store(const BankRows<T>& r, const T* __restrict__ q, const T* __restrict__ v, const T* __restrict__ a, Layout Lq, Layout Lv, const BankRowsRegs<T>& x) {
+  bank_row_store<T>(r, q, Lq, r.nq, 0, x.q);
+  bank_row_store<T>(r, v, Lv, r.nv, r.nq, x.v);
+  bank_row_store<T>(r, a, Lv, r.nv, r.nq + r.nv, x.a);
+}
+template <typename T> RBD_DEV void bank_rows_joint(const BankRows<T>& r, const Body<T>& b, T* qj, T* vj, T* aj) {
+  const int nq = joint_nq<T>(b.jtype), nv = joint_nv(b.jtype);
+#pragma unroll
+  for (int k = 0; k < 7; ++k) qj[k] = (b.valid && k < nq) ? r.at(b.qoff + k) : T(0);
+#pragma unroll
+  for (int k = 0; k < 6; ++k) vj[k] = (b.valid && k < nv) ? r.at(r.nq + b.voff + k) : T(0);
+#pragma unroll
+  for (int k = 0; k < 6; ++k) aj[k] = (b.valid && k < nv) ? r.at(r.nq + r.nv + b.voff + k) : T(0);
+}
+template <typename T> RBD_DEV void bank_rows_joint_simple(const BankRows<T>& r, const Body<T>& b, T* qj, T* vj, T* aj) {
+  const int iq = b.qoff, iv = r.nq + b.voff, ia = r.nq + r.nv + b.voff;
+  qj[0] = r.at(iq);
+  vj[0] = r.at(iv);
+  aj[0] = r.at(ia);
+#pragma unroll
+  for (int k = 1; k < 7; ++k) qj[k] = T(0);
+#pragma unroll
+  for (int k = 1; k < 6; ++k) { vj[k] = T(0); aj[k] = T(0); }
+  if (b.jtype == RBD_JOINT_QUAT_FLOATING) {
+    RBD_KEEP_BRANCH();
+#pragma unroll
+    for (int k = 1; k < 7; ++k) qj[k] = r.at(iq + k);
+#pragma unroll
+    for (int k = 1; k < 6; ++k) { vj[k] = r.at(iv + k); aj[k] = r.at(ia + k); }
   }
 }
 
@@ -280,10 +389,8 @@
   Pair2<T>* const col = lds + threadIdx.x;
   RBD_MARK(0);
   BankRegs<T> r0, r1;
+  T* const tbl = reinterpret_cast<T*>(lds + BANK_LDS_PAIRS * 256);
   auto fetch = [&](int k, BankRegs<T>& c, T* qj, T* vj) {
-    load_bank_body(M, k, B, c.b);
-    c.rb = reinterpret_cast<const T*>(M.rb[k]) + (c.b.sub < M.nbk[k] ? c.b.sub : 0) * RB_STRIDE;
-    c.pcol = (int)threadIdx.x - c.b.sub + (c.b.parent >= 0 ? c.b.parent : c.b.sub);
     if (SIMPLE) {
       const bool fl = c.b.jtype == RBD_JOINT_QUAT_FLOATING;
       const long sc = c.b.state < B ? c.b.state : B - 1;
@@ -419,8 +526,36 @@
   };
 
   T qj0[7], vj0[6], qj1[7], vj1[6];
-  fetch(0, r0, qj0, vj0);
-  fetch(1, r1, qj1, vj1);
+  {
+    BankTableRegs<T> tr;
+    bank_table_load<T>(M, tr);
+    const BankRows<T> rows = bank_rows_begin<T>(M, B, lds, PK_XCH);
+    BankRowsRegs<T> rx;
+    if (!FUSED) bank_rows_load<T>(rows, q, v, tau, Lq, Lv, rx);
+    load_bank_body(M, 0, B, r0.b);
+    load_bank_body(M, 1, B, r1.b);
+    r0.rb = bank_table_row<T>(M, tbl, 0, r0.b.sub);
+    r1.rb = bank_table_row<T>(M, tbl, 1, r1.b.sub);
+    r0.pcol = (int)threadIdx.x - r0.b.sub + (r0.b.parent >= 0 ? r0.b.parent : r0.b.sub);
+    r1.pcol = (int)threadIdx.x - r1.b.sub + (r1.b.parent >= 0 ? r1.b.parent : r1.b.sub);
+    if (FUSED) {
+      fetch(0, r0, qj0, vj0);
+      fetch(1, r1, qj1, vj1);
+    }
+    bank_table_store<T>(M, tr, tbl);
+    if (!FUSED) bank_rows_store<T>(rows, q, v, tau, Lq, Lv, rx);
+    __syncthreads();
+    if (!FUSED) {
+      if (SIMPLE) {
+        bank_rows_joint_simple<T>(rows, r0.b, qj0, vj0, r0.tj);
+        bank_rows_joint_simple<T>(rows, r1.b, qj1, vj1, r1.tj);
+      } else {
+        bank_rows_joint<T>(rows, r0.b, qj0, vj0, r0.tj);
+        bank_rows_joint<T>(rows, r1.b, qj1, vj1, r1.tj);
+      }
+      wave_lds_sync();
+    }
+  }
   if (FUSED) {
     if (F.close_prev) {
       mk_stage_lane(r0.b, 4, (T)F.dt, qj0, vj0, (const T*)nullptr, F.W, (T*)F.q_state, (T*)F.v_state, Lq, Lv);
@@ -552,7 +687,6 @@
 }
 #endif
 
-enum { RNEA_LDS_PAIRS = 12 };
 template <typename T> struct RneaRegs {
   Body<T> b;
   const T* rb;
@@ -643,41 +777,30 @@
                             T* __restrict__ jw_out, Pair2<T>* const lds) {
   RneaRegs<T> r0, r1;
   const bool out_vec = store6_vec(acc_out ? acc_out : jw_out, Lf, (int)sizeof(T)) && store6_vec(jw_out ? jw_out : acc_out, Lf, (int)sizeof(T));
-  auto fetch = [&](int k, RneaRegs<T>& c, T* qj, T* vj, T* aj) {
-    load_bank_body(M, k, B, c.b);
-    c.rb = reinterpret_cast<const T*>(M.rb[k]) + (c.b.sub < M.nbk[k] ? c.b.sub : 0) * RB_STRIDE;
-    c.pcol = (int)threadIdx.x - c.b.sub + (c.b.parent >= 0 ? c.b.parent : c.b.sub);
+  T* const tbl = reinterpret_cast<T*>(lds + RNEA_LDS_PAIRS * 256);
+  auto fetch = [&](T* qj0, T* vj0, T* aj0, T* qj1, T* vj1, T* aj1) {
+    BankTableRegs<T> tr;
+    bank_table_load<T>(M, tr);
+    const BankRows<T> rows = bank_rows_begin<T>(M, B, lds, 0);
+    BankRowsRegs<T> rx;
+    bank_rows_load<T>(rows, q, v, vdot, Lq, Lv, rx);
+    load_bank_body(M, 0, B, r0.b);
+    load_bank_body(M, 1, B, r1.b);
+    r0.rb = bank_table_row<T>(M, tbl, 0, r0.b.sub);
+    r1.rb = bank_table_row<T>(M, tbl, 1, r1.b.sub);
+    r0.pcol = (int)threadIdx.x - r0.b.sub + (r0.b.parent >= 0 ? r0.b.parent : r0.b.sub);
+    r1.pcol = (int)threadIdx.x - r1.b.sub + (r1.b.parent >= 0 ? r1.b.parent : r1.b.sub);
+    bank_table_store<T>(M, tr, tbl);
+    bank_rows_store<T>(rows, q, v, vdot, Lq, Lv, rx);
+    __syncthreads();
     if (SIMPLE) {
-      const bool fl = c.b.jtype == RBD_JOINT_QUAT_FLOATING;
-      const long sc = c.b.state < B ? c.b.state : B - 1;
-      const T* qp = q + ((long)c.b.qoff * Lq.sk + sc * Lq.sb);
-      const long va = (long)c.b.voff * Lv.sk + sc * Lv.sb;
-      const bool hv = v != nullptr, ha = vdot != nullptr;
-      qj[0] = qp[0];
-      vj[0] = hv ? v[va] : T(0);
-      aj[0] = ha ? vdot[va] : T(0);
-#pragma unroll
-      for (int k2 = 1; k2 < 7; ++k2) qj[k2] = T(0);
-#pragma unroll
-      for (int k2 = 1; k2 < 6; ++k2) { vj[k2] = T(0); aj[k2] = T(0); }
-      if (fl) {
-        RBD_KEEP_BRANCH();
-#pragma unroll
-        for (int k2 = 1; k2 < 7; ++k2) qj[k2] = qp[k2 * Lq.sk];
-        if (hv) {
-#pragma unroll
-          for (int k2 = 1; k2 < 6; ++k2) vj[k2] = v[va + k2 * Lv.sk];
-        }
-        if (ha) {
-#pragma unroll
-          for (int k2 = 1; k2 < 6; ++k2) aj[k2] = vdot[va + k2 * Lv.sk];
-        }
-      }
+      bank_rows_joint_simple<T>(rows, r0.b, qj0, vj0, aj0);
+      bank_rows_joint_simple<T>(rows, r1.b, qj1, vj1, aj1);
     } else {
-      load_joint_q(c.b, q, Lq, qj);
-      load_joint_v(c.b, v, Lv, vj);
-      load_joint_v(c.b, vdot, Lv, aj);
-    }
+      bank_rows_joint<T>(rows, r0.b, qj0, vj0, aj0);
+      bank_rows_joint<T>(rows, r1.b, qj1, vj1, aj1);
+    }
+    wave_lds_sync();
   };
   auto setup = [&](RneaRegs<T>& c, const T* qj, const T* vj, const T* aj, T* XR, T* Xp, T* tl, T* al, T* ta) {
     if (SIMPLE) {
@@ -772,8 +895,7 @@
   };
 
   T qj0[7], vj0[6], aj0[6], qj1[7], vj1[6], aj1[6];
-  fetch(0, r0, qj0, vj0, aj0);
-  fetch(1, r1, qj1, vj1, aj1);
+  fetch(qj0, vj0, aj0, qj1, vj1, aj1);
   {
     T XR[9], Xp[3], tl[6], al[6], ta[5];
     setup(r0, qj0, vj0, aj0, XR, Xp, tl, al, ta);
diff --git a/rigidbodydynamics.jl_amd/csrc/rbd_bank_kernels.hip b/rigidbodydynamics.jl_amd/csrc/rbd_bank_kernels.hip
--- a/rigidbodydynamics.jl_amd/csrc/rbd_bank_kernels.hip
+++ b/rigidbodydynamics.jl_amd/csrc/rbd_bank_kernels.hip
@@ -4,8 +4,7 @@
 
 namespace rbd {
 
-static_assert(BANK_LDS_PAIRS == 30, "rbd_capi.hip sizes the resident batch of the banked kernel with BANK_LDS_PAIRS_HOST = 30");
-template <typename T> static size_t bank_lds_bytes() { return (size_t)BANK_LDS_PAIRS * 256 * sizeof(Pair2<T>); }
+static_assert(sizeof(Pair2<double>) == 16 && sizeof(Pair2<float>) == 8, "bank_lds_bytes (rbd_device.hpp) counts a pair as two scalars");
 
 template <typename T>
 hipError_t launch_aba_bank(const BankModel& M, long B, const void* q, const void* v, const void* tau, const void* fext, void* vdot, void* qdot,
@@ -15,7 +14,7 @@
   if (fuse) F = *fuse;
   const long spw = 64 / M.lps, waves = (B + spw - 1) / spw;
   const dim3 grid((unsigned)((waves + 3) / 4)), block(256);
-  const size_t lds = bank_lds_bytes<T>();
+  const size_t lds = bank_lds_bytes(0, (int)sizeof(T), M.nbk[0], M.nbk[1]);
 #define RBD_LAUNCH_BANK(FU, SI) \
   hipLaunchKernelGGL((aba_bank_kernel<T, FU, SI>), grid, block, lds, s, M, B, (const T*)q, (const T*)v, (const T*)tau, (const T*)fext, (T*)vdot, (T*)qdot, Lq, Lv, Lf, F)
   if (F.stage >= 0) { if (M.simple) RBD_LAUNCH_BANK(true, true); else RBD_LAUNCH_BANK(true, false); }
@@ -25,7 +24,7 @@
   return hipGetLastError();
 }
 template <typename T> hipError_t configure_bank_kernels() {
-  const int lds = (int)bank_lds_bytes<T>();
+  const int lds = (int)bank_lds_bytes(0, (int)sizeof(T), 32, 32);
   hipError_t e = hipFuncSetAttribute(reinterpret_cast<const void*>(&aba_bank_kernel<T, false, false>), hipFuncAttributeMaxDynamicSharedMemorySize, lds);
   if (e == hipSuccess) e = hipFuncSetAttribute(reinterpret_cast<const void*>(&aba_bank_kernel<T, false, true>), hipFuncAttributeMaxDynamicSharedMemorySize, lds);
   if (e == hipSuccess) e = hipFuncSetAttribute(reinterpret_cast<const void*>(&aba_bank_kernel<T, true, false>), hipFuncAttributeMaxDynamicSharedMemorySize, lds);
@@ -47,7 +46,8 @@
 hipError_t launch_rnea_bank(const BankModel& M, long B, int ncol, const void* q, const void* v, const void* vdot, const void* fext, void* tau, void* qdot,
                             Layout Lq, Layout Lv, Layout Lf, hipStream_t s, void* acc_out, void* jw_out) {
   const long spw = 64 / M.lps, waves = (B + spw - 1) / spw;
-  const size_t lds = (size_t)RNEA_LDS_PAIRS * 256 * sizeof(Pair2<T>);
+  const size_t lds = bank_lds_bytes(1, (int)sizeof(T), M.nbk[0], M.nbk[1]);
+  static_assert(bank_lds_bytes(1, 8, 32, 32) <= 64 * 1024, "rnea_bank_kernel stays under the default dynamic-LDS limit");
   if (M.simple)
     hipLaunchKernelGGL((rnea_bank_kernel<T, true>), dim3((unsigned)((waves + 3) / 4)), dim3(256), lds, s, M, B, ncol, (const T*)q, (const T*)v, (const T*)vdot,
                        (const T*)fext, (T*)tau, (T*)qdot, Lq, Lv, Lf, (T*)acc_out, (T*)jw_out);
diff --git a/rigidbodydynamics.jl_amd/csrc/rbd_capi.hip b/rigidbodydynamics.jl_amd/csrc/rbd_capi.hip
--- a/rigidbodydynamics.jl_amd/csrc/rbd_capi.hip
+++ b/rigidbodydynamics.jl_amd/csrc/rbd_capi.hip
@@ -1,5 +1,4 @@
 #include "rbd_capi_internal.hpp"
-enum { BANK_LDS_PAIRS_HOST = 30 };
 
 thread_local std::string g_last_hip_error;
 
@@ -392,7 +391,7 @@
       const int diff = std::abs(cA - cB);
       if (lanes < best_lanes || (lanes == best_lanes && diff < best_diff)) { best_lanes = lanes; best_L0 = L0; best_diff = diff; }
     }
-    if (best_lanes < m->lps) {
+    if (best_lanes < m->lps && bank_rows_fit(0, best_lanes, m->nq, m->nv) && bank_rows_fit(1, best_lanes, m->nq, m->nv)) {
       m->bank_lps = best_lanes; m->bank_L0 = best_L0;
       std::vector<int> bslot(nb, -1);
       int cnt[2] = {0, 0};
@@ -510,6 +509,19 @@
   return RBD_OK;
 }
 
+int rbd_model_bank_lds(const rbd_model_t* m, int32_t dtype, int64_t* dynamics_bytes, int64_t* inverse_dynamics_bytes, int32_t* workgroups_per_cu,
+                       int32_t* states_per_workgroup, int32_t* row_scalars_per_wavefront) {
+  if (!m || (dtype != RBD_F64 && dtype != RBD_F32)) return RBD_ERR_INVALID_ARGUMENT;
+  if (m->bank_lps <= 0) return RBD_ERR_UNSUPPORTED;
+  const int esize = dtype == RBD_F64 ? 8 : 4;
+  if (dynamics_bytes) *dynamics_bytes = (int64_t)bank_lds_bytes(0, esize, m->bank_nb[0], m->bank_nb[1]);
+  if (inverse_dynamics_bytes) *inverse_dynamics_bytes = (int64_t)bank_lds_bytes(1, esize, m->bank_nb[0], m->bank_nb[1]);
+  if (workgroups_per_cu) *workgroups_per_cu = bank_workgroups_per_cu(esize, m->bank_nb[0], m->bank_nb[1]);
+  if (states_per_workgroup) *states_per_workgroup = 256 / m->bank_lps;
+  if (row_scalars_per_wavefront) *row_scalars_per_wavefront = (64 / m->bank_lps) * (m->nq + 2 * m->nv);
+  return RBD_OK;
+}
+
 int rbd_model_chain_plan(const rbd_model_t* m, int32_t* tracks, int32_t* steps, int32_t* lds_fields, int32_t* table, int32_t capacity) {
   if (!m) return RBD_ERR_INVALID_ARGUMENT;
   if (!m->chain.ok) return RBD_ERR_UNSUPPORTED;
@@ -665,6 +677,7 @@
     }
     if (st != RBD_OK) return st;
     bm.lps = m->bank_lps; bm.nlevels = m->nlevels; bm.L0 = m->bank_L0; bm.perm_down = m->bank_perm_down;
+    bm.nq = m->nq; bm.nv = m->nv;
     bm.simple = bank_simple(m);
     if (tune("bank_generic", 0)) bm.simple = 0;
     nslots_pack_desc(bm.ns_desc, m->nslots.data(), m->nlevels);
@@ -680,8 +693,8 @@
     {
       int ncu = 256;
       (void)hipDeviceGetAttribute(&ncu, hipDeviceAttributeMultiprocessorCount, device);
-      const size_t lds = (size_t)BANK_LDS_PAIRS_HOST * 256 * 2 * (dtype == RBD_F64 ? 8 : 4);
-      const long per_cu = std::max<long>(1, std::min<long>(2, (long)(160 * 1024 / lds)));
+      const long per_cu = bank_workgroups_per_cu(dtype == RBD_F64 ? 8 : 4, m->bank_nb[0], m->bank_nb[1]);
+      if (per_cu < 1) return RBD_ERR_UNSUPPORTED;
       w->bank_resident_states = (long)ncu * per_cu * (256 / m->bank_lps);
     }
   }
@@ -937,7 +950,7 @@
 }
 static std::string bank_program_source(const rbd_model* m, int dtype, int simple) {
   if (m->bank_lps <= 0) return std::string();
-  return spec_bank_source(m->nlevels, m->bank_L0, m->nslots.data(), (unsigned long long)m->bank_perm_down, simple, dtype);
+  return spec_bank_source(m->nlevels, m->bank_L0, m->nslots.data(), (unsigned long long)m->bank_perm_down, simple, dtype, m->bank_nb[0], m->bank_nb[1]);
 }
 static std::string loop_program_source(const rbd_model* m, int dtype, std::vector<int32_t>* xi_store) {
   if (!m->loop_fused_ok) return std::string();
diff --git a/rigidbodydynamics.jl_amd/csrc/rbd_device.hpp b/rigidbodydynamics.jl_amd/csrc/rbd_device.hpp
--- a/rigidbodydynamics.jl_amd/csrc/rbd_device.hpp
+++ b/rigidbodydynamics.jl_amd/csrc/rbd_device.hpp
@@ -59,12 +59,25 @@
   int32_t lps, nlevels, L0;
   int32_t nbk[2];
   int32_t simple;
+  int32_t nq, nv;
   const int32_t* ib[2];
   const void* rb[2];
   uint64_t perm_down;
   uint64_t ns_desc[4];
   double gravity[3];
 };
+enum { BANK_PARK_PAIRS = 16, BANK_XCH_PAIRS = 14, BANK_LDS_PAIRS = BANK_PARK_PAIRS + BANK_XCH_PAIRS, RNEA_LDS_PAIRS = 12 };
+__host__ __device__ constexpr int bank_table_stride(int esize) { return esize == 8 ? 30 : 28; }
+__host__ __device__ constexpr size_t bank_lds_bytes(int kind, int esize, int nbk0, int nbk1) {
+  return (size_t)(kind == 0 ? BANK_LDS_PAIRS : RNEA_LDS_PAIRS) * 256 * 2 * esize + (size_t)(nbk0 + nbk1) * bank_table_stride(esize) * esize;
+}
+__host__ __device__ constexpr int bank_workgroups_per_cu(int esize, int nbk0, int nbk1) {
+  return (int)(160 * 1024 / bank_lds_bytes(0, esize, nbk0, nbk1)) < 2 ? (int)(160 * 1024 / bank_lds_bytes(0, esize, nbk0, nbk1)) : 2;
+}
+__host__ __device__ constexpr bool bank_rows_fit(int kind, int lps, int nq, int nv) {
+  return lps >= 1 && lps <= 32 && (64 / lps) * (nq + 2 * nv) <= (kind == 0 ? BANK_XCH_PAIRS : RNEA_LDS_PAIRS) * 128;
+}
+static_assert(bank_workgroups_per_cu(8, 32, 32) == 1 && bank_workgroups_per_cu(4, 32, 32) == 2, "the largest table (32 + 32 bodies) keeps one fp64 / two fp32 workgroups per compute unit");
 
 enum { TI_W0 = 0, TI_W1, TI_W2, TI_W3, TI_STRIDE = 4 };
 enum { TR_C = 0, TR_PP = 9, TR_J = 12, TR_MC = 18, TR_M = 21, TR_STRIDE = 24 };
diff --git a/rigidbodydynamics.jl_amd/csrc/rbd_jit.hip b/rigidbodydynamics.jl_amd/csrc/rbd_jit.hip
--- a/rigidbodydynamics.jl_amd/csrc/rbd_jit.hip
+++ b/rigidbodydynamics.jl_amd/csrc/rbd_jit.hip
@@ -542,7 +542,8 @@
   return s;
 }
 
-std::string spec_bank_source(int nlevels, int L0, const int32_t* nslots, unsigned long long perm_down, int simple, int dtype) {
+std::string spec_bank_source(int nlevels, int L0, const int32_t* nslots, unsigned long long perm_down, int simple, int dtype, int nbk0, int nbk1) {
+  if (nbk0 < 1 || nbk1 < 1 || nbk0 > 32 || nbk1 > 32) return std::string();
   if (nlevels < 2 || nlevels > 64 || L0 < 1 || L0 >= nlevels) return std::string();
   const char* T = dtype == RBD_F32 ? "float" : "double";
   const char* sfx = dtype == RBD_F32 ? "f32" : "f64";
@@ -555,22 +556,22 @@
   s += b;
   for (int l = 0; l < nlevels; ++l) { snprintf(b, sizeof b, "%s%d", l ? "," : "", (int)nslots[l]); s += b; }
   s += "\n#include \"rbd_lane.hpp\"\n#include \"rbd_bank.hpp\"\n";
-  const char* lds = "  __shared__ __align__(16) unsigned char lds[(size_t)rbd::BANK_LDS_PAIRS * 256 * sizeof(rbd::Pair2<%s>)];\n";
+  const char* lds = "  __shared__ __align__(16) unsigned char lds[rbd::bank_lds_bytes(0, sizeof(%s), %d, %d)];\n";
   for (int fused = 0; fused < 2; ++fused) {
     snprintf(b, sizeof b, "extern \"C\" __global__ __launch_bounds__(256, RBD_BANK_WAVES) void aba_bank_%sspec_%s(rbd::BankModel M, long B, const %s* q, const %s* v, const %s* tau,\n"
                           "    const %s* fext, %s* vdot, %s* qdot, rbd::Layout Lq, rbd::Layout Lv, rbd::Layout Lf, rbd::MkFuse F) {\n",
              fused ? "fused_" : "", sfx, T, T, T, T, T, T);
     s += b;
-    snprintf(b, sizeof b, lds, T);
+    snprintf(b, sizeof b, lds, T, nbk0, nbk1);
     s += b;
     snprintf(b, sizeof b, "  rbd::aba_bank_body<%s, %s, %s>(M, B, q, v, tau, fext, vdot, qdot, Lq, Lv, Lf, F, reinterpret_cast<rbd::Pair2<%s>*>(lds));\n}\n", T, fused ? "true" : "false", SI, T);
     s += b;
   }
   snprintf(b, sizeof b, "extern \"C\" __global__ __launch_bounds__(256, 2) void rnea_bank_spec_%s(rbd::BankModel M, long B, int ncol, const %s* q, const %s* v, const %s* vdot, const %s* fext,\n"
                         "    %s* tau, %s* qdot, rbd::Layout Lq, rbd::Layout Lv, rbd::Layout Lf, %s* acc_out, %s* jw_out) {\n"
-                        "  __shared__ __align__(16) unsigned char lds[(size_t)rbd::RNEA_LDS_PAIRS * 256 * sizeof(rbd::Pair2<%s>)];\n"
+                        "  __shared__ __align__(16) unsigned char lds[rbd::bank_lds_bytes(1, sizeof(%s), %d, %d)];\n"
                         "  rbd::rnea_bank_body<%s, %s>(M, B, ncol, q, v, vdot, fext, tau, qdot, Lq, Lv, Lf, acc_out, jw_out, reinterpret_cast<rbd::Pair2<%s>*>(lds));\n}\n",
-           sfx, T, T, T, T, T, T, T, T, T, T, SI, T);
+           sfx, T, T, T, T, T, T, T, T, T, nbk0, nbk1, T, SI, T);
   s += b;
   return s;
 }
diff --git a/rigidbodydynamics.jl_amd/csrc/rbd_jit.hpp b/rigidbodydynamics.jl_amd/csrc/rbd_jit.hpp
--- a/rigidbodydynamics.jl_amd/csrc/rbd_jit.hpp
+++ b/rigidbodydynamics.jl_amd/csrc/rbd_jit.hpp
@@ -20,7 +20,7 @@
   const double* gravity;
 };
 std::string spec_loop_source(const LoopTables& L, int dtype);
-std::string spec_bank_source(int nlevels, int L0, const int32_t* nslots, unsigned long long perm_down, int simple, int dtype);
+std::string spec_bank_source(int nlevels, int L0, const int32_t* nslots, unsigned long long perm_down, int simple, int dtype, int nbk0, int nbk1);
 struct WalkTables {
   int ns, G, nA, nB, nS, nq, nv, flt, gen, rr;
   const std::vector<int32_t>*ri, *wk;
diff --git a/rigidbodydynamics.jl_amd/state.py b/rigidbodydynamics.jl_amd/state.py
--- a/rigidbodydynamics.jl_amd/state.py
+++ b/rigidbodydynamics.jl_amd/state.py
@@ -981,6 +981,22 @@
         L.rbd_model_destroy(h)
 
 
+def bank_lds(flat, dtype=torch.float64):
+    L = _capi.lib()
+    h = ctypes.c_void_p()
+    _raise(L.rbd_model_create(ctypes.cast(ctypes.byref(flat.c_struct()), ctypes.c_void_p), ctypes.byref(h)), "rbd_model_create")
+    try:
+        b = [ctypes.c_int64() for _ in range(2)]
+        v = [ctypes.c_int32() for _ in range(3)]
+        st = L.rbd_model_bank_lds(h, _capi.F64 if dtype == torch.float64 else _capi.F32, *[ctypes.byref(x) for x in b + v])
+        if st == 3:
+            return None
+        _raise(st, "rbd_model_bank_lds")
+        return {"dynamics": b[0].value, "inverse_dynamics": b[1].value, "workgroups_per_cu": v[0].value, "states_per_workgroup": v[1].value, "row_scalars": v[2].value}
+    finally:
+        L.rbd_model_destroy(h)
+
+
 
 def contact_dynamics_vjp_(state: MechanismState, cw_bar: Optional[torch.Tensor] = None, sd_bar: Optional[torch.Tensor] = None,
                           s_out_bar: Optional[torch.Tensor] = None, q_bar: Optional[torch.Tensor] = None, v_bar: Optional[torch.Tensor] = None,
```

New measurement: 205.7 million. -4.8%, worse.
